# MohammadJohari/myslam

Measured on AMD Instinct MI355X. Metric: ray.samples/s (render+bwd), higher is better.
Workload: dtype f32; 1 GPU; BASELINE configs[1]: Replica room0 (synthetic), 4096 rays x 64 samples (56+8); mapping iteration: sample + render fwd + loss + bwd (planes+decoders), no optimiser; rays_of_the_job=4096, rays_this_rank=4096, samples_per_ray=64, plane_bytes=27147008, planes_layout=channels_last, parallelism=single GPU, launch=hipGraph replay of the captured iteration

## Files before the change

### include/eslam_hip.h

```cpp
#ifndef ESLAM_HIP_H
#define ESLAM_HIP_H

#include <stdint.h>

#ifdef __cplusplus
extern "C" {
#endif

#define ESLAM_ABI_VERSION 5
#define ESLAM_C_DIM 32
#define ESLAM_HIDDEN 16
#define ESLAM_FEAT (2 * ESLAM_C_DIM)
#define ESLAM_N_PLANES 12
#define ESLAM_MAX_SAMPLES 256
#define ESLAM_RAY_ORDERS 3
#define ESLAM_RAY_ORDER_WORDS(R) (ESLAM_RAY_ORDERS * (int64_t)(R) + 4)
#define ESLAM_N_DEC_PARAMS (2 * (16 * 64 + 16 + 16 * 16 + 16) + (1 * 16 + 1) + (3 * 16 + 3))

typedef void* eslam_stream_t;

typedef struct {
    const float* data;
    float* grad;
    int32_t h, w;
// ... 35 lines not shown
int eslam_importance_z(const eslam_plane_t* planes, const eslam_decoders_t* dec, const float* bound6_host,
                       const float* rays_o, const float* rays_d, const float* gt_depth, int R, int n_strat,
                       int n_imp, const float* t_free, const float* t_rand_uni, const float* u, float* z_vals,
                       eslam_stream_t stream);

int eslam_sample_z_all(const eslam_plane_t* planes, const eslam_decoders_t* dec, const float* bound6_host,
                       const float* rays_o, const float* rays_d, const float* gt_depth, int R, int n_strat, int n_imp,
                       double truncation, const float* t_free, const float* t_surf, const float* t_rand,
                       const float* t_rand_uni, const float* u, float* z_vals, eslam_stream_t stream);

int eslam_sample_z_all_rng(const eslam_plane_t* planes, const eslam_decoders_t* dec, const float* bound6_host,
                           const float* rays_o, const float* rays_d, const float* gt_depth, int R, int n_strat, int n_imp,
                           double truncation, const float* t_free, const float* t_surf, int perturb, uint64_t seed,
                           const uint32_t* rng_state, int64_t ray_offset, float* z_vals, eslam_stream_t stream);

int eslam_render_fwd(const eslam_plane_t* planes, const eslam_decoders_t* dec, const float* bound6_host,
                     const float* rays_o, const float* rays_d, const float* z_vals, int R, int S, float* depth,
                     float* rgb, float* sdf, float* raw_rgb, float* feat, const int32_t* ray_order,
                     uint32_t* rng_bump, eslam_stream_t stream);

int eslam_render_fwd_loss(const eslam_plane_t* planes, const eslam_decoders_t* dec, const float* bound6_host,
                          const float* rays_o, const float* rays_d, const float* z_vals, int R, int S, float* depth,
                          float* rgb, float* sdf, float* raw_rgb, float* feat, const int32_t* ray_order,
                          const float* gt_depth, const float* gt_color, double truncation, const float* weights5_host,
                          const uint8_t* ray_mask, float* scratch, float* acc, float* loss, uint32_t* rng_bump,
                          eslam_stream_t stream);

int eslam_planes_to_half(const eslam_plane_t* planes, eslam_stream_t stream);

int eslam_planes_relayout(const eslam_plane_t* src, const eslam_plane_t* dst, int field, eslam_stream_t stream);

int eslam_render_fwd_lowp(const eslam_plane_t* planes_f16, const eslam_decoders_t* dec, const float* bound6_host,
                          const float* rays_o, const float* rays_d, const float* z_vals, int R, int S, float* depth,
                          float* rgb, float* sdf, eslam_stream_t stream);

int eslam_ray_order(const float* rays_o, const float* rays_d, int R, int32_t* perm, eslam_stream_t stream);

int64_t eslam_bwd_workspace_bytes(int64_t n_points);

int eslam_render_bwd(const eslam_plane_t* planes, const eslam_decoders_t* dec, const float* bound6_host,
                     const float* rays_o, const float* rays_d, const float* z_vals, int R, int S,
                     const float* sdf, const float* raw_rgb, const float* feat, const float* g_depth,
                     const float* g_rgb, const float* g_sdf, float* g_dec, float* g_beta, float* g_rays_o,
                     float* g_rays_d, const int32_t* ray_order, void* workspace, eslam_stream_t stream);

int eslam_render_bwd_loss(const eslam_plane_t* planes, const eslam_decoders_t* dec, const float* bound6_host,
                          const float* rays_o, const float* rays_d, const float* z_vals, int R, int S,
                          const float* sdf, const float* raw_rgb, const float* feat, const float* depth,
                          const float* rgb, const float* gt_depth, const float* gt_color, double truncation,
                          const float* weights5_host, const uint8_t* ray_mask, const float* acc,
                          const float* upstream, float* loss_out, const float* g_depth, const float* g_rgb,
                          const float* g_sdf, float* g_dec, float* g_beta, float* g_rays_o, float* g_rays_d,
                          const int32_t* ray_order, void* workspace, eslam_stream_t stream);

#define ESLAM_DECODE_SDF_ONLY 1
#define ESLAM_DECODE_MASK_OUTSIDE 2
int eslam_decode_fwd(const eslam_plane_t* planes, const eslam_decoders_t* dec, const float* bound6_host,
                     const float* pts, int64_t N, int flags, float* raw, float* feat, eslam_stream_t stream);

int eslam_sdf_grid(const eslam_plane_t* planes, const eslam_decoders_t* dec, const float* bound6_host,
                   const float* xs, const float* ys, const float* zs, int64_t nx, int64_t ny, int64_t nz,
                   const float* halfspaces, int n_halfspaces, int flags, float* vol, eslam_stream_t stream);

int64_t eslam_mc_workspace_bytes(int64_t nx, int64_t ny, int64_t nz);
int eslam_mc_count(const float* vol, int64_t nx, int64_t ny, int64_t nz, float level, void* workspace, int64_t* counts,
                   eslam_stream_t stream);
int eslam_mc_emit(const float* vol, int64_t nx, int64_t ny, int64_t nz, float level, const double* origin3_host,
                  const double* spacing3_host, const void* workspace, int64_t n_verts, int64_t n_faces, float* verts,
                  int32_t* faces, eslam_stream_t stream);

int eslam_mc_count_masked(const float* vol, const float* weight, int64_t nx, int64_t ny, int64_t nz, float level,
                          void* workspace, int64_t* counts, eslam_stream_t stream);

int eslam_tsdf_integrate(float* tsdf, float* weight, float* color, int64_t nx, int64_t ny, int64_t nz,
                         const float* origin3_host, float voxel, float trunc, const float* depths, const float* colors,
                         const float* w2c, const float* depth_max, int n_frames, int H, int W, float fx, float fy, float cx,
                         float cy, eslam_stream_t stream);

int eslam_tsdf_sample_color(const float* color, int64_t nx, int64_t ny, int64_t nz, const float* origin3_host, float voxel,
                            const float* pts, int64_t n, float* out, eslam_stream_t stream);

int eslam_frame_out_shape(int Hc, int Wc, int Hd, int Wd, int crop_h, int crop_w, int crop_edge, int* H_out_host,
                          int* W_out_host);
int eslam_frame_prepare(const uint8_t* rgb, int Hc, int Wc, const uint16_t* depth, int Hd, int Wd, int crop_h, int crop_w,
                        int crop_edge, float png_depth_scale, float scale, float* color_out, float* depth_out,
                        eslam_stream_t stream);

int eslam_frame_undistort(const uint8_t* rgb, const float* grid, int H, int W, uint8_t* out, eslam_stream_t stream);

int eslam_cull_vertices(const float* verts, int64_t n_verts, const float* depths, int n_frames, int depth_h, int depth_w,
                        const float* w2c, float fx, float fy, float cx, float cy, int H, int W, float truncation,
                        int depth_test, uint8_t* seen, eslam_stream_t stream);

#define ESLAM_NN_MAX_CELLS (1 << 24)
#define ESLAM_NN_CELLS_PER_POINT 2
#define ESLAM_NN_INPUT_ORDER 1
typedef struct {
    float lo[3];
    float cell;
    int32_t dims[3];
    int32_t reserved;
} eslam_nn_grid_t;
int eslam_nn_grid_plan(int64_t n_ref, const float* bbox6_host, eslam_nn_grid_t* grid);
int64_t eslam_nn_workspace_bytes(const eslam_nn_grid_t* grid, int64_t n_ref);
int eslam_nn_build(const float* ref, int64_t n_ref, const eslam_nn_grid_t* grid, void* workspace, eslam_stream_t stream);
int64_t eslam_nn_query_workspace_bytes(const eslam_nn_grid_t* grid, int64_t n_query);
// ... 52 lines not shown
                    const double* stats, const uint8_t* lut, uint8_t* out, eslam_stream_t stream);

int eslam_views_see_points(const float* points, int64_t n_points, const float* w2c, int n_views, float fx, float fy,
                           float cx, float cy, int H, int W, uint8_t* seen, eslam_stream_t stream);

int eslam_decode_bwd(const eslam_plane_t* planes, const eslam_decoders_t* dec, const float* bound6_host,
                     const float* pts, int64_t N, const float* raw, const float* feat, const float* g_raw,
                     float* g_dec, float* g_pts, void* workspace, eslam_stream_t stream);

int eslam_mapping_loss(const float* depth, const float* rgb, const float* sdf, const float* z_vals,
                       const float* gt_depth, const float* gt_color, int R, int S, double truncation,
                       const float* weights5_host, const uint8_t* ray_mask, float* loss,
                       float* g_depth, float* g_rgb, float* g_sdf, void* scratch, eslam_stream_t stream);

#define ESLAM_LOSS_ACC 16
int eslam_loss_reduce(const float* depth, const float* rgb, const float* sdf, const float* z_vals,
                      const float* gt_depth, const float* gt_color, int R, int S, double truncation,
                      const uint8_t* ray_mask, float* acc, eslam_stream_t stream);
int eslam_loss_grad(const float* depth, const float* rgb, const float* sdf, const float* z_vals,
                    const float* gt_depth, const float* gt_color, int R, int S, double truncation,
                    const float* weights5_host, const uint8_t* ray_mask, const float* acc, float* loss,
                    float* g_depth, float* g_rgb, float* g_sdf, const float* upstream, eslam_stream_t stream);

#define ESLAM_ADAM_MAX_TENSORS 32
typedef struct {
    float* param;
    float* grad;
    float* exp_avg;
    float* exp_avg_sq;
    int64_t n;
    double lr;
} eslam_adam_tensor_t;
int eslam_adam_step(const eslam_adam_tensor_t* tensors_host, int n_tensors, int step, int32_t* step_dev,
                    double beta1, double beta2, double eps, int zero_grad, eslam_stream_t stream);

int eslam_keyframe_overlap(const float* rays_o, const float* rays_d, const float* gt_depth, int n_rays,
                           int num_samples, const float* c2ws, int n_keyframes, int H, int W, float fx, float fy,
                           float cx, float cy, int edge, int32_t* counts, eslam_stream_t stream);

#define ESLAM_TRACKING_MASK_MAX 8192
int eslam_prefilter(const float* rays_o, const float* rays_d, const float* gt_depth, int R, const float* bound6_host,
                    int need_depth, uint8_t* keep, eslam_stream_t stream);
int eslam_pose_to_c2w(const float* poses, int b, float* c2ws, eslam_stream_t stream);
int eslam_pose_to_c2w_bwd(const float* poses, const float* g_c2ws, int b, float* g_poses, eslam_stream_t stream);
int eslam_tracking_mask(const float* depth, const float* gt_depth, const uint8_t* keep, int R, float factor,
                        uint8_t* mask, eslam_stream_t stream);
int eslam_keep_best(const float* loss, const float* pose, int n, float* best, float* best_pose,
                    eslam_stream_t stream);

#define ESLAM_LOSS_SCRATCH (32 * 17)
int eslam_deterministic(void);
int eslam_scatter_bundle_samples(int64_t n, int S, int render);
int eslam_last_backward_rank16(void);

int eslam_stream_wait(eslam_stream_t waiter, eslam_stream_t signaler);

int eslam_zero_async(void* ptr, int64_t bytes, eslam_stream_t stream);
int64_t eslam_loss_scratch_floats(int64_t n_rays);
int eslam_loss_scratch_reset(float* scratch, int64_t floats, eslam_stream_t stream);
int eslam_loss_value(const float* depth, const float* rgb, const float* sdf, const float* z_vals,
                     const float* gt_depth, const float* gt_color, int R, int S, double truncation,
                     const float* weights5_host, const uint8_t* ray_mask, float* scratch, float* acc, float* loss,
                     eslam_stream_t stream);

#define ESLAM_PROF_KERNELS 12
int eslam_profile_enable(int on);
int eslam_profile_read(float* ms_out);
const char* eslam_profile_name(int kernel_id);

int eslam_loss_set_sizes(const float* gt_depth, const uint8_t* ray_mask, int R, int n_strat, int n_imp, double truncation,
                         const float* t_free, const float* t_surf, const float* t_rand, int perturb, uint64_t seed,
                         const uint32_t* rng_state, uint32_t* scratch, float* acc_out, eslam_stream_t stream);
int eslam_mark_rays(const eslam_plane_t* planes, const float* bound6_host, const float* rays_o, const float* rays_d,
                    const float* gt_depth, int R, double truncation, const int64_t* block_base_host, int64_t n_blocks,
                    uint8_t* touched, eslam_stream_t stream);
int64_t eslam_blocks_compact_scratch_words(int64_t n_blocks);
int eslam_blocks_compact(uint8_t* touched, int64_t n_blocks, uint32_t* scratch, int32_t* idx, int32_t* meta,
                         int32_t* host_meta_dev, int clear_touched, eslam_stream_t stream);
int eslam_host_meta_alloc(void** host_ptr, void** dev_ptr);
int eslam_host_meta_free(void* host_ptr);
int eslam_shard_prologue(float* clear_flat, const int32_t* clear_idx, const int32_t* clear_meta, int64_t clear_capacity,
                         float* clear_tail, int64_t clear_n_tail, const float* rays_o, const float* rays_d,
                         const float* gt_depth, const uint8_t* ray_mask, int R, int n_strat, int n_imp, double truncation,
                         const float* t_free, const float* t_surf, int perturb, uint64_t seed, const uint32_t* rng_state,
                         uint32_t* sizes_scratch, float* acc_out, const eslam_plane_t* mark_planes, const float* bound6_host,
                         const int64_t* block_base_host, int64_t n_blocks, uint8_t* touched, eslam_stream_t stream);
int eslam_blocks_pack_dev(const float* flat, const int32_t* idx, const int32_t* meta, int64_t capacity, const float* tail,
                          int64_t n_tail, int64_t tail_pad, float* buf, uint32_t* step_bump, eslam_stream_t stream);
int eslam_blocks_unpack_dev(float* flat, const int32_t* idx, const int32_t* meta, int64_t capacity, float* tail,
                            int64_t n_tail, int64_t tail_pad, const float* buf, eslam_stream_t stream);
int eslam_blocks_zero_dev(float* flat, const int32_t* idx, const int32_t* meta, int64_t capacity, float* tail, int64_t n_tail,
                          eslam_stream_t stream);

#ifdef __cplusplus
}
#endif
#endif
```

### myslam_amd/_hip.py

```python
import ctypes
import os
import threading

import torch

_HERE = os.path.dirname(os.path.abspath(__file__))
LIB_PATH = os.environ.get("ESLAM_HIP_LIB") or os.path.join(_HERE, "lib", "libeslam_hip.so")

ABI_VERSION = 5
RAY_ORDERS = 3


def ray_order_words(R):
    return RAY_ORDERS * int(R) + 4
N_DEC_PARAMS = 2692
N_PLANES = 12


class PlaneDesc(ctypes.Structure):
    _fields_ = [("data", ctypes.c_void_p), ("grad", ctypes.c_void_p), ("h", ctypes.c_int32), ("w", ctypes.c_int32),
                ("stride_c", ctypes.c_int64), ("stride_y", ctypes.c_int64), ("stride_x", ctypes.c_int64),
                ("data_f16", ctypes.c_void_p)]


# ... 15 lines not shown
NN_INPUT_ORDER = 1
ICP_MOMENTS = 17
MESH_MAX_COUNT = 1 << 30
RASTER_LARGE_AREA = 64
RASTER_Z_NEAR = 0.01
RASTER_Z_FAR = 20.0
STATS_BLOCK_PIXELS = 4096
SSIM_TILE_H = 16
SSIM_TILE_W = 32
Bound6 = ctypes.c_float * 6

_vp, _i, _i64, _f, _d = ctypes.c_void_p, ctypes.c_int, ctypes.c_int64, ctypes.c_float, ctypes.c_double
_PP = ctypes.POINTER(PlaneDesc)
_DP = ctypes.POINTER(DecodersDesc)
_BP = ctypes.POINTER(ctypes.c_float)
_GP = ctypes.POINTER(NnGrid)

SIGNATURES = {
    "eslam_last_error": (ctypes.c_char_p, []),
    "eslam_abi_version": (_i, []),
    "eslam_sample_rays": (_i, [_vp, _i, _i, _i, _i, _i, _i, _i, _i, _f, _f, _f, _f, _vp, _vp, _vp, _vp, _vp, _vp, _vp, _vp]),
    "eslam_sample_rays_bwd": (_i, [_vp, _i, _i, _i, _i, _i, _f, _f, _f, _f, _vp, _vp, _vp, _vp]),
    "eslam_image_rays": (_i, [_i, _i, _f, _f, _f, _f, _vp, _vp, _vp, _vp]),
    "eslam_aabb_exit": (_i, [_vp, _vp, _i, _BP, _vp, _vp]),
    "eslam_sample_z": (_i, [_vp, _i, _i, _i, _d, _vp, _vp, _vp, _vp, _vp]),
    "eslam_importance_z": (_i, [_PP, _DP, _BP, _vp, _vp, _vp, _i, _i, _i, _vp, _vp, _vp, _vp, _vp]),
    "eslam_sample_z_all": (_i, [_PP, _DP, _BP, _vp, _vp, _vp, _i, _i, _i, _d, _vp, _vp, _vp, _vp, _vp, _vp, _vp]),
    "eslam_sample_z_all_rng": (_i, [_PP, _DP, _BP, _vp, _vp, _vp, _i, _i, _i, _d, _vp, _vp, _i, ctypes.c_uint64, _vp, _i64, _vp, _vp]),
    "eslam_loss_set_sizes": (_i, [_vp, _vp, _i, _i, _i, _d, _vp, _vp, _vp, _i, ctypes.c_uint64, _vp, _vp, _vp, _vp]),
    "eslam_mark_rays": (_i, [_PP, _BP, _vp, _vp, _vp, _i, _d, _vp, _i64, _vp, _vp]),
    "eslam_blocks_compact_scratch_words": (_i64, [_i64]),
    "eslam_blocks_compact": (_i, [_vp, _i64, _vp, _vp, _vp, _vp, _i, _vp]),
    "eslam_host_meta_alloc": (_i, [ctypes.POINTER(ctypes.c_void_p), ctypes.POINTER(ctypes.c_void_p)]),
    "eslam_host_meta_free": (_i, [_vp]),
    "eslam_shard_prologue": (_i, [_vp, _vp, _vp, _i64, _vp, _i64, _vp, _vp, _vp, _vp, _i, _i, _i, _d, _vp, _vp, _i, ctypes.c_uint64,
                                  _vp, _vp, _vp, _PP, _BP, _vp, _i64, _vp, _vp]),
    "eslam_blocks_pack_dev": (_i, [_vp, _vp, _vp, _i64, _vp, _i64, _i64, _vp, _vp, _vp]),
    "eslam_blocks_unpack_dev": (_i, [_vp, _vp, _vp, _i64, _vp, _i64, _i64, _vp, _vp]),
    "eslam_blocks_zero_dev": (_i, [_vp, _vp, _vp, _i64, _vp, _i64, _vp]),
    "eslam_render_fwd": (_i, [_PP, _DP, _BP, _vp, _vp, _vp, _i, _i, _vp, _vp, _vp, _vp, _vp, _vp, _vp, _vp]),
    "eslam_render_fwd_loss": (_i, [_PP, _DP, _BP, _vp, _vp, _vp, _i, _i, _vp, _vp, _vp, _vp, _vp, _vp, _vp, _vp, _d, _BP, _vp,
                                   _vp, _vp, _vp, _vp, _vp]),
    "eslam_planes_to_half": (_i, [_PP, _vp]),
    "eslam_planes_relayout": (_i, [_PP, _PP, _i, _vp]),
    "eslam_render_fwd_lowp": (_i, [_PP, _DP, _BP, _vp, _vp, _vp, _i, _i, _vp, _vp, _vp, _vp]),
    "eslam_ray_order": (_i, [_vp, _vp, _i, _vp, _vp]),
    "eslam_stream_wait": (_i, [_vp, _vp]),
    "eslam_zero_async": (_i, [_vp, _i64, _vp]),
    "eslam_bwd_workspace_bytes": (_i64, [_i64]),
    "eslam_render_bwd": (_i, [_PP, _DP, _BP, _vp, _vp, _vp, _i, _i, _vp, _vp, _vp, _vp, _vp, _vp, _vp, _vp, _vp, _vp,
                              _vp, _vp, _vp]),
    "eslam_render_bwd_loss": (_i, [_PP, _DP, _BP, _vp, _vp, _vp, _i, _i, _vp, _vp, _vp, _vp, _vp, _vp, _vp, _d, _BP, _vp, _vp,
                                   _vp, _vp, _vp, _vp, _vp, _vp, _vp, _vp, _vp, _vp, _vp, _vp]),
    "eslam_decode_fwd": (_i, [_PP, _DP, _BP, _vp, _i64, _i, _vp, _vp, _vp]),
    "eslam_sdf_grid": (_i, [_PP, _DP, _BP, _vp, _vp, _vp, _i64, _i64, _i64, _vp, _i, _i, _vp, _vp]),
    "eslam_mc_workspace_bytes": (_i64, [_i64, _i64, _i64]),
    "eslam_mc_count": (_i, [_vp, _i64, _i64, _i64, _f, _vp, _vp, _vp]),
    "eslam_mc_emit": (_i, [_vp, _i64, _i64, _i64, _f, ctypes.POINTER(_d), ctypes.POINTER(_d), _vp, _i64, _i64, _vp, _vp, _vp]),
    "eslam_mc_count_masked": (_i, [_vp, _vp, _i64, _i64, _i64, _f, _vp, _vp, _vp]),
    "eslam_tsdf_integrate": (_i, [_vp, _vp, _vp, _i64, _i64, _i64, ctypes.POINTER(_f), _f, _f, _vp, _vp, _vp, _vp, _i, _i, _i,
                                  _f, _f, _f, _f, _vp]),
    "eslam_tsdf_sample_color": (_i, [_vp, _i64, _i64, _i64, ctypes.POINTER(_f), _f, _vp, _i64, _vp, _vp]),
    "eslam_frame_out_shape": (_i, [_i, _i, _i, _i, _i, _i, _i, ctypes.POINTER(_i), ctypes.POINTER(_i)]),
    "eslam_frame_prepare": (_i, [_vp, _i, _i, _vp, _i, _i, _i, _i, _i, _f, _f, _vp, _vp, _vp]),
    "eslam_frame_undistort": (_i, [_vp, _vp, _i, _i, _vp, _vp]),
    "eslam_cull_vertices": (_i, [_vp, _i64, _vp, _i, _i, _i, _vp, _f, _f, _f, _f, _i, _i, _f, _i, _vp, _vp]),
    "eslam_nn_grid_plan": (_i, [_i64, _BP, _GP]),
    "eslam_nn_workspace_bytes": (_i64, [_GP, _i64]),
    "eslam_nn_build": (_i, [_vp, _i64, _GP, _vp, _vp]),
    "eslam_nn_query_workspace_bytes": (_i64, [_GP, _i64]),
    "eslam_nn_query": (_i, [_GP, _vp, _i64, _vp, _i64, _f, _i, _vp, _vp, _vp, _vp]),
    "eslam_icp_moments_workspace_bytes": (_i64, []),
    "eslam_icp_moments": (_i, [_vp, _vp, _vp, _vp, _i64, _f, _vp, _vp, _vp]),
    "eslam_mesh_weld_workspace_bytes": (_i64, [_i64]),
    "eslam_mesh_weld": (_i, [_vp, _i64, _vp, _vp, _vp]),
    "eslam_mesh_components": (_i, [_vp, _i64, _i64, _vp, _vp]),
    "eslam_mesh_component_sizes": (_i, [_vp, _i64, _vp, _i64, _vp, _vp]),
    "eslam_raster_workspace_bytes": (_i64, [_i64, _i, _i, _i]),
    "eslam_raster_depth": (_i, [_vp, _i64, _vp, _i64, _vp, _i, _f, _f, _f, _f, _i, _i, _f, _f, _i, _vp, _vp, _vp]),
    "eslam_viewer_workspace_bytes": (_i64, [_i64, _i, _i, _i]),
    "eslam_viewer_begin": (_i, [_i, _i, _i, _vp, _vp]),
    "eslam_viewer_mesh": (_i, [_vp, _i64, _vp, _i64, _vp, _vp, _i, _f, _f, _f, _f, _i, _i, _f, _f, _i, _i, _vp, _vp]),
    "eslam_viewer_points": (_i, [_vp, _i64, _vp, _i, _i, _vp, _i, _f, _f, _f, _f, _i, _i, _f, _f, _vp, _vp]),
    "eslam_viewer_resolve": (_i, [_i, _i, _i, _i, _i, _i, _vp, _vp, _vp, _vp]),
    "eslam_depth_l1_workspace_bytes": (_i64, [_i]),
    "eslam_depth_l1": (_i, [_vp, _vp, _i, _i64, _vp, _vp, _vp]),
    "eslam_views_see_points": (_i, [_vp, _i64, _vp, _i, _f, _f, _f, _f, _i, _i, _vp, _vp]),
    "eslam_frame_stats_workspace_bytes": (_i64, [_i, _i]),
    "eslam_frame_stats": (_i, [_vp, _vp, _vp, _vp, _i, _i, _vp, _vp, _vp]),
    "eslam_ssim_workspace_bytes": (_i64, [_i, _i, _i]),
    "eslam_ssim": (_i, [_vp, _vp, _i, _i, _i, _vp, _vp, _vp, _vp]),
    "eslam_vis_panel": (_i, [_vp, _vp, _vp, _vp, _i, _i, _vp, _vp, _vp, _vp]),
    "eslam_decode_bwd": (_i, [_PP, _DP, _BP, _vp, _i64, _vp, _vp, _vp, _vp, _vp, _vp, _vp]),
    "eslam_mapping_loss": (_i, [_vp, _vp, _vp, _vp, _vp, _vp, _i, _i, _d, _BP, _vp, _vp, _vp, _vp, _vp, _vp, _vp]),
    "eslam_loss_reduce": (_i, [_vp, _vp, _vp, _vp, _vp, _vp, _i, _i, _d, _vp, _vp, _vp]),
    "eslam_profile_enable": (_i, [_i]),
    "eslam_profile_read": (_i, [_BP]),
    "eslam_profile_name": (ctypes.c_char_p, [_i]),
    "eslam_loss_grad": (_i, [_vp, _vp, _vp, _vp, _vp, _vp, _i, _i, _d, _BP, _vp, _vp, _vp, _vp, _vp, _vp, _vp, _vp]),
    "eslam_deterministic": (_i, []),
    "eslam_scatter_bundle_samples": (_i, [_i64, _i, _i]),
    "eslam_last_backward_rank16": (_i, []),
    "eslam_loss_scratch_floats": (_i64, [_i64]),
    "eslam_loss_scratch_reset": (_i, [_vp, _i64, _vp]),
    "eslam_loss_value": (_i, [_vp, _vp, _vp, _vp, _vp, _vp, _i, _i, _d, _BP, _vp, _vp, _vp, _vp, _vp]),
    "eslam_adam_step": (_i, [_vp, _i, _i, _vp, _d, _d, _d, _i, _vp]),
    "eslam_prefilter": (_i, [_vp, _vp, _vp, _i, _BP, _i, _vp, _vp]),
    "eslam_pose_to_c2w": (_i, [_vp, _i, _vp, _vp]),
    "eslam_pose_to_c2w_bwd": (_i, [_vp, _vp, _i, _vp, _vp]),
    "eslam_tracking_mask": (_i, [_vp, _vp, _vp, _i, _f, _vp, _vp]),
    "eslam_keep_best": (_i, [_vp, _vp, _i, _vp, _vp, _vp]),
    "eslam_keyframe_overlap": (_i, [_vp, _vp, _vp, _i, _i, _vp, _i, _i, _i, _f, _f, _f, _f, _i, _vp, _vp]),
}

PROF_KERNELS = 12


class AdamTensor(ctypes.Structure):
    _fields_ = [("param", ctypes.c_void_p), ("grad", ctypes.c_void_p), ("exp_avg", ctypes.c_void_p),
                ("exp_avg_sq", ctypes.c_void_p), ("n", ctypes.c_int64), ("lr", ctypes.c_double)]


_lib = None
_lock = threading.Lock()


def load_library(path=None):
    global _lib
    with _lock:
        if _lib is not None and path is None:
            return _lib
        p = path or LIB_PATH
        if not os.path.exists(p):
            raise RuntimeError(
                f"HIP extension not built: {p} is missing. Run `python -c 'import __graft_entry__ as g; g.build()'` "
                "(or `make -C myslam_amd/csrc`). There is no CPU fallback for the render path.")
        lib = ctypes.CDLL(p)
        for name, (res, args) in SIGNATURES.items():
            fn = getattr(lib, name)
            fn.restype = res
            fn.argtypes = args
        if lib.eslam_abi_version() != ABI_VERSION:
            raise RuntimeError(f"ABI mismatch: library reports version {lib.eslam_abi_version()}, binding expects {ABI_VERSION}")
        if path is None:
            _lib = lib
        return lib


def lib():
    return _lib if _lib is not None else load_library()


def check(rc, what):
    if rc != 0:
        msg = lib().eslam_last_error()
# ... 159 lines not shown
```

### myslam_amd/csrc/eslam_decode_tile.h

```cpp
#pragma once
#include "eslam_common.h"

__device__ __forceinline__ int piece_channel(int g, int i) { return i < 4 ? 4 * g + i : 12 + 4 * g + i; }

template <bool CL>
__device__ __forceinline__ void gather8(const eslam_plane_t& P, float u, float v, int q, float acc[8]) {
    const AxisCoord ax = axis_coord(u, P.w);
    const AxisCoord ay = axis_coord(v, P.h);
    const float w00 = (1.0f - ax.t) * (1.0f - ay.t);
    const float w01 = ax.t * (1.0f - ay.t);
    const float w10 = (1.0f - ax.t) * ay.t;
    const float w11 = ax.t * ay.t;
    const unsigned sy = (unsigned)P.stride_y, sx = (unsigned)P.stride_x;
    const unsigned r0 = ay.i0 * sy, r1 = ay.i1 * sy;
    const unsigned c0 = ax.i0 * sx, c1 = ax.i1 * sx;
    const float* __restrict__ data = P.data;
    if (CL) {
        const unsigned q4 = 4u * q;
        const unsigned o00 = r0 + c0 + q4, o01 = r0 + c1 + q4, o10 = r1 + c0 + q4, o11 = r1 + c1 + q4;
        const float4_t a00 = *(const float4_t*)(data + o00), b00 = *(const float4_t*)(data + o00 + 16u);
        const float4_t a01 = *(const float4_t*)(data + o01), b01 = *(const float4_t*)(data + o01 + 16u);
        const float4_t a10 = *(const float4_t*)(data + o10), b10 = *(const float4_t*)(data + o10 + 16u);
        const float4_t a11 = *(const float4_t*)(data + o11), b11 = *(const float4_t*)(data + o11 + 16u);
#pragma unroll
        for (int i = 0; i < 4; ++i) {
            acc[i] += a00[i] * w00 + a01[i] * w01 + a10[i] * w10 + a11[i] * w11;
            acc[4 + i] += b00[i] * w00 + b01[i] * w01 + b10[i] * w10 + b11[i] * w11;
        }
    } else {
        const unsigned sc = (unsigned)P.stride_c;
#pragma unroll
        for (int i = 0; i < 8; ++i) {
            const unsigned co = (unsigned)piece_channel(q, i) * sc;
            acc[i] += data[co + r0 + c0] * w00 + data[co + r0 + c1] * w01 + data[co + r1 + c0] * w10 +
                      data[co + r1 + c1] * w11;
        }
    }
}

struct DecFrag {
    float w1[16];
    float4_t w2;
    float4_t w3;
    float4_t b1, b2;
    float4_t b3;
};

__device__ __forceinline__ void load_dec_frag(DecFrag& f, const float* L, int r, int q) {
#pragma unroll
    for (int lvl = 0; lvl < 2; ++lvl) {
        const float4_t a = *(const float4_t*)(L + DEC_W1 + r * 64 + lvl * 32 + 4 * q);
        const float4_t b = *(const float4_t*)(L + DEC_W1 + r * 64 + lvl * 32 + 16 + 4 * q);
#pragma unroll
        for (int i = 0; i < 4; ++i) {
            f.w1[lvl * 8 + i] = a[i];
            f.w1[lvl * 8 + 4 + i] = b[i];
        }
    }
    f.w2 = *(const float4_t*)(L + DEC_W2 + r * 16 + 4 * q);
    f.w3 = *(const float4_t*)(L + DEC_W3 + (r & 3) * 16 + 4 * q);
    f.b1 = *(const float4_t*)(L + DEC_B1 + 4 * q);
    f.b2 = *(const float4_t*)(L + DEC_B2 + 4 * q);
    f.b3 = *(const float4_t*)(L + DEC_B3);
}

__device__ __forceinline__ void mlp_hidden(const DecFrag& f, const float feat[16], float4_t& h1, float4_t& h2) {
    float4_t a1 = f.b1;
#pragma unroll
    for (int ks = 0; ks < 16; ++ks) a1 = mfma16(f.w1[ks], feat[ks], a1);
#pragma unroll
    for (int i = 0; i < 4; ++i) h1[i] = fmaxf(a1[i], 0.0f);
    float4_t a2 = f.b2;
#pragma unroll
    for (int ks = 0; ks < 4; ++ks) a2 = mfma16(f.w2[ks], h1[ks], a2);
#pragma unroll
    for (int i = 0; i < 4; ++i) h2[i] = fmaxf(a2[i], 0.0f);
}

__device__ __forceinline__ void mlp_out_accum(const DecFrag& f, const float4_t& h2, int b, int r, float4_t& out) {
    const bool mine = (r >> 2) == b;
#pragma unroll
    for (int ks = 0; ks < 4; ++ks) out = mfma16(mine ? f.w3[ks] : 0.0f, h2[ks], out);
}

#define GATHER_PIPELINE 1

struct PlaneTaps {
    float4_t a00, b00, a01, b01, a10, b10, a11, b11;
    float w00, w01, w10, w11;
};

__device__ __forceinline__ void issue_taps(const eslam_plane_t& P, float u, float v, int q, PlaneTaps& t) {
    const AxisCoord ax = axis_coord(u, P.w);
    const AxisCoord ay = axis_coord(v, P.h);
    t.w00 = (1.0f - ax.t) * (1.0f - ay.t);
    t.w01 = ax.t * (1.0f - ay.t);
    t.w10 = (1.0f - ax.t) * ay.t;
    t.w11 = ax.t * ay.t;
    const unsigned sy = (unsigned)P.stride_y, sx = (unsigned)P.stride_x;
    const unsigned r0 = ay.i0 * sy, r1 = ay.i1 * sy;
    const unsigned c0 = ax.i0 * sx, c1 = ax.i1 * sx;
    const float* __restrict__ data = P.data;
    const unsigned q4 = 4u * q;
    const unsigned o00 = r0 + c0 + q4, o01 = r0 + c1 + q4, o10 = r1 + c0 + q4, o11 = r1 + c1 + q4;
    t.a00 = *(const float4_t*)(data + o00); t.b00 = *(const float4_t*)(data + o00 + 16u);
    t.a01 = *(const float4_t*)(data + o01); t.b01 = *(const float4_t*)(data + o01 + 16u);
    t.a10 = *(const float4_t*)(data + o10); t.b10 = *(const float4_t*)(data + o10 + 16u);
    t.a11 = *(const float4_t*)(data + o11); t.b11 = *(const float4_t*)(data + o11 + 16u);
}

__device__ __forceinline__ void accumulate_taps(const PlaneTaps& t, float acc[8]) {
#pragma unroll
    for (int i = 0; i < 4; ++i) {
        acc[i] += t.a00[i] * t.w00 + t.a01[i] * t.w01 + t.a10[i] * t.w10 + t.a11[i] * t.w11;
        acc[4 + i] += t.b00[i] * t.w00 + t.b01[i] * t.w01 + t.b10[i] * t.w10 + t.b11[i] * t.w11;
    }
}

template <bool CL>
__device__ __forceinline__ void gather_features(const PlaneSet& planes, int d, float x, float y, float z, int q,
                                                float feat[16], int opaque0) {
#pragma unroll
    for (int i = 0; i < 16; ++i) feat[i] = 0.0f;
    if (CL && GATHER_PIPELINE) {
        constexpr int D = GATHER_PIPELINE + 1;
        PlaneTaps taps[D];
#pragma unroll
        for (int k = 0; k < D - 1 && k < 6; ++k)
            issue_taps(planes.p[2 * (3 * d + (k % 3)) + (k / 3) + opaque0], ORIENT_U(k % 3, x, y, z),
                       ORIENT_V(k % 3, x, y, z), q, taps[k % D]);
// ... 18 lines not shown
        }
    }
}

__device__ __forceinline__ void issue_plane0(const PlaneSet& planes, int d, float x, float y, float z, int q, int opaque0,
                                             PlaneTaps& t) {
    issue_taps(planes.p[6 * d + opaque0], ORIENT_U(0, x, y, z), ORIENT_V(0, x, y, z), q, t);
}

__device__ __forceinline__ void gather_features_chain(const PlaneSet& planes, int d, float x, float y, float z, int q,
                                                      float feat[16], int opaque0, PlaneTaps& carry, int dn, float xn, float yn,
                                                      float zn) {
#pragma unroll
    for (int i = 0; i < 16; ++i) feat[i] = 0.0f;
    PlaneTaps odd;
#pragma unroll
    for (int k = 0; k < 6; ++k) {
        const int kn = k + 1;
        if (kn < 6) {
            issue_taps(planes.p[2 * (3 * d + (kn % 3)) + (kn / 3) + opaque0], ORIENT_U(kn % 3, x, y, z),
                       ORIENT_V(kn % 3, x, y, z), q, (kn & 1) ? odd : carry);
        } else {
            issue_plane0(planes, dn, xn, yn, zn, q, opaque0, carry);
        }
        accumulate_taps((k & 1) ? odd : carry, feat + 8 * (k / 3));
        __builtin_amdgcn_sched_barrier(0);
    }
}

__device__ __forceinline__ void store_features(float* feat_out, int64_t pt, int d, int q, const float feat[16]) {
    float* dst = feat_out + pt * 128 + d * 64 + 4 * q;
#pragma unroll
    for (int lvl = 0; lvl < 2; ++lvl) {
        float4_t a, b;
#pragma unroll
        for (int i = 0; i < 4; ++i) {
            a[i] = feat[lvl * 8 + i];
            b[i] = feat[lvl * 8 + 4 + i];
        }
        __builtin_nontemporal_store(a, (float4_t*)(dst + lvl * 32));
        __builtin_nontemporal_store(b, (float4_t*)(dst + lvl * 32 + 16));
    }
}

typedef unsigned uint4_bits __attribute__((ext_vector_type(4)));
#define ESLAM_OOB_OFFSET 0xFFFFFF00u
__device__ __forceinline__ void store_features_buffer(__amdgpu_buffer_rsrc_t rsrc, unsigned byte_off, const float feat[16]) {
#pragma unroll
    for (int j = 0; j < 4; ++j)
        __builtin_amdgcn_raw_buffer_store_b128(__builtin_bit_cast(uint4_bits, (float4_t){feat[4 * j], feat[4 * j + 1], feat[4 * j + 2], feat[4 * j + 3]}),
                                               rsrc, (int)byte_off + 64 * j, 0, 2);
}

__device__ __forceinline__ void load_features(const float* feat_in, int64_t pt, int d, int q, float feat[16]) {
    const float* src = feat_in + pt * 128 + d * 64 + 4 * q;
#pragma unroll
    for (int lvl = 0; lvl < 2; ++lvl) {
        const float4_t a = *(const float4_t*)(src + lvl * 32), b = *(const float4_t*)(src + lvl * 32 + 16);
#pragma unroll
        for (int i = 0; i < 4; ++i) {
            feat[lvl * 8 + i] = a[i];
            feat[lvl * 8 + 4 + i] = b[i];
        }
    }
}

template <bool CL> __device__ __forceinline__ int gather_point(int lane) { return CL ? lane >> 2 : lane & 15; }
template <bool CL> __device__ __forceinline__ int gather_piece(int lane) { return CL ? lane & 3 : lane >> 4; }

template <bool CL, int NREG>
__device__ __forceinline__ void to_mfma_role(float v[NREG], int lane) {
    if (!CL) return;
    const int src = (((lane & 15) << 2) | (lane >> 4)) << 2;
#pragma unroll
    for (int i = 0; i < NREG; ++i) v[i] = __int_as_float(__builtin_amdgcn_ds_bpermute(src, __float_as_int(v[i])));
}

template <bool CL, int NREG>
__device__ __forceinline__ void to_gather_role(float v[NREG], int lane) {
    if (!CL) return;
    const int src = (((lane & 3) << 4) | (lane >> 2)) << 2;
#pragma unroll
    for (int i = 0; i < NREG; ++i) v[i] = __int_as_float(__builtin_amdgcn_ds_bpermute(src, __float_as_int(v[i])));
}

typedef _Float16 half8_t __attribute__((ext_vector_type(8)));
typedef short short8_t __attribute__((ext_vector_type(8)));
typedef short short4_t __attribute__((ext_vector_type(4)));
#define LP_W1 0
#define LP_W2 1024
#define LP_W3 1280
#define LP_SHORTS 1344
#define LP_BIAS_FLOATS 36
#define LP_LDS_FLOATS (LP_SHORTS + 2 * LP_BIAS_FLOATS)

__device__ __forceinline__ short f2bf(float x) {
    unsigned u = __builtin_bit_cast(unsigned, x);
    u += 0x7FFFu + ((u >> 16) & 1u);
    return (short)(u >> 16);
}
__device__ __forceinline__ short4_t pack4(float a, float b, float c, float d) { return (short4_t){f2bf(a), f2bf(b), f2bf(c), f2bf(d)}; }

__device__ __forceinline__ short* lp_weights(float* lds, int d) { return (short*)lds + d * LP_SHORTS; }
__device__ __forceinline__ float* lp_biases(float* lds, int d) { return lds + LP_SHORTS + d * LP_BIAS_FLOATS; }

__device__ __forceinline__ void stage_decoder_weights_lowp(float* lds, const eslam_decoders_t& dec, int tid, int nthreads) {
// ... 118 lines not shown
```

### myslam_amd/csrc/eslam_render_bwd.hip

```cpp
#include <stdlib.h>
#include "eslam_decode_tile.h"
#include "eslam_loss_final.h"
#include "eslam_dec_reduce.h"

struct RayUp { float gd, gr, gg, gb; };

__device__ __forceinline__ float4_t composite_bwd_chunk(const RayUp up, float beta, bool valid, float sd, float z, float cr,
                                                        float cg, float cb, float g_sdf_s, float trans_in, float& carry,
                                                        float& gbeta_acc, int lane) {
    const float sg = sigmoidf_(-sd * beta);
    const float e = expf(-beta * sg);
    const float alpha = valid ? 1.0f - e : 0.0f;
    const float fac = valid ? (1.0f - alpha) + 1e-10f : 1.0f;
    const float pin = wave_incl_prod(fac, lane);
    const float pex = wave_up1(pin, 1.0f);
    const float T = trans_in * pex;
    const float w = alpha * T;
    const float gw = (up.gd != 0.0f ? up.gd * z : 0.0f) + up.gr * cr + up.gg * cg + up.gb * cb;
    const float v = valid ? gw * w : 0.0f;
    const float vn = wave_down1(v, 0.0f);
    const float after_local = wave_incl_suffix_sum(vn, lane);
    const float after = after_local + carry;
    const float g_alpha = gw * T - after / fac;
    carry += wave_lane<0>(after_local) + wave_lane<0>(v);
    float4_t o = (float4_t){0.f, 0.f, 0.f, 0.f};
    if (valid) {
        const float ds = sg * (1.0f - sg);
        const float dalpha_dsdf = -beta * beta * e * ds;
        const float dalpha_dbeta = e * (sg - beta * ds * sd);
        gbeta_acc += g_alpha * dalpha_dbeta;
        const float g_sdf_tot = g_sdf_s + g_alpha * dalpha_dsdf;
        o[0] = w * up.gr * cr * (1.0f - cr);
        o[1] = w * up.gg * cg * (1.0f - cg);
        o[2] = w * up.gb * cb * (1.0f - cb);
        o[3] = g_sdf_tot * (1.0f - sd * sd);
    }
    return o;
}

__global__ void decode_act_bwd_kernel(const float* __restrict__ raw, const float* __restrict__ g_raw, int64_t N,
                                      float* __restrict__ g_o) {
    const int64_t i = (int64_t)blockIdx.x * blockDim.x + threadIdx.x;
    if (i >= N) return;
    const float4_t v = *(const float4_t*)(raw + 4 * i);
    const float4_t g = *(const float4_t*)(g_raw + 4 * i);
    float4_t o;
    o[0] = g[0] * v[0] * (1.0f - v[0]);
    o[1] = g[1] * v[1] * (1.0f - v[1]);
    o[2] = g[2] * v[2] * (1.0f - v[2]);
    o[3] = g[3] * (1.0f - v[3] * v[3]);
    *(float4_t*)(g_o + 4 * i) = o;
}

#define TP 20
#define TPF 68
#define TPH 72

struct RayBwdIn {
    const float* z_vals;
    const float* sdf;
    const float* raw_rgb;
    const float* beta;
    const float* g_depth;
    const float* g_rgb;
    const float* g_sdf;
    float* beta_parts;
    int R, S;
};

template <int MODE, bool WGRAD, bool LOWP, bool GZ = false>
__global__ __launch_bounds__(256, 2) void mlp_bwd_kernel(const eslam_decoders_t dec, const float* __restrict__ feat,
                                                      const float* __restrict__ g_o, int64_t N,
                                                      float* __restrict__ g_feat, float* __restrict__ slabs,
                                                      const RayBwdIn rb, const LossGradIn li) {
    __shared__ __attribute__((aligned(16))) float wlds[2 * DEC_LDS];
    __shared__ __attribute__((aligned(16))) float tiles[4][4][16 * TP];
    __shared__ __attribute__((aligned(16))) float gtile[4][64 * 4];
    __shared__ __attribute__((aligned(16))) float ftile[WGRAD ? 4 : 1][WGRAD ? (LOWP ? 16 * TPH / 2 : 16 * TPF) : 4];
    if (LOWP) stage_decoder_weights_lowp(wlds, dec, threadIdx.x, blockDim.x);
    else stage_decoder_weights(wlds, dec, threadIdx.x, blockDim.x);
    __syncthreads();

    static_assert(!GZ || (!LOWP && MODE != 0), "GZ: float32 rays only");
    const int d = blockIdx.y;
    const int nout = d ? 3 : 1;
    const float* L = wlds + d * DEC_LDS;
    const int lane = threadIdx.x & 63, wave = threadIdx.x >> 6;
    const int r = lane & 15, q = lane >> 4;
    const int gp = lane >> 2, gq = lane & 3;
    float* tz1 = tiles[wave][0];
    float* tz2 = tiles[wave][1];
    float* th1 = tiles[wave][2];
    float* th2 = tiles[wave][3];
    float* gt = gtile[wave];

    DecFrag f;
    float w3col[4], w2t[4], w1t[4][4];
    DecFragLP fl;
    short4_t w3colp = {0, 0, 0, 0}, w2tp = {0, 0, 0, 0}, w1tp[4];
    if (LOWP) {
        const short* W = lp_weights(wlds, d);
        load_dec_frag_lp(fl, W, lp_biases(wlds, d), r, q);
#pragma unroll
        for (int jj = 0; jj < 4; ++jj) {
            if (q == 0) w3colp[jj] = W[LP_W3 + jj * 16 + r];
            w2tp[jj] = W[LP_W2 + (4 * q + jj) * 16 + r];
#pragma unroll
            for (int mb = 0; mb < 4; ++mb) w1tp[mb][jj] = W[LP_W1 + (4 * q + jj) * 64 + 16 * mb + r];
        }
    } else {
    load_dec_frag(f, L, r, q);
#pragma unroll
    for (int ks = 0; ks < 4; ++ks) {
        w3col[ks] = L[DEC_W3 + ks * 16 + r];
        w2t[ks] = L[DEC_W2 + (4 * q + ks) * 16 + r];
#pragma unroll
        for (int mb = 0; mb < 4; ++mb)
            if (!GZ) w1t[mb][ks] = L[DEC_W1 + (4 * q + ks) * 64 + (mb >> 1) * 32 + 16 * (mb & 1) + r];
    }
    }

    float4_t gW1[4], gW2, gW3, gb1, gb2;
#pragma unroll
    for (int i = 0; i < 4; ++i) gW1[i] = (float4_t){0.f, 0.f, 0.f, 0.f};
    gW2 = gW3 = gb1 = gb2 = (float4_t){0.f, 0.f, 0.f, 0.f};
    float gb3[3] = {0.f, 0.f, 0.f};
    float gbeta_acc = 0.0f;

    typedef unsigned uint4_t __attribute__((ext_vector_type(4)));
    const __amdgpu_buffer_rsrc_t gfrsrc = __builtin_amdgcn_make_buffer_rsrc((void*)g_feat, 0, (int)((unsigned)N * (GZ ? 128u : 512u)), 0x00020000);
    auto dropped_stores = [&]() {
#pragma unroll
        for (int j = 0; j < (GZ ? 1 : 4); ++j) __builtin_amdgcn_raw_buffer_store_b128((uint4_t){0u, 0u, 0u, 0u}, gfrsrc, (int)(0xFFFFFF00u + 16u * j), 0, 0);
    };
    const unsigned gz_base = (unsigned)d * ((unsigned)N * 64u);
    auto store_gz = [&](const int64_t p0, const int b, const int nvalid, const float gzr[4]) {
        const unsigned off = (16 * b + gp < nvalid) ? (unsigned)(p0 + 16 * b + gp) * 64u + gz_base + (unsigned)(gq * 16) : 0xFFFFFF00u;
        __builtin_amdgcn_raw_buffer_store_b128(__builtin_bit_cast(uint4_t, (float4_t){gzr[0], gzr[1], gzr[2], gzr[3]}), gfrsrc, (int)off, 0, 0);
    };
    auto store_rows = [&](const int64_t p0, const int b, const int nvalid, const float gf[16]) {
        const unsigned off = (16 * b + gp < nvalid) ? (unsigned)(p0 + 16 * b + gp) * 512u + (unsigned)(d * 256 + gq * 16) : 0xFFFFFF00u;
#pragma unroll
        for (int j = 0; j < 4; ++j)
            __builtin_amdgcn_raw_buffer_store_b128(__builtin_bit_cast(uint4_t, (float4_t){gf[4 * j], gf[4 * j + 1], gf[4 * j + 2], gf[4 * j + 3]}),
                                                   gfrsrc, (int)off + 64 * j, 0, 0);
    };
    auto load_block = [&](int b, float4_t v[4], const int64_t pbase) {
        const int64_t pt = min(pbase + 16 * b + gp, N - 1);
        if (LOWP) {
            const short* fp = (const short*)feat + pt * 128 + d * 64 + 8 * gq;
            v[0] = *(const float4_t*)(fp);
            v[1] = *(const float4_t*)(fp + 32);
            v[2] = v[3] = (float4_t){0.f, 0.f, 0.f, 0.f};
            return;
        }
        const float* fp = feat + pt * 128 + d * 64 + 4 * gq;
        v[0] = *(const float4_t*)(fp);
        v[1] = *(const float4_t*)(fp + 16);
        v[2] = *(const float4_t*)(fp + 32);
        v[3] = *(const float4_t*)(fp + 48);
    };
#define TOUCH(x) asm volatile("" :: "v"(x))
#define TOUCH_ROWS { TOUCH(fnext[0]); TOUCH(fnext[1]); TOUCH(fnext[2]); TOUCH(fnext[3]); }
    float4_t fnext[4];
    auto tile_bwd = [&](const int64_t p0, const int nvalid, const float go[4], const int64_t p0_next) {
        const int nblk = (nvalid + 15) >> 4;
        __builtin_assume(nblk >= 1);
#pragma unroll
        for (int o = 0; o < 3; ++o) gb3[o] += go[o];
        *(float4_t*)(gt + lane * 4) = (float4_t){go[0], go[1], go[2], go[3]};

#pragma unroll 1
        for (int b = 0; b < nblk; ++b) {
            float ft[16];
#pragma unroll
            for (int i = 0; i < 4; ++i) {
                ft[i] = fnext[0][i]; ft[4 + i] = fnext[1][i]; ft[8 + i] = fnext[2][i]; ft[12 + i] = fnext[3][i];
            }
            load_block(0, fnext, b + 1 < nblk ? p0 + 16 * (b + 1) : p0_next);
            float4_t fbk[4];
            short4_t fbkp[4];
            if (WGRAD && LOWP) {
                short* T = (short*)ftile[wave] + gp * TPH + 8 * gq;
                *(float4_t*)(T) = (float4_t){ft[0], ft[1], ft[2], ft[3]};
                *(float4_t*)(T + 32) = (float4_t){ft[4], ft[5], ft[6], ft[7]};
            } else if (WGRAD) {
                float* T = ftile[wave] + gp * TPF + 4 * gq;
#pragma unroll
                for (int j = 0; j < 4; ++j) *(float4_t*)(T + 16 * j) = (float4_t){ft[4 * j], ft[4 * j + 1], ft[4 * j + 2], ft[4 * j + 3]};
            }
            if (LOWP) to_mfma_role<true, 8>(ft, lane);
            else to_mfma_role<true, 16>(ft, lane);
            float4_t h1, h2, gz1, gz2;
            const float4_t zero4 = (float4_t){0.f, 0.f, 0.f, 0.f};
            float gf[16];
            if (LOWP) {
                float4_t a1, a2;
                short8_t bfeat[2];
#pragma unroll
                for (int lvl = 0; lvl < 2; ++lvl)
#pragma unroll
                    for (int i = 0; i < 4; ++i) {
                        const unsigned u = __builtin_bit_cast(unsigned, ft[lvl * 4 + i]);
                        bfeat[lvl][2 * i] = (short)(u & 0xFFFFu);
                        bfeat[lvl][2 * i + 1] = (short)(u >> 16);
                    }
                mlp_hidden_lp_bf(fl, bfeat, a1, a2);
#pragma unroll
                for (int i = 0; i < 4; ++i) { h1[i] = fmaxf(a1[i], 0.f); h2[i] = fmaxf(a2[i], 0.f); }
                const float s0 = __shfl(go[0], 16 * b + r, WAVE), s1 = __shfl(go[1], 16 * b + r, WAVE), s2 = __shfl(go[2], 16 * b + r, WAVE);
                const short4_t bgo = (q == 0) ? pack4(s0, s1, s2, 0.f) : (short4_t){0, 0, 0, 0};
                const float4_t gh2 = __builtin_amdgcn_mfma_f32_16x16x16bf16_1k(w3colp, bgo, zero4, 0, 0, 0);
#pragma unroll
                for (int i = 0; i < 4; ++i) gz2[i] = a2[i] > 0.0f ? gh2[i] : 0.0f;
                const float4_t gh1 = __builtin_amdgcn_mfma_f32_16x16x16bf16_1k(w2tp, pack4(gz2[0], gz2[1], gz2[2], gz2[3]), zero4, 0, 0, 0);
#pragma unroll
                for (int i = 0; i < 4; ++i) gz1[i] = a1[i] > 0.0f ? gh1[i] : 0.0f;
                gb1 += gz1;
                gb2 += gz2;
                const short4_t bz1 = pack4(gz1[0], gz1[1], gz1[2], gz1[3]);
#pragma unroll
                for (int mb = 0; mb < 4; ++mb) {
                    const float4_t acc = __builtin_amdgcn_mfma_f32_16x16x16bf16_1k(w1tp[mb], bz1, zero4, 0, 0, 0);
#pragma unroll
                    for (int i = 0; i < 4; ++i) gf[4 * mb + i] = acc[i];
                }
                to_gather_role<true, 16>(gf, lane);
                store_rows(p0, b, nvalid, gf);
            } else {
            mlp_hidden(f, ft, h1, h2);

            float4_t gh2 = (float4_t){0.f, 0.f, 0.f, 0.f};
            const bool mine = (q == b);
#pragma unroll
            for (int ks = 0; ks < 4; ++ks) gh2 = mfma16(mine ? w3col[ks] : 0.0f, go[ks], gh2);
#pragma unroll
            for (int i = 0; i < 4; ++i) gz2[i] = h2[i] > 0.0f ? gh2[i] : 0.0f;
            float4_t gh1 = (float4_t){0.f, 0.f, 0.f, 0.f};
#pragma unroll
            for (int ks = 0; ks < 4; ++ks) gh1 = mfma16(w2t[ks], gz2[ks], gh1);
#pragma unroll
            for (int i = 0; i < 4; ++i) gz1[i] = h1[i] > 0.0f ? gh1[i] : 0.0f;
            gb1 += gz1;
            gb2 += gz2;

            if (GZ) {
                float gzr[4] = {gz1[0], gz1[1], gz1[2], gz1[3]};
                to_gather_role<true, 4>(gzr, lane);
                store_gz(p0, b, nvalid, gzr);
            } else {
#pragma unroll
            for (int mb = 0; mb < 4; ++mb) {
                float4_t acc = (float4_t){0.f, 0.f, 0.f, 0.f};
#pragma unroll
                for (int ks = 0; ks < 4; ++ks) acc = mfma16(w1t[mb][ks], gz1[ks], acc);
#pragma unroll
                for (int i = 0; i < 4; ++i) gf[(mb >> 1) * 8 + 4 * (mb & 1) + i] = acc[i];
            }
            to_gather_role<true, 16>(gf, lane);
            store_rows(p0, b, nvalid, gf);
            }
            }
            if (!WGRAD) continue;

            *(float4_t*)(tz1 + r * TP + 4 * q) = gz1;
            *(float4_t*)(tz2 + r * TP + 4 * q) = gz2;
            *(float4_t*)(th1 + r * TP + 4 * q) = h1;
            *(float4_t*)(th2 + r * TP + 4 * q) = h2;
            WAVE_SYNC();

            float az1[4], az2[4], bh1[4], bh2[4], ago[4];
#pragma unroll
            for (int ks = 0; ks < 4; ++ks) {
                const int prow = 4 * q + ks;
                az1[ks] = tz1[prow * TP + r];
                az2[ks] = tz2[prow * TP + r];
                bh1[ks] = th1[prow * TP + r];
                bh2[ks] = th2[prow * TP + r];
                ago[ks] = (r < 4) ? gt[(16 * b + prow) * 4 + r] : 0.0f;
            }
            if (LOWP) {
                gW2 = __builtin_amdgcn_mfma_f32_16x16x16bf16_1k(pack4(az2[0], az2[1], az2[2], az2[3]),
                                                                pack4(bh1[0], bh1[1], bh1[2], bh1[3]), gW2, 0, 0, 0);
                gW3 = __builtin_amdgcn_mfma_f32_16x16x16bf16_1k(pack4(ago[0], ago[1], ago[2], ago[3]),
                                                                pack4(bh2[0], bh2[1], bh2[2], bh2[3]), gW3, 0, 0, 0);
                const short4_t a1p = pack4(az1[0], az1[1], az1[2], az1[3]);
#pragma unroll
                for (int ks = 0; ks < 4; ++ks) fbkp[ks] = *(const short4_t*)((const short*)ftile[wave] + (4 * q + ks) * TPH + 4 * r);
#pragma unroll
                for (int nb = 0; nb < 4; ++nb)
                    gW1[nb] = __builtin_amdgcn_mfma_f32_16x16x16bf16_1k(a1p, (short4_t){fbkp[0][nb], fbkp[1][nb], fbkp[2][nb], fbkp[3][nb]},
                                                                        gW1[nb], 0, 0, 0);
            } else {
#pragma unroll
            for (int ks = 0; ks < 4; ++ks) {
                gW2 = mfma16(az2[ks], bh1[ks], gW2);
                gW3 = mfma16(ago[ks], bh2[ks], gW3);
            }
#pragma unroll
            for (int ks = 0; ks < 4; ++ks) fbk[ks] = *(const float4_t*)(ftile[wave] + (4 * q + ks) * TPF + 4 * r);
#pragma unroll
            for (int ks = 0; ks < 4; ++ks) {
#pragma unroll
                for (int nb = 0; nb < 4; ++nb) gW1[nb] = mfma16(az1[ks], fbk[ks][nb], gW1[nb]);
            }
            }
            WAVE_SYNC();
        }
    };

    if (MODE == 0) {
        const int64_t ntiles = (N + 63) / 64;
        int64_t tile = (int64_t)blockIdx.x * 4 + wave;
        if (tile < ntiles) {
            load_block(0, fnext, tile * 64);
            dropped_stores();
        }
        for (; tile < ntiles; tile += (int64_t)gridDim.x * 4) {
            const int64_t p0 = tile * 64;
            const int nvalid = (int)min((int64_t)64, N - p0);
            float go[4] = {0.f, 0.f, 0.f, 0.f};
            if (lane < nvalid) {
                const float4_t g = *(const float4_t*)(g_o + (p0 + lane) * 4);
                if (d == 0) go[0] = g[3];
                else { go[0] = g[0]; go[1] = g[1]; go[2] = g[2]; }
            }
            TOUCH_ROWS
            tile_bwd(p0, nvalid, go, (tile + (int64_t)gridDim.x * 4) * 64);
        }
    } else {
        const int R = rb.R, S = rb.S;
        const int nchunk = (S + WAVE - 1) / WAVE;
        __builtin_assume(nchunk >= 1);
        const float beta = rb.beta[0];
        LossW lw = {};
        LossK lk = {};
        float nd = 1.0f, ncol = 1.0f;
        if (MODE == 2) {
            lw = loss_scaled_weights(li.w, li.upstream);
            lk = loss_sdf_factors(lw, li.tr, li.acc);
            nd = li.acc[A_N_DEPTH]; ncol = li.acc[A_N_COLOR];
            if (blockIdx.x == 0 && blockIdx.y == 0 && threadIdx.x == 0 && li.loss_out)
                li.loss_out[0] = loss_value_from_acc(li.w, li.acc);
        }
        struct RayIn { float gd, gr, gg, gb, gtd, dep, cr, cg, cb, tr, tg, tb; int mask; };
        struct ChunkIn { float sd, z, cr, cg, cb, gs; };
        auto load_ray = [&](int ray) {
            RayIn x;
            x.gd = rb.g_depth ? rb.g_depth[ray] : 0.0f;
            x.gr = rb.g_rgb ? rb.g_rgb[3 * ray + 0] : 0.0f;
            x.gg = rb.g_rgb ? rb.g_rgb[3 * ray + 1] : 0.0f;
            x.gb = rb.g_rgb ? rb.g_rgb[3 * ray + 2] : 0.0f;
            x.gtd = x.dep = x.cr = x.cg = x.cb = x.tr = x.tg = x.tb = 0.0f;
            x.mask = 1;
            if (MODE == 2) {
                x.gtd = li.gt_depth[ray];
                x.mask = li.ray_mask ? (int)li.ray_mask[ray] : 1;
                x.dep = li.depth[ray];
                x.cr = li.rgb[3 * ray + 0]; x.cg = li.rgb[3 * ray + 1]; x.cb = li.rgb[3 * ray + 2];
                x.tr = li.gt_color[3 * ray + 0]; x.tg = li.gt_color[3 * ray + 1]; x.tb = li.gt_color[3 * ray + 2];
            }
            return x;
        };
        auto load_chunk = [&](int ray, int c) {
            ChunkIn x = {0.f, 0.f, 0.f, 0.f, 0.f, 0.f};
            const int s = c * WAVE + lane;
            if (s < S) {
                const int64_t i = (int64_t)ray * S + s;
                x.sd = rb.sdf[i];
                x.z = rb.z_vals[i];
                x.cr = rb.raw_rgb[i * 3 + 0];
                x.cg = rb.raw_rgb[i * 3 + 1];
                x.cb = rb.raw_rgb[i * 3 + 2];
                if (rb.g_sdf) x.gs = rb.g_sdf[i];
            }
            return x;
        };
        static_assert(ESLAM_MAX_SAMPLES <= 4 * WAVE, "pass A prefetch holds three chunks");
        struct PassA { float sd[3]; };
        auto load_pa = [&](int ray) {
            PassA x = {{0.f, 0.f, 0.f}};
#pragma unroll
            for (int k = 0; k < 3; ++k)
                if (k < nchunk - 1) x.sd[k] = rb.sdf[(int64_t)ray * S + k * WAVE + lane];
            return x;
        };
        const int stride = gridDim.x * 4;
        int ray = blockIdx.x * 4 + wave;
        RayIn rin = {};
        ChunkIn cin = {};
        PassA pin = {{0.f, 0.f, 0.f}};
        if (ray < R) {
            rin = load_ray(ray);
            cin = load_chunk(ray, nchunk - 1);
            pin = load_pa(ray);
            load_block(0, fnext, (int64_t)ray * S + (nchunk - 1) * WAVE);
        }
        dropped_stores();
#define TOUCH_CHUNK(ci) { TOUCH(ci.sd); TOUCH(ci.z); TOUCH(ci.cr); TOUCH(ci.cg); TOUCH(ci.cb); TOUCH(ci.gs); }
        for (; ray < R; ray += stride) {
            const int64_t base = (int64_t)ray * S;
            TOUCH(rin.gd); TOUCH(rin.gr); TOUCH(rin.gg); TOUCH(rin.gb); TOUCH(rin.gtd); TOUCH(rin.dep); TOUCH(rin.cr); TOUCH(rin.cg);
            TOUCH(rin.cb); TOUCH(rin.tr); TOUCH(rin.tg); TOUCH(rin.tb); TOUCH(rin.mask);
            TOUCH_CHUNK(cin)
            TOUCH(pin.sd[0]); TOUCH(pin.sd[1]); TOUCH(pin.sd[2]);
            TOUCH_ROWS
            ChunkIn ch = cin;
            RayIn rnx = {};
            ChunkIn cnx = {};
            PassA pnx = {{0.f, 0.f, 0.f}};
            if (ray + stride < R) { rnx = load_ray(ray + stride); cnx = load_chunk(ray + stride, nchunk - 1); pnx = load_pa(ray + stride); }
            RayUp up;
            up.gd = rin.gd; up.gr = rin.gr; up.gg = rin.gg; up.gb = rin.gb;
            const float gtd = rin.gtd;
            bool m = false;
            if (MODE == 2) {
                const bool mc = rin.mask != 0;
                m = mc && gtd > 0.0f;
                up.gd += loss_g_depth(m, gtd, rin.dep, lw, nd);
                up.gr += loss_g_color(mc, rin.tr, rin.cr, lw, ncol);
                up.gg += loss_g_color(mc, rin.tg, rin.cg, lw, ncol);
                up.gb += loss_g_color(mc, rin.tb, rin.cb, lw, ncol);
            }
            float myprod = 1.0f;
#pragma unroll
            for (int c = 0; c < 3; ++c) {
                if (c < nchunk - 1) {
                    const float sd = pin.sd[c];
                    const float alpha = 1.0f - expf(-beta * sigmoidf_(-sd * beta));
                    const float cp = wave_lane<63>(wave_incl_prod((1.0f - alpha) + 1e-10f, lane));
                    if (lane == c) myprod = cp;
                }
            }
            float carry = 0.0f;
            int c = nchunk - 1;
            do {
                ChunkIn cn = {};
                if (c > 0) cn = load_chunk(ray, c - 1);
                float trans_in = 1.0f;
                for (int k = 0; k < c; ++k) trans_in *= __shfl(myprod, k, WAVE);
                const bool valid = c * WAVE + lane < S;
                float gs = ch.gs;
                if (MODE == 2 && valid) gs += loss_g_sdf(m, ch.z, ch.sd, gtd, li.tr, lk);
                const float4_t o = composite_bwd_chunk(up, beta, valid, ch.sd, ch.z, ch.cr, ch.cg, ch.cb, gs, trans_in, carry,
                                                       gbeta_acc, lane);
                float go[4] = {0.f, 0.f, 0.f, 0.f};
                if (d == 0) go[0] = o[3];
                else { go[0] = o[0]; go[1] = o[1]; go[2] = o[2]; }
                tile_bwd(base + c * WAVE, min(WAVE, S - c * WAVE), go,
                         c > 0 ? base + (c - 1) * WAVE : (int64_t)(ray + stride) * S + (nchunk - 1) * WAVE);
                if (c > 0) {
                    TOUCH_CHUNK(cn)
                    TOUCH_ROWS
                    ch = cn;
                }
            } while (--c >= 0);
            rin = rnx;
            cin = cnx;
            pin = pnx;
        }
#undef TOUCH_CHUNK
        __shared__ float beta_part[4];
        const float tot = wave_sum(gbeta_acc);
        if (lane == 0) beta_part[wave] = tot;
        __syncthreads();
        if (d == 0 && threadIdx.x == 0 && rb.beta_parts)
            rb.beta_parts[blockIdx.x] = (beta_part[0] + beta_part[1]) + (beta_part[2] + beta_part[3]);
    }

    if (!WGRAD) return;
    __shared__ __attribute__((aligned(16))) float comb[4][SLAB];
    float* sl = comb[wave];
    for (int i = lane; i < SLAB; i += WAVE) sl[i] = 0.0f;
    WAVE_SYNC();
#pragma unroll
    for (int reg = 0; reg < 4; ++reg) {
        const int j = 4 * q + reg;
        float4_t v;
#pragma unroll
        for (int nb = 0; nb < 4; ++nb) v[nb] = gW1[nb][reg];
        *(float4_t*)(sl + SL_W1 + j * 64 + 4 * r) = v;
        sl[SL_W2 + j * 16 + r] = gW2[reg];
        if (q == 0 && reg < nout) sl[SL_W3 + reg * 16 + r] = gW3[reg];
    }
#pragma unroll
    for (int reg = 0; reg < 4; ++reg) {
        float a = gb1[reg], c = gb2[reg];
#pragma unroll
        for (int m = 8; m >= 1; m >>= 1) {
            a += __shfl_xor(a, m, WAVE);
            c += __shfl_xor(c, m, WAVE);
        }
        if (r == 0) {
            sl[SL_B1 + 4 * q + reg] = a;
            sl[SL_B2 + 4 * q + reg] = c;
        }
    }
#pragma unroll
    for (int o = 0; o < 3; ++o) {
        const float t = wave_sum(gb3[o]);
        if (lane == 0 && o < nout) sl[SL_B3 + o] = t;
    }
    __syncthreads();
// ... 236 lines not shown
    }
    if (RENDER) {
        const bool any_live = __ballot(live) != 0ull;
#pragma unroll
        for (int k = 0; k < 3; ++k) {
            const float a = wave_sum(go_acc[k]);
            const float b = wave_sum(gd_acc[k]);
            if (lane == 0) {
                g_rays_o[unit * 3 + k] = a;
                g_rays_d[unit * 3 + k] = any_live ? b : 0.0f;
            }
        }
    } else if (16 * g + r < scount) {
        float* dst = g_rays_o + (base + 16 * g + r) * 3;
        dst[0] = go_acc[0]; dst[1] = go_acc[1]; dst[2] = go_acc[2];
    }
}

bool eslam_planes_channels_last(const eslam_plane_t* planes, int first, int count);
int eslam_validate_planes(const eslam_plane_t* planes, int first, int count);
int eslam_planes_lowp(const eslam_plane_t* planes);

static Bound make_bound(const float* b6) {
    Bound b;
    for (int k = 0; k < 3; ++k) {
        b.lo[k] = b6[2 * k];
        b.hi[k] = b6[2 * k + 1];
    }
    return b;
}

#define MLP_BWD_MAX_WG 256

int eslam_scatter_v2(const eslam_plane_t* planes, const Bound& bnd, const float* rays_o, const float* rays_d,
                     const float* z_or_pts, int64_t R, int S, bool render, const float* g_feat, const int* perm,
                     hipStream_t st, const DecReduceArgs* red, const eslam_decoders_t* gz_dec);
bool eslam_scatter_can_reduce(bool render);


static int64_t align256(int64_t v) { return (v + 255) & ~(int64_t)255; }

static int64_t slab_region_bytes(int64_t n_points) {
    return ((int64_t)MLP_BWD_MAX_WG * 4 * 2 * SLAB + n_points / 4 + 1) * 4;
}

extern "C" int64_t eslam_bwd_workspace_bytes(int64_t n_points) {
    if (n_points < 0) return -1;
    return align256(n_points * 4 * 4) + align256(n_points * 128 * 4) +
           align256(slab_region_bytes(n_points)) + align256(n_points * 4);
}

static int g_last_backward_rank16 = 0;
extern "C" int eslam_last_backward_rank16(void) { return g_last_backward_rank16; }

static int bwd_common(const eslam_plane_t* planes, const eslam_decoders_t* dec, const Bound& bnd, const float* rays_o,
                      const float* rays_d, const float* z_or_pts, int64_t R, int S, int mode, const float* feat,
                      float* g_o, float* g_feat, float* slabs, const int* perm, float* g_dec, float* g_out_a, float* g_out_b,
                      RayBwdIn rb, const LossGradIn* li, float* g_beta, hipStream_t st) {
    const bool render = mode != 0;
    const int64_t N = render ? R * S : R;
    PlaneSet ps;
    for (int i = 0; i < NPL; ++i) ps.p[i] = planes[i];
    const bool cl = eslam_planes_channels_last(planes, 0, NPL);

    const int64_t ntiles = render ? R : (N + 63) / 64;
    const int nwg = (int)((ntiles + 3) / 4 < MLP_BWD_MAX_WG ? (ntiles + 3) / 4 : MLP_BWD_MAX_WG);
    float* beta_parts = slabs + (int64_t)MLP_BWD_MAX_WG * 4 * 2 * SLAB;
    rb.beta_parts = render ? beta_parts : nullptr;
    const LossGradIn none = {};
    if (N * 512 >= ((int64_t)1 << 32) - 256) {
        eslam_set_error("backward: %lld points exceed the 32-bit offset range of the feature-gradient buffer (8.3 M): split the batch",
                        (long long)N);
        return 1;
    }
    eslam_prof_begin(PROF_MLP_BWD, st);
#define LAUNCH_MB(MD, WG, LP, ...) \
    hipLaunchKernelGGL((mlp_bwd_kernel<MD, WG, LP, ##__VA_ARGS__>), dim3(nwg, 2), dim3(256), 0, st, *dec, feat, g_o, N, g_feat, slabs, rb, \
                       li ? *li : none)
    const int lowp = eslam_planes_lowp(planes);
    if (lowp < 0) return 1;
    bool any_grad = false, all_grad = true;
    for (int i = 0; i < NPL; ++i) {
        any_grad |= planes[i].grad != nullptr;
        all_grad &= planes[i].grad != nullptr;
    }
    if (any_grad && !all_grad) {
        eslam_set_error("plane gradients must be requested for all 12 planes or for none");
        return 1;
    }
    const bool gz = !lowp && render && any_grad && !g_out_a && !eslam_deterministic();
    g_last_backward_rank16 = gz ? 1 : 0;
    if (gz) {
        if (mode == 1) { if (g_dec) LAUNCH_MB(1, true, false, true); else LAUNCH_MB(1, false, false, true); }
        else { if (g_dec) LAUNCH_MB(2, true, false, true); else LAUNCH_MB(2, false, false, true); }
    }
    else if (lowp) {
        if (mode == 0) { if (g_dec) LAUNCH_MB(0, true, true); else LAUNCH_MB(0, false, true); }
        else if (mode == 1) { if (g_dec) LAUNCH_MB(1, true, true); else LAUNCH_MB(1, false, true); }
        else { if (g_dec) LAUNCH_MB(2, true, true); else LAUNCH_MB(2, false, true); }
    }
    else if (mode == 0) { if (g_dec) LAUNCH_MB(0, true, false); else LAUNCH_MB(0, false, false); }
    else if (mode == 1) { if (g_dec) LAUNCH_MB(1, true, false); else LAUNCH_MB(1, false, false); }
    else { if (g_dec) LAUNCH_MB(2, true, false); else LAUNCH_MB(2, false, false); }
#undef LAUNCH_MB
    eslam_prof_end(PROF_MLP_BWD, st);
    if (int rc = eslam_check_launch("mlp_bwd_kernel")) return rc;
    const int n_beta_parts = render ? nwg : 0;
    DecReduceArgs red = {};
    red.slabs = slabs; red.nrows = nwg; red.g_dec = g_dec;
    red.beta_parts = render ? beta_parts : nullptr; red.n_beta_parts = n_beta_parts; red.g_beta = g_beta;
    const bool fold = g_dec && any_grad && eslam_scatter_can_reduce(render);
    if (g_dec && !fold) {
        eslam_prof_begin(PROF_DEC_REDUCE, st);
        hipLaunchKernelGGL(dec_grad_reduce_kernel, dim3(DEC_RED_COLBLOCKS, 2), dim3(1024), 0, st, red);
        eslam_prof_end(PROF_DEC_REDUCE, st);
        if (int rc = eslam_check_launch("dec_grad_reduce_kernel")) return rc;
    } else if (!g_dec && g_beta && render) {
        hipLaunchKernelGGL(beta_sum_kernel, dim3(1), dim3(1024), 0, st, beta_parts, n_beta_parts, g_beta);
        if (int rc = eslam_check_launch("beta_sum_kernel")) return rc;
    }

    if (any_grad) {
        eslam_prof_begin(PROF_SCATTER, st);
        if (int rc = eslam_scatter_v2(planes, bnd, rays_o, rays_d, z_or_pts, R, S, render, g_feat, perm, st, fold ? &red : nullptr,
                                      gz ? dec : nullptr))
            return rc;
        eslam_prof_end(PROF_SCATTER, st);
    }
    if (g_out_a) {
        const int64_t nunits = render ? R : (N + 63) / 64;
        dim3 grid((unsigned)((nunits + 3) / 4)), block(256);
#define LAUNCH(CLv, RD)                                                                                            \
    hipLaunchKernelGGL((coord_bwd_kernel<CLv, RD>), grid, block, 0, st, ps, bnd, rays_o, rays_d, z_or_pts, (int)R, \
                       S, g_feat, g_out_a, g_out_b)
        eslam_prof_begin(PROF_COORD_BWD, st);
        if (lowp && render)
            hipLaunchKernelGGL(coord_bwd_lowp_kernel<true>, grid, block, 0, st, ps, bnd, rays_o, rays_d, z_or_pts, (int)R, S, g_feat,
                               g_out_a, g_out_b);
        else if (lowp)
            hipLaunchKernelGGL(coord_bwd_lowp_kernel<false>, grid, block, 0, st, ps, bnd, rays_o, rays_d, z_or_pts, (int)R, S, g_feat,
                               g_out_a, g_out_b);
        else if (cl && render) LAUNCH(true, true);
        else if (cl) LAUNCH(true, false);
        else if (render) LAUNCH(false, true);
        else LAUNCH(false, false);
#undef LAUNCH
        eslam_prof_end(PROF_COORD_BWD, st);
        if (int rc = eslam_check_launch("coord_bwd_kernel")) return rc;
    }
    return 0;
}

static int render_bwd_impl(const char* who, const eslam_plane_t* planes, const eslam_decoders_t* dec,
                           const float* bound6_host, const float* rays_o, const float* rays_d, const float* z_vals, int R,
                           int S, const float* sdf, const float* raw_rgb, const float* feat, const float* g_depth,
                           const float* g_rgb, const float* g_sdf, const LossGradIn* li, float* g_dec, float* g_beta,
                           float* g_rays_o, float* g_rays_d, const int32_t* ray_order, void* workspace,
                           eslam_stream_t stream) {
    if (R <= 0) return 0;
    if (S <= 0 || S > ESLAM_MAX_SAMPLES) {
        eslam_set_error("%s: S=%d outside [1,%d]", who, S, ESLAM_MAX_SAMPLES);
        return 1;
    }
    if (!planes || !dec || !bound6_host || !rays_o || !rays_d || !z_vals || !sdf || !raw_rgb || !feat || !workspace) {
        eslam_set_error("%s: null argument", who);
        return 1;
    }
    if ((g_rays_o == nullptr) != (g_rays_d == nullptr)) {
        eslam_set_error("%s: g_rays_o and g_rays_d must both be given or both be NULL", who);
        return 1;
    }
    if ((int64_t)R * S * 128 >= ((int64_t)1 << 40)) {
        eslam_set_error("%s: batch too large", who);
        return 1;
    }
    if (eslam_validate_planes(planes, 0, NPL)) return 1;
    hipStream_t st = (hipStream_t)stream;
    const int64_t N = (int64_t)R * S;
    char* ws = (char*)workspace;
    float* g_o = (float*)ws;
    float* g_feat = (float*)(ws + align256(N * 16));
    float* slabs = (float*)(ws + align256(N * 16) + align256(N * 512));
    const int* perm = ray_order;
    bool scatter_runs = false;
    for (int i = 0; i < NPL; ++i) scatter_runs = scatter_runs || planes[i].grad != nullptr;
    if (!perm && scatter_runs && (int64_t)ESLAM_RAY_ORDER_WORDS(R) <= N) {
        int* own = (int*)(ws + align256(N * 16) + align256(N * 512) + align256(slab_region_bytes(N)));
        if (int rc = eslam_ray_order(rays_o, rays_d, R, own, st)) return rc;
        perm = own;
    }
    const Bound bnd = make_bound(bound6_host);
    RayBwdIn rb = {};
    rb.z_vals = z_vals; rb.sdf = sdf; rb.raw_rgb = raw_rgb; rb.beta = dec->beta;
    rb.g_depth = g_depth; rb.g_rgb = g_rgb; rb.g_sdf = g_sdf; rb.R = R; rb.S = S;
    return bwd_common(planes, dec, bnd, rays_o, rays_d, z_vals, R, S, li ? 2 : 1, feat, g_o, g_feat, slabs, perm, g_dec,
                      g_rays_o, g_rays_d, rb, li, g_beta, st);
}

extern "C" int eslam_render_bwd(const eslam_plane_t* planes, const eslam_decoders_t* dec, const float* bound6_host,
                                const float* rays_o, const float* rays_d, const float* z_vals, int R, int S,
                                const float* sdf, const float* raw_rgb, const float* feat, const float* g_depth,
                                const float* g_rgb, const float* g_sdf, float* g_dec, float* g_beta, float* g_rays_o,
                                float* g_rays_d, const int32_t* ray_order, void* workspace, eslam_stream_t stream) {
    return render_bwd_impl("eslam_render_bwd", planes, dec, bound6_host, rays_o, rays_d, z_vals, R, S, sdf, raw_rgb, feat,
                           g_depth, g_rgb, g_sdf, nullptr, g_dec, g_beta, g_rays_o, g_rays_d, ray_order, workspace, stream);
}

extern "C" int eslam_render_bwd_loss(const eslam_plane_t* planes, const eslam_decoders_t* dec, const float* bound6_host,
                                     const float* rays_o, const float* rays_d, const float* z_vals, int R, int S,
                                     const float* sdf, const float* raw_rgb, const float* feat, const float* depth,
                                     const float* rgb, const float* gt_depth, const float* gt_color, double truncation,
                                     const float* weights5_host, const uint8_t* ray_mask, const float* acc,
                                     const float* upstream, float* loss_out, const float* g_depth, const float* g_rgb,
                                     const float* g_sdf, float* g_dec, float* g_beta, float* g_rays_o, float* g_rays_d,
                                     const int32_t* ray_order, void* workspace, eslam_stream_t stream) {
    if (!depth || !rgb || !gt_depth || !gt_color || !weights5_host || !acc) {
        eslam_set_error("eslam_render_bwd_loss: null loss argument");
        return 1;
    }
    LossGradIn li = {};
    li.gt_depth = gt_depth; li.gt_color = gt_color; li.ray_mask = ray_mask; li.depth = depth; li.rgb = rgb;
    li.acc = acc; li.upstream = upstream; li.loss_out = loss_out;
    li.tr = make_trunc(truncation);
    li.w = LossW{weights5_host[0], weights5_host[1], weights5_host[2], weights5_host[3], weights5_host[4]};
    return render_bwd_impl("eslam_render_bwd_loss", planes, dec, bound6_host, rays_o, rays_d, z_vals, R, S, sdf, raw_rgb,
                           feat, g_depth, g_rgb, g_sdf, &li, g_dec, g_beta, g_rays_o, g_rays_d, ray_order, workspace, stream);
}

extern "C" int eslam_decode_bwd(const eslam_plane_t* planes, const eslam_decoders_t* dec, const float* bound6_host,
                                const float* pts, int64_t N, const float* raw, const float* feat, const float* g_raw,
                                float* g_dec, float* g_pts, void* workspace, eslam_stream_t stream) {
    if (N <= 0) return 0;
    if (!planes || !dec || !bound6_host || !pts || !raw || !feat || !g_raw || !workspace) {
        eslam_set_error("eslam_decode_bwd: null argument");
        return 1;
    }
    if (N >= ((int64_t)1 << 31)) {
        eslam_set_error("eslam_decode_bwd: N too large");
        return 1;
    }
    if (eslam_validate_planes(planes, 0, NPL)) return 1;
    hipStream_t st = (hipStream_t)stream;
    char* ws = (char*)workspace;
    float* g_o = (float*)ws;
    float* g_feat = (float*)(ws + align256(N * 16));
    float* slabs = (float*)(ws + align256(N * 16) + align256(N * 512));
    const Bound bnd = make_bound(bound6_host);
    hipLaunchKernelGGL(decode_act_bwd_kernel, dim3((unsigned)((N + 255) / 256)), dim3(256), 0, st, raw, g_raw, N, g_o);
    if (int rc = eslam_check_launch("decode_act_bwd_kernel")) return rc;
    return bwd_common(planes, dec, bnd, nullptr, nullptr, pts, N, 64, 0, feat, g_o, g_feat, slabs, nullptr, g_dec,
                      g_pts, nullptr, RayBwdIn{}, nullptr, nullptr, st);
}
```

### myslam_amd/csrc/eslam_render_fwd.hip

```cpp
#include "eslam_decode_tile.h"
#include "eslam_loss_final.h"

struct LossIn {
    const float* gt_depth;
    const float* gt_color;
    const uint8_t* ray_mask;
    float* scratch;
    float* acc;
    float* loss;
    Trunc tr;
    LossW w;
    int det;
};

#define FWD_WAVES 2

#define DECODE_LP_WAVES 3

template <bool CL, bool SAVE, bool LOSS, bool LOWP>
__global__ __launch_bounds__(256, FWD_WAVES) void render_fwd_kernel(const PlaneSet planes, const eslam_decoders_t dec,
                                                         const Bound bnd, const float* __restrict__ rays_o,
                                                         const float* __restrict__ rays_d,
                                                         const float* __restrict__ z_vals, int R, int S,
                                                         float* __restrict__ depth_out, float* __restrict__ rgb_out,
                                                         float* __restrict__ sdf_out, float* __restrict__ raw_rgb_out,
                                                         float* __restrict__ feat_out, const int* __restrict__ perm,
                                                         const LossIn li, uint32_t* __restrict__ rng_bump) {
    if (rng_bump && blockIdx.x == 0 && threadIdx.x == 0) rng_bump[0] += 1u;
    __shared__ __attribute__((aligned(16))) float wlds[2 * DEC_LDS];
    static_assert(LP_LDS_FLOATS <= 2 * DEC_LDS, "the bf16 weight image shares the float32 image's LDS");
    if (LOWP) stage_decoder_weights_lowp(wlds, dec, threadIdx.x, blockDim.x);
    else stage_decoder_weights(wlds, dec, threadIdx.x, blockDim.x);
    __syncthreads();

    const int lane = threadIdx.x & 63;
    const int wave = threadIdx.x >> 6;
    const int r = lane & 15, q = lane >> 4;
    const int gp = gather_point<CL>(lane), gq = gather_piece<CL>(lane);
    const __amdgpu_buffer_rsrc_t frsrc = __builtin_amdgcn_make_buffer_rsrc((void*)feat_out, 0, (int)((unsigned)R * (unsigned)S * 512u), 0x00020000);
    float lv[A_COUNT];
#pragma unroll
    for (int k = 0; k < A_COUNT; ++k) lv[k] = 0.0f;
    const int cpx = gridDim.x >> 3;
    const int lblock = (blockIdx.x & 7) * cpx + (blockIdx.x >> 3);
    if (!LOSS && lblock * 4 + wave >= R) return;
    for (int slot = lblock * 4 + wave; slot < R; slot += (int)gridDim.x * 4) {
    const int ray = perm ? perm[slot] : slot;
    const float gtd = LOSS ? li.gt_depth[ray] : 0.0f;
    const bool in_batch = LOSS ? (li.ray_mask ? li.ray_mask[ray] != 0 : true) : false;
    const bool has_depth = in_batch && gtd > 0.0f;

    const float ox = rays_o[ray * 3 + 0], oy = rays_o[ray * 3 + 1], oz = rays_o[ray * 3 + 2];
    const float dx = rays_d[ray * 3 + 0], dy = rays_d[ray * 3 + 1], dz = rays_d[ray * 3 + 2];
    const float beta = dec.beta[0];
    const float* zrow = z_vals + (int64_t)ray * S;

    float trans_in = 1.0f;
    float acc_depth = 0.0f, acc_r = 0.0f, acc_g = 0.0f, acc_b = 0.0f;

    for (int c0 = 0; c0 < S; c0 += WAVE) {
        const int nvalid = min(WAVE, S - c0);
        const int nblk = (nvalid + 15) >> 4;

        float4_t out[2];
        const float zs = zrow[min(c0 + lane, S - 1)];
        auto block_point = [&](int b, float& px, float& py, float& pz) {
            const float zb = __shfl(zs, 16 * b + gp, WAVE);
            px = norm_coord(ox + dx * zb, bnd.lo[0], bnd.hi[0]);
            py = norm_coord(oy + dy * zb, bnd.lo[1], bnd.hi[1]);
            pz = norm_coord(oz + dz * zb, bnd.lo[2], bnd.hi[2]);
        };
        constexpr bool CHAIN = CL && !LOWP;
        PlaneTaps carry;
        float cx = 0.f, cy = 0.f, cz = 0.f;
        if (CHAIN) {
            block_point(0, cx, cy, cz);
            issue_plane0(planes, 0, cx, cy, cz, gq, opaque_zero(c0), carry);
        }
#pragma unroll
        for (int d = 0; d < 2; ++d) {
            out[d] = LOWP ? *(const float4_t*)(lp_biases(wlds, d) + 32) : *(const float4_t*)(wlds + d * DEC_LDS + DEC_B3);
#pragma unroll 1
            for (int b = 0; b < nblk; ++b) {
                const int oz0 = opaque_zero(b);
                const int sb = c0 + 16 * b + gp;
                float feat[16];
                if (CHAIN) {
                    const bool last = b + 1 == nblk;
                    float nx, ny, nz;
                    block_point(last ? 0 : b + 1, nx, ny, nz);
                    gather_features_chain(planes, d, cx, cy, cz, gq, feat, oz0, carry, last ? 1 : d, nx, ny, nz);
                    cx = nx; cy = ny; cz = nz;
                    if (SAVE) {
                        __builtin_amdgcn_sched_barrier(0);
                        store_features_buffer(frsrc, sb < S ? (unsigned)(ray * S + sb) * 512u + (unsigned)(d * 256 + gq * 16)
                                                            : ESLAM_OOB_OFFSET, feat);
                        __builtin_amdgcn_sched_barrier(0);
                    }
                    to_mfma_role<CL, 16>(feat, lane);
                    DecFrag f;
                    load_dec_frag(f, wlds + d * DEC_LDS + oz0, r, q);
                    float4_t h1, h2;
                    mlp_hidden(f, feat, h1, h2);
                    mlp_out_accum(f, h2, b, r, out[d]);
                    continue;
                }
                float px, py, pz;
                block_point(b, px, py, pz);
                if (LOWP) {
                    gather_features_half(planes, d, px, py, pz, gq, feat, oz0);
                    if (SAVE) {
                        if (sb < S) store_features_lp(feat_out, (int64_t)ray * S + sb, d, gq, feat);
                    }
                    to_mfma_role<true, 16>(feat, lane);
                    DecFragLP fl;
                    load_dec_frag_lp(fl, lp_weights(wlds, d) + oz0, lp_biases(wlds, d) + oz0, r, q);
                    float4_t a1, a2;
                    mlp_hidden_lp(fl, feat, a1, a2);
                    mlp_out_accum_lp(fl, a2, b, r, out[d]);
                    continue;
                }
                gather_features<CL>(planes, d, px, py, pz, gq, feat, oz0);
                if (SAVE) {
                    if (sb < S) store_features(feat_out, (int64_t)ray * S + sb, d, gq, feat);
                }
                to_mfma_role<CL, 16>(feat, lane);
                DecFrag f;
                load_dec_frag(f, wlds + d * DEC_LDS + oz0, r, q);
                float4_t h1, h2;
                mlp_hidden(f, feat, h1, h2);
                mlp_out_accum(f, h2, b, r, out[d]);
            }
        }

        const bool valid = lane < nvalid;
        const int s = c0 + lane;
        const float z = valid ? zs : 0.0f;
        const float sdf = tanhf(out[0][0]);
        const float cr = sigmoidf_(out[1][0]), cg = sigmoidf_(out[1][1]), cb = sigmoidf_(out[1][2]);
        if (valid) {
            sdf_out[(int64_t)ray * S + s] = sdf;
            if (SAVE) {
                float* rr = raw_rgb_out + ((int64_t)ray * S + s) * 3;
                rr[0] = cr; rr[1] = cg; rr[2] = cb;
            }
        }
        const float sg = sigmoidf_(-sdf * beta);
        float alpha = 1.0f - expf(-beta * sg);
        if (!valid) alpha = 0.0f;
        const float fac = valid ? (1.0f - alpha) + 1e-10f : 1.0f;
        const float pin = wave_incl_prod(fac, lane);
        const float pex = wave_up1(pin, 1.0f);
        const float w = alpha * (trans_in * pex);
        acc_depth += wave_sum(w * z);
        acc_r += wave_sum(w * cr);
        acc_g += wave_sum(w * cg);
        acc_b += wave_sum(w * cb);
        trans_in *= wave_lane<63>(pin);
        if (LOSS && valid && has_depth) {
            const int reg = sdf_region(z, gtd, li.tr);
            if (reg == 0) { lv[A_N_FRONT] += 1.0f; const float e = sdf - 1.0f; lv[A_S_FRONT] += e * e; }
            else if (reg == 1) { lv[A_N_CENTER] += 1.0f; const float e = (z + sdf * li.tr.t) - gtd; lv[A_S_CENTER] += e * e; }
            else if (reg == 2) { lv[A_N_TAIL] += 1.0f; const float e = (z + sdf * li.tr.t) - gtd; lv[A_S_TAIL] += e * e; }
        }
    }
    if (lane == 0) {
        depth_out[ray] = acc_depth;
        rgb_out[ray * 3 + 0] = acc_r;
        rgb_out[ray * 3 + 1] = acc_g;
        rgb_out[ray * 3 + 2] = acc_b;
        if (LOSS) {
            if (has_depth) { const float e = gtd - acc_depth; lv[A_N_DEPTH] += 1.0f; lv[A_S_DEPTH] += e * e; }
            if (in_batch) {
                const float er = li.gt_color[3 * ray] - acc_r, eg = li.gt_color[3 * ray + 1] - acc_g,
                            eb = li.gt_color[3 * ray + 2] - acc_b;
                lv[A_S_COLOR] += (er * er + eg * eg) + eb * eb;
                lv[A_N_COLOR] += 3.0f;
            }
        }
    }
    }
    if (LOSS) {
        __shared__ float red[4][A_COUNT];
// ... 149 lines not shown
                }
                to_mfma_role<CL, 16>(feat, lane);
                DecFrag f;
                load_dec_frag(f, wlds + d * DEC_LDS + oz0, r, q);
                float4_t h1, h2;
                mlp_hidden(f, feat, h1, h2);
                mlp_out_accum(f, h2, b, r, out[d]);
            }
        }
        bool keep = true;
        if (cls == TILE_TEST) {
            float x, y, z;
            src.point(tile, min(lane, nvalid - 1), x, y, z);
            keep = src.inside(tile, x, y, z);
        }
        if (lane < nvalid) {
            float sdf = tanhf(out[0][0]);
            if (mask_outside) {
                float x, y, z;
                src.point(tile, lane, x, y, z);
                const bool in = x < bnd.hi[0] && x > bnd.lo[0] && y < bnd.hi[1] && y > bnd.lo[1] && z < bnd.hi[2] &&
                                z > bnd.lo[2];
                if (!in) sdf = -1.0f;
            }
            if (!keep) sdf = -1.0f;
            if (SDF_ONLY) {
                raw[p0 + lane] = sdf;
            } else {
                float4_t v;
                v[0] = sigmoidf_(out[1][0]);
                v[1] = sigmoidf_(out[1][1]);
                v[2] = sigmoidf_(out[1][2]);
                v[3] = sdf;
                *(float4_t*)(raw + (p0 + lane) * 4) = v;
            }
        }
    }
}

bool eslam_planes_channels_last(const eslam_plane_t* planes, int first, int count);
int eslam_validate_planes(const eslam_plane_t* planes, int first, int count);
int eslam_planes_lowp(const eslam_plane_t* planes);
static Bound make_bound(const float* b6) {
    Bound b;
    for (int k = 0; k < 3; ++k) {
        b.lo[k] = b6[2 * k];
        b.hi[k] = b6[2 * k + 1];
    }
    return b;
}

static int render_fwd_common(const char* who, const eslam_plane_t* planes, const eslam_decoders_t* dec,
                             const float* bound6_host, const float* rays_o, const float* rays_d, const float* z_vals,
                             int R, int S, float* depth, float* rgb, float* sdf, float* raw_rgb, float* feat,
                             const int32_t* ray_order, const LossIn* li, uint32_t* rng_bump, eslam_stream_t stream) {
    if (R <= 0) return 0;
    if (S <= 0 || S > ESLAM_MAX_SAMPLES) {
        eslam_set_error("%s: S=%d outside [1,%d]", who, S, ESLAM_MAX_SAMPLES);
        return 1;
    }
    if (!planes || !dec || !bound6_host || !rays_o || !rays_d || !z_vals || !depth || !rgb || !sdf) {
        eslam_set_error("%s: null argument", who);
        return 1;
    }
    if ((raw_rgb == nullptr) != (feat == nullptr)) {
        eslam_set_error("%s: raw_rgb and feat must both be given or both be NULL", who);
        return 1;
    }
    if (eslam_validate_planes(planes, 0, NPL)) return 1;
    PlaneSet ps;
    for (int i = 0; i < NPL; ++i) ps.p[i] = planes[i];
    const Bound bnd = make_bound(bound6_host);
    const bool cl = eslam_planes_channels_last(planes, 0, NPL);
    const bool save = feat != nullptr;
    if (save && (int64_t)R * S * 512 >= ((int64_t)1 << 32) - 256) {
        eslam_set_error("%s: %lld points exceed the 32-bit offset range of the saved-feature buffer (8.3 M): split the batch", who,
                        (long long)R * S);
        return 1;
    }
    const int nblocks = (R + 3) / 4;
    static const int resident = [] {
        int dev = 0, cus = 256;
        if (hipGetDevice(&dev) == hipSuccess) (void)hipDeviceGetAttribute(&cus, hipDeviceAttributeMultiprocessorCount, dev);
        return ((FWD_WAVES * cus) / 8) * 8;
    }();
    int nwg = ((nblocks + 7) / 8) * 8;
    if (nwg > resident && nwg % resident == 0) nwg = resident;
    dim3 grid(nwg), block(256);
    hipStream_t st = (hipStream_t)stream;
    const LossIn none = {};
#define LAUNCH(CLv, SV, LS)                                                                                             \
    hipLaunchKernelGGL((render_fwd_kernel<CLv, SV, LS, false>), grid, block, 0, st, ps, *dec, bnd, rays_o, rays_d, z_vals, R, \
                       S, depth, rgb, sdf, raw_rgb, feat, (const int*)ray_order, LS ? *li : none, rng_bump)
#define LAUNCH_LP(SV, LS)                                                                                               \
    hipLaunchKernelGGL((render_fwd_kernel<true, SV, LS, true>), grid, block, 0, st, ps, *dec, bnd, rays_o, rays_d, z_vals, R, \
                       S, depth, rgb, sdf, raw_rgb, feat, (const int*)ray_order, LS ? *li : none, rng_bump)
    eslam_prof_begin(PROF_RENDER_FWD, st);
    const int lowp = eslam_planes_lowp(planes);
    if (lowp < 0) return 1;
    if (lowp) {
        if (li) { if (save) LAUNCH_LP(true, true); else LAUNCH_LP(false, true); }
        else { if (save) LAUNCH_LP(true, false); else LAUNCH_LP(false, false); }
    } else if (li) {
        if (cl && save) LAUNCH(true, true, true);
        else if (cl) LAUNCH(true, false, true);
        else if (save) LAUNCH(false, true, true);
        else LAUNCH(false, false, true);
    } else {
        if (cl && save) LAUNCH(true, true, false);
        else if (cl) LAUNCH(true, false, false);
        else if (save) LAUNCH(false, true, false);
        else LAUNCH(false, false, false);
    }
#undef LAUNCH
#undef LAUNCH_LP
    eslam_prof_end(PROF_RENDER_FWD, st);
    return eslam_check_launch("render_fwd_kernel");
}

extern "C" int eslam_render_fwd(const eslam_plane_t* planes, const eslam_decoders_t* dec, const float* bound6_host,
                                const float* rays_o, const float* rays_d, const float* z_vals, int R, int S,
                                float* depth, float* rgb, float* sdf, float* raw_rgb, float* feat,
                                const int32_t* ray_order, uint32_t* rng_bump, eslam_stream_t stream) {
    return render_fwd_common("eslam_render_fwd", planes, dec, bound6_host, rays_o, rays_d, z_vals, R, S, depth, rgb, sdf,
                             raw_rgb, feat, ray_order, nullptr, rng_bump, stream);
}

extern "C" int eslam_render_fwd_loss(const eslam_plane_t* planes, const eslam_decoders_t* dec, const float* bound6_host,
                                     const float* rays_o, const float* rays_d, const float* z_vals, int R, int S,
                                     float* depth, float* rgb, float* sdf, float* raw_rgb, float* feat,
                                     const int32_t* ray_order, const float* gt_depth, const float* gt_color,
                                     double truncation, const float* weights5_host, const uint8_t* ray_mask,
                                     float* scratch, float* acc, float* loss, uint32_t* rng_bump, eslam_stream_t stream) {
    if (!gt_depth || !gt_color || !weights5_host || !scratch || !acc) {
        eslam_set_error("eslam_render_fwd_loss: null loss argument");
        return 1;
    }
    if (R <= 0) {
        eslam_set_error("eslam_render_fwd_loss: empty batch");
        return 1;
    }
    LossIn li;
    li.gt_depth = gt_depth; li.gt_color = gt_color; li.ray_mask = ray_mask;
    li.scratch = scratch; li.acc = acc; li.loss = loss;
    li.det = eslam_deterministic();
    li.tr = make_trunc(truncation);
    li.w = LossW{weights5_host[0], weights5_host[1], weights5_host[2], weights5_host[3], weights5_host[4]};
    return render_fwd_common("eslam_render_fwd_loss", planes, dec, bound6_host, rays_o, rays_d, z_vals, R, S, depth, rgb,
                             sdf, raw_rgb, feat, ray_order, &li, rng_bump, stream);
}

extern "C" int eslam_decode_fwd(const eslam_plane_t* planes, const eslam_decoders_t* dec, const float* bound6_host,
                                const float* pts, int64_t N, int flags, float* raw, float* feat,
                                eslam_stream_t stream) {
    if (N <= 0) return 0;
    if (flags & ~(ESLAM_DECODE_SDF_ONLY | ESLAM_DECODE_MASK_OUTSIDE)) {
        eslam_set_error("eslam_decode_fwd: unknown flags 0x%x", flags);
        return 1;
    }
    const int sdf_only = flags & ESLAM_DECODE_SDF_ONLY;
    const int mask_outside = (flags & ESLAM_DECODE_MASK_OUTSIDE) ? 1 : 0;
    if (!planes || !dec || !bound6_host || !pts || !raw) {
        eslam_set_error("eslam_decode_fwd: null argument");
        return 1;
    }
    if (sdf_only && feat) {
        eslam_set_error("eslam_decode_fwd: feat cannot be saved in sdf_only mode");
        return 1;
    }
    if (eslam_validate_planes(planes, 0, sdf_only ? 6 : NPL)) return 1;
    PlaneSet ps;
    for (int i = 0; i < NPL; ++i) ps.p[i] = planes[sdf_only && i >= 6 ? i - 6 : i];
    const Bound bnd = make_bound(bound6_host);
    const bool cl = eslam_planes_channels_last(planes, 0, sdf_only ? 6 : NPL);
    const int64_t ntiles = (N + 63) / 64;
    const int64_t nwg = (ntiles + 3) / 4;
    dim3 grid((unsigned)(nwg < 8192 ? nwg : 8192)), block(256);
    hipStream_t st = (hipStream_t)stream;
    const PointList src{pts, N};
#define LAUNCH(CLv, SO, SV) \
    hipLaunchKernelGGL((decode_fwd_kernel<CLv, SO, SV, PointList>), grid, block, 0, st, ps, *dec, bnd, src, raw, feat, \
                       mask_outside)
#define LAUNCH_LP(SO, SV) \
    hipLaunchKernelGGL((decode_fwd_kernel<true, SO, SV, PointList, true>), grid, block, 0, st, ps, *dec, bnd, src, raw, feat, \
                       mask_outside)
    const int lowp = eslam_planes_lowp(ps.p);
    if (lowp < 0) return 1;
    eslam_prof_begin(PROF_DECODE_FWD, st);
    if (lowp) {
        if (sdf_only) LAUNCH_LP(true, false);
        else if (feat) LAUNCH_LP(false, true);
        else LAUNCH_LP(false, false);
    } else if (sdf_only) {
        if (cl) LAUNCH(true, true, false);
        else LAUNCH(false, true, false);
    } else if (feat) {
        if (cl) LAUNCH(true, false, true);
        else LAUNCH(false, false, true);
    } else {
        if (cl) LAUNCH(true, false, false);
        else LAUNCH(false, false, false);
    }
// ... 52 lines not shown
```

### myslam_amd/csrc/eslam_torch_ext.cpp

```cpp
#include <torch/extension.h>
#include <c10/hip/HIPGuard.h>
#include <c10/hip/HIPStream.h>
#include <hip/hip_runtime_api.h>

#include <cstdio>
#include <cstdlib>
#include <mutex>
#include <vector>

#include "../../include/eslam_hip.h"

namespace {

using torch::Tensor;
using torch::autograd::AutogradContext;
using torch::autograd::variable_list;

void check(int rc, const char* what) {
    TORCH_CHECK(rc == 0, what, " failed (rc=", rc, "): ", eslam_last_error());
}

struct Config {
    int64_t n_strat = 0, n_imp = 0;
    bool perturb = true;
// ... 30 lines not shown
    for (int i = 0; i < 12; ++i) {
        const Tensor& t = params[i];
        TORCH_CHECK(t.is_cuda() && t.scalar_type() == at::kFloat && t.is_contiguous(), "decoder parameter ", i, ": expected a contiguous float32 tensor on the GPU");
        const bool ok = shapes[i][1] ? (t.dim() == 2 && t.size(0) == shapes[i][0] && t.size(1) == shapes[i][1]) : (t.dim() == 1 && t.size(0) == shapes[i][0]);
        TORCH_CHECK(ok, "decoder parameter ", i, ": unexpected shape (c_dim=32, hidden=16, 2 blocks)");
        ptr[i] = t.data_ptr<float>();
    }
    TORCH_CHECK(beta.is_cuda() && beta.scalar_type() == at::kFloat && beta.numel() == 1, "beta: expected a float32 device tensor [1]");
    d->w1 = ptr[0]; d->b1 = ptr[1]; d->w2 = ptr[2]; d->b2 = ptr[3]; d->w3 = ptr[4]; d->b3 = ptr[5];
    d->cw1 = ptr[6]; d->cb1 = ptr[7]; d->cw2 = ptr[8]; d->cb2 = ptr[9]; d->cw3 = ptr[10]; d->cb3 = ptr[11];
    d->beta = beta.data_ptr<float>();
}

hipStream_t side_stream(int dev) {
    static std::mutex mu;
    static hipStream_t streams[64];
    TORCH_CHECK(dev >= 0 && dev < 64, "device index out of range");
    std::lock_guard<std::mutex> lk(mu);
    if (!streams[dev]) TORCH_CHECK(hipStreamCreateWithFlags(&streams[dev], hipStreamNonBlocking) == hipSuccess, "hipStreamCreate failed");
    return streams[dev];
}

struct LossArgs {
    Tensor gt_color, ray_mask, scratch, acc_out;
    std::vector<float> weights5;
};

enum class Layout { same, channels_last, nchw };
std::pair<Tensor, std::vector<Tensor>> alloc_plane_grads(const std::vector<Tensor>& planes, Layout layout = Layout::same) {
    int64_t total = 0;
    for (auto& p : planes) total += p.numel();
    Tensor flat = at::empty({total}, planes[0].options());
    std::vector<Tensor> views;
    views.reserve(12);
    int64_t off = 0;
    for (auto& p : planes) {
        TORCH_CHECK(p.is_contiguous() || p.is_contiguous(at::MemoryFormat::ChannelsLast), "planes must be dense (contiguous or channels_last)");
        const int64_t c = p.size(1), h = p.size(2), w = p.size(3);
        if (layout == Layout::same) views.push_back(at::as_strided(flat, p.sizes(), p.strides(), off));
        else if (layout == Layout::channels_last) views.push_back(at::as_strided(flat, p.sizes(), {c * h * w, 1, c * w, c}, off));
        else views.push_back(at::as_strided(flat, p.sizes(), {c * h * w, h * w, w, 1}, off));
        off += p.numel();
    }
    return {flat, views};
}

void relayout(const std::vector<Tensor>& src, const std::vector<Tensor>& dst, int field, hipStream_t st) {
    eslam_plane_t a[ESLAM_N_PLANES], b[ESLAM_N_PLANES];
    fill_planes(src, field ? &src : nullptr, a);
    fill_planes(dst, field ? &dst : nullptr, b);
    check(eslam_planes_relayout(a, b, field, st), "eslam_planes_relayout");
}

class RenderNode : public torch::autograd::Function<RenderNode> {
public:
    struct IO {
        Config cfg;
        Tensor gt_depth, t_free, t_surf, rng_state;
        uint64_t seed = 0;
        int64_t ray_offset = 0;
        LossArgs loss;
        bool needs = false, planes_grad = false;
        bool relayout = false;
    };

    static variable_list forward(AutogradContext* ctx, at::TensorList in, const IO& io) {
        const Tensor& rays_o_in = in[0];
        const Tensor& rays_d_in = in[1];
        const Tensor& beta = in[2];
        std::vector<Tensor> planes(in.begin() + 3, in.begin() + 15), params(in.begin() + 15, in.begin() + 27);
        TORCH_CHECK(rays_o_in.is_cuda() && rays_o_in.scalar_type() == at::kFloat, "rays_o: expected a float32 tensor on the GPU; the HIP render path has no CPU fallback");
        TORCH_CHECK(rays_d_in.is_cuda() && rays_d_in.scalar_type() == at::kFloat, "rays_d: expected a float32 tensor on the GPU");
        TORCH_CHECK(io.gt_depth.is_cuda() && io.gt_depth.scalar_type() == at::kFloat, "gt_depth: expected a float32 tensor on the GPU");
        const Tensor rays_o = rays_o_in.detach().contiguous(), rays_d = rays_d_in.detach().contiguous();
        const Tensor gd = io.gt_depth.detach().reshape({-1}).contiguous();
        const int64_t R = gd.size(0), S = io.cfg.n_strat + io.cfg.n_imp;
        TORCH_CHECK(rays_o.size(0) == R && rays_d.size(0) == R, "rays and gt_depth disagree on the number of rays");
        const int dev = rays_o.get_device();
        c10::hip::HIPGuard guard(dev);
        hipStream_t st = c10::hip::getCurrentHIPStream(dev).stream();
        const bool with_loss = io.loss.gt_color.defined();

        const bool needs = io.needs, planes_grad = io.planes_grad;
        auto opt = rays_o.options();
        Tensor z = at::empty({R, S}, opt), depth = at::empty({R}, opt), rgb = at::empty({R, 3}, opt), sdf = at::empty({R, S}, opt);
        Tensor raw_rgb, feat, perm, acc, value;
        if (needs) {
            raw_rgb = at::empty({R, S, 3}, opt);
            feat = at::empty({R * S, 128}, opt);
            perm = at::empty({planes_grad ? ESLAM_RAY_ORDER_WORDS(R) : 0}, opt.dtype(at::kInt));
        }
        if (io.relayout && R > 0) {
            auto cl = alloc_plane_grads(planes, Layout::channels_last);
            relayout(planes, cl.second, 0, st);
            planes = std::move(cl.second);
        }
        eslam_plane_t pd[ESLAM_N_PLANES];
        fill_planes(planes, nullptr, pd);
        eslam_decoders_t dd;
        fill_decoders(params, beta, &dd);

        std::vector<Tensor> grad_views;
        Tensor grad_flat;
        hipStream_t side = nullptr;
        if (planes_grad && R > 0) {
            side = side_stream(dev);
            auto gv = alloc_plane_grads(planes);
            grad_flat = gv.first;
            grad_views = std::move(gv.second);
            check(eslam_stream_wait(side, st), "eslam_stream_wait");
            check(eslam_zero_async(grad_flat.data_ptr<float>(), grad_flat.numel() * 4, side), "eslam_zero_async");
            check(eslam_ray_order(rays_o.data_ptr<float>(), rays_d.data_ptr<float>(), (int)R, perm.data_ptr<int32_t>(), side), "eslam_ray_order");
        }
        if (R > 0) {
            check(eslam_sample_z_all_rng(pd, &dd, io.cfg.bound_sample.data(), rays_o.data_ptr<float>(), rays_d.data_ptr<float>(),
                                         gd.data_ptr<float>(), (int)R, (int)io.cfg.n_strat, (int)io.cfg.n_imp, io.cfg.truncation,
                                         io.t_free.data_ptr<float>(), io.t_surf.data_ptr<float>(), io.cfg.perturb ? 1 : 0, io.seed,
                                         (const uint32_t*)io.rng_state.data_ptr<int32_t>(), io.ray_offset, z.data_ptr<float>(), st),
                  "eslam_sample_z_all_rng");
        }
        uint32_t* bump = (uint32_t*)io.rng_state.data_ptr<int32_t>();
        if (with_loss) {
            TORCH_CHECK(R > 0, "eslam_render_fwd_loss: empty batch");
            TORCH_CHECK(io.loss.gt_color.is_cuda() && io.loss.gt_color.scalar_type() == at::kFloat, "gt_color: expected a float32 tensor on the GPU");
            acc = io.loss.acc_out.defined() ? io.loss.acc_out : at::empty({16}, opt);
            value = at::empty({}, opt);
            const Tensor gc = io.loss.gt_color.contiguous();
            const uint8_t* mask = io.loss.ray_mask.defined() ? (const uint8_t*)io.loss.ray_mask.data_ptr() : nullptr;
            check(eslam_render_fwd_loss(pd, &dd, io.cfg.bound_decode.data(), rays_o.data_ptr<float>(), rays_d.data_ptr<float>(),
                                        z.data_ptr<float>(), (int)R, (int)S, depth.data_ptr<float>(), rgb.data_ptr<float>(),
                                        sdf.data_ptr<float>(), needs ? raw_rgb.data_ptr<float>() : nullptr,
                                        needs ? feat.data_ptr<float>() : nullptr, nullptr, gd.data_ptr<float>(), gc.data_ptr<float>(),
                                        io.cfg.truncation, io.loss.weights5.data(), mask, io.loss.scratch.data_ptr<float>(),
                                        acc.data_ptr<float>(), value.data_ptr<float>(), bump, st), "eslam_render_fwd_loss");
            ctx->saved_data["gt_color"] = gc;
            if (io.loss.ray_mask.defined()) ctx->saved_data["ray_mask"] = io.loss.ray_mask;
            ctx->saved_data["acc"] = acc;
            ctx->saved_data["w5"] = std::vector<double>(io.loss.weights5.begin(), io.loss.weights5.end());
        } else if (R > 0) {
            check(eslam_render_fwd(pd, &dd, io.cfg.bound_decode.data(), rays_o.data_ptr<float>(), rays_d.data_ptr<float>(), z.data_ptr<float>(),
                                   (int)R, (int)S, depth.data_ptr<float>(), rgb.data_ptr<float>(), sdf.data_ptr<float>(),
                                   needs ? raw_rgb.data_ptr<float>() : nullptr, needs ? feat.data_ptr<float>() : nullptr, nullptr, bump, st),
                  "eslam_render_fwd");
        }
        if (side) check(eslam_stream_wait(st, side), "eslam_stream_wait");
        if (needs) {
            variable_list saved = {rays_o, rays_d, z, sdf, raw_rgb, feat, perm, beta, depth, rgb, gd};
            saved.insert(saved.end(), planes.begin(), planes.end());
            saved.insert(saved.end(), params.begin(), params.end());
            ctx->save_for_backward(saved);
            ctx->saved_data["with_loss"] = with_loss;
            ctx->saved_data["relayout"] = io.relayout && R > 0;
            ctx->saved_data["truncation"] = io.cfg.truncation;
            ctx->saved_data["bound"] = std::vector<double>(io.cfg.bound_decode.begin(), io.cfg.bound_decode.end());
            if (planes_grad) ctx->saved_data["grad_views"] = grad_views;
        }
        ctx->set_materialize_grads(false);
        ctx->mark_non_differentiable({z});
        variable_list out = {depth, rgb, sdf, z};
        if (with_loss) {
            out.push_back(value);
            out.push_back(acc);
            ctx->mark_non_differentiable({acc});
        }
        return out;
    }

    static variable_list backward(AutogradContext* ctx, variable_list g) {
        auto saved = ctx->get_saved_variables();
        TORCH_CHECK(saved.size() == 35, "eslam_torch_ext: expected 35 saved tensors, got ", saved.size());
        const Tensor &rays_o = saved[0], &rays_d = saved[1], &z = saved[2], &sdf = saved[3], &raw_rgb = saved[4], &feat = saved[5],
                     &perm = saved[6], &beta = saved[7], &depth = saved[8], &rgb = saved[9], &gd = saved[10];
        std::vector<Tensor> planes(saved.begin() + 11, saved.begin() + 23), params(saved.begin() + 23, saved.begin() + 35);
        const int64_t R = z.size(0), S = z.size(1);
        const int dev = rays_o.get_device();
        c10::hip::HIPGuard guard(dev);
        hipStream_t st = c10::hip::getCurrentHIPStream(dev).stream();
        const bool with_loss = ctx->saved_data["with_loss"].toBool();
        const bool need_ro = ctx->needs_input_grad(0), need_rd = ctx->needs_input_grad(1), need_beta = ctx->needs_input_grad(2);
        bool need_planes = false, need_dec = false;
        for (int i = 0; i < 12; ++i) need_planes = need_planes || ctx->needs_input_grad(3 + i);
        for (int i = 0; i < 12; ++i) need_dec = need_dec || ctx->needs_input_grad(15 + i);
        const bool need_rays = need_ro || need_rd;
        auto opt = rays_o.options();
        std::vector<Tensor> grad_views;
        if (need_planes) {
            if (ctx->saved_data.count("grad_views")) {
                grad_views = ctx->saved_data["grad_views"].toTensorVector();
                ctx->saved_data.erase("grad_views");
            } else {
                auto gv = alloc_plane_grads(planes);
                gv.first.zero_();
                grad_views = std::move(gv.second);
            }
        }
        eslam_plane_t pd[ESLAM_N_PLANES];
        fill_planes(planes, need_planes ? &grad_views : nullptr, pd);
        eslam_decoders_t dd;
        fill_decoders(params, beta, &dd);
        Tensor g_dec = need_dec ? at::empty({ESLAM_N_DEC_PARAMS}, opt) : Tensor();
        Tensor g_beta = need_beta ? at::empty({1}, opt) : Tensor();
        Tensor g_ro = need_rays ? at::empty({R, 3}, opt) : Tensor(), g_rd = need_rays ? at::empty({R, 3}, opt) : Tensor();
        if (R == 0) {
            if (need_dec) g_dec.zero_();
            if (need_beta) g_beta.zero_();
        }
        Tensor ws = at::empty({eslam_bwd_workspace_bytes(R * S)}, opt.dtype(at::kByte));
        Tensor gdep = g[0].defined() ? g[0].contiguous() : Tensor(), grgb = g[1].defined() ? g[1].contiguous() : Tensor(),
               gsdf = g[2].defined() ? g[2].contiguous() : Tensor();
        auto bound_d = ctx->saved_data["bound"].toDoubleVector();
        float bound[6];
        for (int i = 0; i < 6; ++i) bound[i] = (float)bound_d[i];
        const double truncation = ctx->saved_data["truncation"].toDouble();
        const bool loss_grad = with_loss && g.size() > 4 && g[4].defined();
        if (loss_grad) {
            const Tensor up = g[4].detach().reshape({1}).to(at::kFloat).contiguous();
            const Tensor gc = ctx->saved_data["gt_color"].toTensor();
            const Tensor acc = ctx->saved_data["acc"].toTensor();
            const uint8_t* mask = ctx->saved_data.count("ray_mask") ? (const uint8_t*)ctx->saved_data["ray_mask"].toTensor().data_ptr() : nullptr;
            auto w5d = ctx->saved_data["w5"].toDoubleVector();
            float w5[5];
            for (int i = 0; i < 5; ++i) w5[i] = (float)w5d[i];
            check(eslam_render_bwd_loss(pd, &dd, bound, rays_o.data_ptr<float>(), rays_d.data_ptr<float>(), z.data_ptr<float>(), (int)R, (int)S,
                                        sdf.data_ptr<float>(), raw_rgb.data_ptr<float>(), feat.data_ptr<float>(), depth.data_ptr<float>(),
                                        rgb.data_ptr<float>(), gd.data_ptr<float>(), gc.data_ptr<float>(), truncation, w5, mask,
                                        acc.data_ptr<float>(), up.data_ptr<float>(), nullptr, gdep.defined() ? gdep.data_ptr<float>() : nullptr,
                                        grgb.defined() ? grgb.data_ptr<float>() : nullptr, gsdf.defined() ? gsdf.data_ptr<float>() : nullptr,
                                        need_dec ? g_dec.data_ptr<float>() : nullptr, need_beta ? g_beta.data_ptr<float>() : nullptr,
                                        need_rays ? g_ro.data_ptr<float>() : nullptr, need_rays ? g_rd.data_ptr<float>() : nullptr,
                                        perm.numel() ? perm.data_ptr<int32_t>() : nullptr, ws.data_ptr(), st), "eslam_render_bwd_loss");
        } else {
            check(eslam_render_bwd(pd, &dd, bound, rays_o.data_ptr<float>(), rays_d.data_ptr<float>(), z.data_ptr<float>(), (int)R, (int)S,
                                   sdf.data_ptr<float>(), raw_rgb.data_ptr<float>(), feat.data_ptr<float>(), gdep.defined() ? gdep.data_ptr<float>() : nullptr,
                                   grgb.defined() ? grgb.data_ptr<float>() : nullptr, gsdf.defined() ? gsdf.data_ptr<float>() : nullptr,
                                   need_dec ? g_dec.data_ptr<float>() : nullptr, need_beta ? g_beta.data_ptr<float>() : nullptr,
                                   need_rays ? g_ro.data_ptr<float>() : nullptr, need_rays ? g_rd.data_ptr<float>() : nullptr,
                                   perm.numel() ? perm.data_ptr<int32_t>() : nullptr, ws.data_ptr(), st), "eslam_render_bwd");
        }
        variable_list out(28);
        if (need_ro) out[0] = g_ro;
        if (need_rd) out[1] = g_rd;
        if (need_beta) out[2] = g_beta;
        if (need_planes && ctx->saved_data["relayout"].toBool()) {
            auto nchw = alloc_plane_grads(grad_views, Layout::nchw);
            relayout(grad_views, nchw.second, 1, st);
            grad_views = std::move(nchw.second);
        }
        for (int i = 0; i < 12; ++i)
            if (need_planes && ctx->needs_input_grad(3 + i)) out[3 + i] = grad_views[i];
        if (need_dec) {
            static const int64_t sizes[12] = {1024, 16, 256, 16, 16, 1, 1024, 16, 256, 16, 48, 3};
            int64_t off = 0;
            for (int i = 0; i < 12; ++i) {
                if (ctx->needs_input_grad(15 + i)) out[15 + i] = g_dec.narrow(0, off, sizes[i]).view(params[i].sizes());
                off += sizes[i];
            }
        }
        return out;
    }
};

class LossNode : public torch::autograd::Function<LossNode> {
public:
    struct IO {
        Tensor z, gt_depth, gt_color, ray_mask, scratch;
        double truncation = 0.0;
        std::vector<float> w5;
    };
    static Tensor forward(AutogradContext* ctx, const Tensor& depth_in, const Tensor& rgb_in, const Tensor& sdf_in, const IO& io) {
        for (const Tensor* t : {&depth_in, &rgb_in, &sdf_in, &io.z, &io.gt_depth, &io.gt_color})
            TORCH_CHECK(t->is_cuda() && t->scalar_type() == at::kFloat, "loss: expected float32 tensors on the GPU; the HIP render path has no CPU fallback");
        const Tensor depth = depth_in.detach().contiguous(), rgb = rgb_in.detach().contiguous(), sdf = sdf_in.detach().contiguous();
        const Tensor z = io.z.detach().contiguous(), gd = io.gt_depth.detach().contiguous(), gc = io.gt_color.detach().contiguous();
        const int64_t R = sdf.size(0), S = sdf.size(1);
        const int dev = sdf.get_device();
        c10::hip::HIPGuard guard(dev);
        hipStream_t st = c10::hip::getCurrentHIPStream(dev).stream();
        Tensor acc = at::empty({16}, sdf.options()), loss = at::empty({}, sdf.options());
        const uint8_t* mask = io.ray_mask.defined() ? (const uint8_t*)io.ray_mask.data_ptr() : nullptr;
        check(eslam_loss_value(depth.data_ptr<float>(), rgb.data_ptr<float>(), sdf.data_ptr<float>(), z.data_ptr<float>(), gd.data_ptr<float>(),
                               gc.data_ptr<float>(), (int)R, (int)S, io.truncation, io.w5.data(), mask, io.scratch.data_ptr<float>(),
                               acc.data_ptr<float>(), loss.data_ptr<float>(), st), "eslam_loss_value");
        ctx->save_for_backward({depth, rgb, sdf, z, gd, gc, acc});
        if (io.ray_mask.defined()) ctx->saved_data["ray_mask"] = io.ray_mask;
        ctx->saved_data["truncation"] = io.truncation;
        ctx->saved_data["w5"] = std::vector<double>(io.w5.begin(), io.w5.end());
        return loss;
    }
    static variable_list backward(AutogradContext* ctx, variable_list g) {
        auto sv = ctx->get_saved_variables();
        TORCH_CHECK(sv.size() == 7, "eslam_torch_ext: loss node lost its saved tensors");
        const Tensor &depth = sv[0], &rgb = sv[1], &sdf = sv[2], &z = sv[3], &gd = sv[4], &gc = sv[5], &acc = sv[6];
        const int64_t R = sdf.size(0), S = sdf.size(1);
        const int dev = sdf.get_device();
        c10::hip::HIPGuard guard(dev);
        hipStream_t st = c10::hip::getCurrentHIPStream(dev).stream();
        auto opt = sdf.options();
        Tensor g_depth = at::empty({R}, opt), g_rgb = at::empty({R, 3}, opt), g_sdf = at::empty({R, S}, opt);
        const Tensor up = g[0].detach().reshape({1}).to(at::kFloat).contiguous();
        auto w5d = ctx->saved_data["w5"].toDoubleVector();
        float w5[5];
        for (int i = 0; i < 5; ++i) w5[i] = (float)w5d[i];
        const uint8_t* mask = ctx->saved_data.count("ray_mask") ? (const uint8_t*)ctx->saved_data["ray_mask"].toTensor().data_ptr() : nullptr;
        check(eslam_loss_grad(depth.data_ptr<float>(), rgb.data_ptr<float>(), sdf.data_ptr<float>(), z.data_ptr<float>(), gd.data_ptr<float>(),
                              gc.data_ptr<float>(), (int)R, (int)S, ctx->saved_data["truncation"].toDouble(), w5, mask, acc.data_ptr<float>(),
                              nullptr, g_depth.data_ptr<float>(), g_rgb.data_ptr<float>(), g_sdf.data_ptr<float>(), up.data_ptr<float>(), st),
              "eslam_loss_grad");
        return {g_depth, g_rgb, g_sdf, Tensor()};
    }
};

Tensor mapping_loss(const Tensor& depth, const Tensor& rgb, const Tensor& sdf, const Tensor& z, const Tensor& gt_depth, const Tensor& gt_color,
                    double truncation, const std::vector<double>& weights5, const c10::optional<Tensor>& ray_mask, const Tensor& scratch) {
    TORCH_CHECK(weights5.size() == 5 && sdf.dim() == 2, "mapping_loss: 5 weights and sdf [R,S] expected");
    LossNode::IO io;
    io.z = z; io.gt_depth = gt_depth; io.gt_color = gt_color; io.scratch = scratch; io.truncation = truncation;
    io.w5.assign(weights5.begin(), weights5.end());
    if (ray_mask.has_value()) io.ray_mask = ray_mask->contiguous();
    return LossNode::apply(depth, rgb, sdf, io);
}

std::vector<Tensor> render(const Config& cfg, const Tensor& rays_o, const Tensor& rays_d, const Tensor& gt_depth, const Tensor& beta,
                           const std::vector<Tensor>& planes, const std::vector<Tensor>& params, const Tensor& t_free, const Tensor& t_surf,
                           const Tensor& rng_state, uint64_t seed, int64_t ray_offset, const c10::optional<Tensor>& gt_color,
                           const c10::optional<Tensor>& ray_mask, const c10::optional<Tensor>& scratch, const c10::optional<Tensor>& acc_out,
                           const std::vector<double>& weights5, bool relayout) {
    TORCH_CHECK(cfg.n_strat >= 3 && cfg.bound_sample.size() == 6 && cfg.bound_decode.size() == 6, "Config not initialised");
    TORCH_CHECK(planes.size() == 12 && params.size() == 12, "expected 12 planes and 12 decoder tensors");
    RenderNode::IO io;
    io.cfg = cfg;
    io.gt_depth = gt_depth; io.t_free = t_free; io.t_surf = t_surf; io.rng_state = rng_state;
    io.seed = seed; io.ray_offset = ray_offset; io.relayout = relayout;
    TORCH_CHECK(t_free.numel() == cfg.n_strat && t_surf.numel() == cfg.n_imp && rng_state.scalar_type() == at::kInt, "bad sampler tensors");
    if (gt_color.has_value()) {
        TORCH_CHECK(scratch.has_value() && weights5.size() == 5, "the fused loss needs its scratch and 5 weights");
        io.loss.gt_color = *gt_color;
        if (ray_mask.has_value()) io.loss.ray_mask = ray_mask->contiguous();
        io.loss.scratch = *scratch;
        if (acc_out.has_value()) io.loss.acc_out = *acc_out;
        io.loss.weights5.assign(weights5.begin(), weights5.end());
    }
    if (torch::GradMode::is_enabled()) {
        bool dec_grad = false;
        for (auto& p : planes) io.planes_grad = io.planes_grad || p.requires_grad();
        for (auto& p : params) dec_grad = dec_grad || p.requires_grad();
        io.needs = io.planes_grad || dec_grad || beta.requires_grad() || rays_o.requires_grad() || rays_d.requires_grad();
    }
    variable_list in;
    in.reserve(27);
    in.push_back(rays_o); in.push_back(rays_d); in.push_back(beta);
    in.insert(in.end(), planes.begin(), planes.end());
    in.insert(in.end(), params.begin(), params.end());
    return RenderNode::apply(at::TensorList(in), io);
}

}

PYBIND11_MODULE(TORCH_EXTENSION_NAME, m) {
    m.doc() = "compiled host glue of Renderer.render_batch_ray (see the header comment of eslam_torch_ext.cpp)";
    py::class_<Config>(m, "Config")
        .def(py::init([](int64_t n_strat, int64_t n_imp, bool perturb, double truncation, std::vector<float> bound_sample,
                         std::vector<float> bound_decode) {
            Config c;
            c.n_strat = n_strat; c.n_imp = n_imp; c.perturb = perturb; c.truncation = truncation;
            c.bound_sample = std::move(bound_sample); c.bound_decode = std::move(bound_decode);
            return c;
        }));
    m.def("render", &render, py::arg("cfg"), py::arg("rays_o"), py::arg("rays_d"), py::arg("gt_depth"), py::arg("beta"), py::arg("planes"),
          py::arg("params"), py::arg("t_free"), py::arg("t_surf"), py::arg("rng_state"), py::arg("seed"), py::arg("ray_offset"),
          py::arg("gt_color") = py::none(), py::arg("ray_mask") = py::none(), py::arg("scratch") = py::none(), py::arg("acc_out") = py::none(),
          py::arg("weights5") = std::vector<double>(), py::arg("relayout") = false);
    m.def("mapping_loss", &mapping_loss, py::arg("depth"), py::arg("rgb"), py::arg("sdf"), py::arg("z_vals"), py::arg("gt_depth"),
          py::arg("gt_color"), py::arg("truncation"), py::arg("weights5"), py::arg("ray_mask"), py::arg("scratch"));
    m.def("abi_version", []() { return eslam_abi_version(); });
}
```

### myslam_amd/ops.py

```python
import ctypes
import math
import os
import sys

import torch

from . import _hip

_const_cache = {}


def _cached(key, make):
    t = _const_cache.get(key)
    if t is None:
        t = make()
        _const_cache[key] = t
    return t


def beta_tensor(beta, device):
    if torch.is_tensor(beta):
        return beta
    dev = torch.device(device)
    return _cached(("beta", float(beta), dev.index), lambda: torch.full((1,), float(beta), device=dev))
# ... 168 lines not shown
        return False
    return all(p.is_cuda and p.dtype == torch.float32 and p.dim() == 4 and p.is_contiguous() for p in flat)


def planes_for_kernels(all_planes, n_points):
    if not wants_relayout(all_planes, n_points):
        return all_planes
    return _split_planes(ChannelsLastFn.apply(*[p for grp in all_planes for p in grp]))


_DEC_SIZES = [16 * 64, 16, 16 * 16, 16, 16, 1, 16 * 64, 16, 16 * 16, 16, 48, 3]


def _split_dec_grads(g_dec):
    parts = g_dec.split(_DEC_SIZES)
    return [t.view(shape) if len(shape) > 1 else t for t, (_, _, shape) in zip(parts, _hip.DEC_FIELDS)]


_dec_param_cache = {}


_side_streams = {}


def ray_order_async(rays_o, rays_d, grad_planes=None):
    _hip.require_gpu_f32("rays_o", rays_o)
    _hip.require_gpu_f32("rays_d", rays_d)
    dev = rays_o.device
    ro, rd = _c(rays_o.detach()), _c(rays_d.detach())
    R = ro.shape[0]
    side = _side_streams.get(dev.index)
    if side is None:
        side = _side_streams[dev.index] = torch.cuda.Stream(device=dev)
    perm = torch.empty(_hip.ray_order_words(R), dtype=torch.int32, device=dev)
    pre = None
    if grad_planes is not None and _grad_sink is None and not _keep_layout:
        pre = _alloc_plane_grads(grad_planes, zero=False)
    _hip.stream_wait(dev, side, None)
    with _hip.on_device(dev):
        if pre is not None:
            _hip.check(_hip.lib().eslam_zero_async(_hip.ptr(pre[0]), pre[0].numel() * 4, ctypes.c_void_p(side.cuda_stream)),
                       "eslam_zero_async")
        _hip.check(_hip.lib().eslam_ray_order(_hip.ptr(ro), _hip.ptr(rd), R, _hip.ptr(perm),
                                              ctypes.c_void_p(side.cuda_stream)), "eslam_ray_order")
    perm.record_stream(side)
    for t, src in ((ro, rays_o), (rd, rays_d)):
        if t.data_ptr() != src.data_ptr():
            t.record_stream(side)
    return (perm, side) if pre is None else (perm, side, pre[1])


_fused_loss = None

_EXT_WANTED = os.environ.get("ESLAM_TORCH_EXT", "1") != "0"
_ext_mod = False


def torch_ext():
    global _ext_mod
    if _ext_mod is False:
        _ext_mod = None
        path = os.path.join(os.path.dirname(_hip.LIB_PATH), "eslam_torch_ext.so")
        if _EXT_WANTED and os.path.exists(path) and not os.environ.get("ESLAM_HIP_LIB"):
            import importlib.util
            _hip.load_library()
            spec = importlib.util.spec_from_file_location("eslam_torch_ext", path)
            mod = importlib.util.module_from_spec(spec)
            spec.loader.exec_module(mod)
            if mod.abi_version() != _hip.ABI_VERSION:
                raise RuntimeError(f"eslam_torch_ext was built against ABI {mod.abi_version()}, the binding expects {_hip.ABI_VERSION}: "
                                   "run `make -C myslam_amd/csrc torch_ext`")
            _ext_mod = mod
    return _ext_mod


def ext_render_ok(rays_o, n_strat, rand):
    return (rand is None and _USE_KERNEL_RNG and n_strat >= 3 and _half_planes is None and _grad_sink is None and not _keep_layout and
            _rng_override is None and rays_o.is_cuda and torch_ext() is not None)


def ext_render(cfg, rays_o, rays_d, gt_depth, beta, flat_planes, dec_params, n_strat, n_imp, fl, relayout=False):
    dev = rays_o.device
    seed_v = _rng_seed(dev)
    state = _rng_state(dev)
    if _rng_pending.get(dev.index, False):
        state[0] += 1
        _rng_pending[dev.index] = False
    ext = torch_ext()
    with _hip.on_device(dev):
        if fl is None:
            outs = ext.render(cfg, rays_o, rays_d, gt_depth, beta, flat_planes, dec_params, linspace01(n_strat, dev), linspace01(n_imp, dev),
                              state, seed_v, _ray_offset, relayout=relayout)
        else:
            mask = fl.ray_mask
            if mask is not None:
                mask = _c(mask.view(torch.uint8) if mask.dtype == torch.bool else mask.to(torch.uint8))
            outs = ext.render(cfg, rays_o, rays_d, gt_depth, beta, flat_planes, dec_params, linspace01(n_strat, dev), linspace01(n_imp, dev),
                              state, seed_v, _ray_offset, fl.gt_color, mask, _loss_scratch(dev, rays_o.shape[0]), fl.acc_out,
                              list(fl.state.weights5), relayout)
            fl.loss, fl.acc = outs[4], outs[5]
            fl.value = outs[4].detach()
    return outs[0], outs[1], outs[2], outs[3]


class _LossState:
    __slots__ = ("truncation", "weights5", "rewrite_value", "gt_depth", "gt_color", "ray_mask", "acc", "value", "acc_global")

    def __init__(self, truncation, weights5, rewrite_value):
        self.truncation, self.weights5, self.rewrite_value = float(truncation), tuple(float(v) for v in weights5), rewrite_value
        self.gt_depth = self.gt_color = self.ray_mask = self.acc = self.value = self.acc_global = None


class fused_loss:

    def __init__(self, gt_depth, gt_color, truncation, weights5, ray_mask=None, rewrite_value=False, acc_out=None):
        self.gt_depth, self.gt_color, self.truncation, self.weights5, self.ray_mask = gt_depth, gt_color, truncation, weights5, ray_mask
        self.acc = self.value = self.loss = None
        self.acc_out = acc_out
        self.state = _LossState(truncation, weights5, rewrite_value)

    @property
    def acc_global(self):
        return self.state.acc_global

    @acc_global.setter
    def acc_global(self, t):
        self.state.acc_global = t

    def __enter__(self):
        global _fused_loss
        self._prev, _fused_loss = _fused_loss, self
        return self

    def __exit__(self, *a):
        global _fused_loss
        _fused_loss = self._prev


def current_fused_loss():
    return _fused_loss


_half_planes = None
_half_ray_grads = False
_half_points = False


class mixed_precision:

    def __init__(self, half, ray_grads=False, points=False):
        self.half = half
        self.ray_grads = bool(ray_grads)
# ... 105 lines not shown
    gd = _c(gt_depth.detach().reshape(-1))
    R = gd.shape[0]
    if ray_mask is not None:
        ray_mask = _c(ray_mask.view(torch.uint8) if ray_mask.dtype == torch.bool else ray_mask.to(torch.uint8))
    scratch = _pooled_scratch(dev, 7 * 32, "set_sizes")
    acc = torch.empty(16, device=dev) if out is None else out
    seed_v = 0 if t_rand is not None else _rng_seed(dev)
    if state is None:
        state = _rng_state(dev)
        if t_rand is None and _rng_pending.get(dev.index, False):
            state[0] += 1
            _rng_pending[dev.index] = False
    with _hip.on_device(dev):
        _hip.check(_hip.lib().eslam_loss_set_sizes(_hip.ptr(gd), _hip.ptr(ray_mask), R, n_strat, n_imp, float(truncation),
                                                  _hip.ptr(linspace01(n_strat, dev)), _hip.ptr(linspace01(n_imp, dev)),
                                                  _hip.ptr(None if t_rand is None else _c(t_rand)), 1 if perturb else 0, seed_v,
                                                  _hip.ptr(state), _hip.ptr(scratch), _hip.ptr(acc), _hip.stream_handle(dev)),
                   "eslam_loss_set_sizes")
    return acc


def _take_rng_bump(dev):
    if _rng_pending.pop(dev.index, False):
        return _hip.ptr(_rng_state(dev))
    return None


class RenderFn(torch.autograd.Function):

    N_LEAD = 7

    @staticmethod
    def forward(ctx, rays_o, rays_d, z_vals, bound6, beta, order_in, lossctx, *tensors):
        planes, params = tensors[:12], tensors[12:24]
        for n, t in (("rays_o", rays_o), ("rays_d", rays_d), ("z_vals", z_vals)):
            _hip.require_gpu_f32(n, t)
        rays_o, rays_d, z_vals = _c(rays_o.detach()), _c(rays_d.detach()), _c(z_vals.detach())
        R, S = z_vals.shape
        dev = rays_o.device
        lib = _hip.lib()
        half = None if _half_planes is None else list(_half_planes.flat)
        ctx.half = half
        arr, _ = _hip.make_planes(planes, half=half)
        dec, keep = _hip.make_decoders(params, beta)
        needs = any(ctx.needs_input_grad)
        if half is not None and not _half_ray_grads and (ctx.needs_input_grad[0] or ctx.needs_input_grad[1]):
            raise RuntimeError("mixed precision: gradients with respect to the rays (pose) are off; ask for them with "
                               "ops.mixed_precision(half, ray_grads=True) or detach the rays")
        depth = torch.empty(R, device=dev)
        rgb = torch.empty(R, 3, device=dev)
        sdf = torch.empty(R, S, device=dev)
        raw_rgb = torch.empty(R, S, 3, device=dev) if needs else None
        feat = torch.empty(R * S, 128, device=dev, dtype=torch.float32 if half is None else torch.bfloat16) if needs else None
        order = None
        ctx.pregrads = None
        if order_in is not None:
            order, side = order_in[0], order_in[1]
            if len(order_in) > 2 and needs:
                ctx.pregrads = order_in[2]
        fl = lossctx
        ctx.set_materialize_grads(False)
        ctx.lossctx = None
        with _hip.on_device(dev):
            if fl is None:
                _hip.check(lib.eslam_render_fwd(arr, ctypes.byref(dec), _hip.make_bound(bound6), _hip.ptr(rays_o),
                                                _hip.ptr(rays_d), _hip.ptr(z_vals), R, S, _hip.ptr(depth), _hip.ptr(rgb),
                                                _hip.ptr(sdf), _hip.ptr(raw_rgb), _hip.ptr(feat),
                                                None, _take_rng_bump(dev),
                                                _hip.stream_handle(dev)), "eslam_render_fwd")
            else:
                _hip.require_gpu_f32("gt_depth", fl.gt_depth)
                _hip.require_gpu_f32("gt_color", fl.gt_color)
                mask = fl.ray_mask
                if mask is not None:
                    mask = _c(mask.view(torch.uint8) if mask.dtype == torch.bool else mask.to(torch.uint8))
                fl.acc = torch.empty(16, device=dev) if getattr(fl, "acc_out", None) is None else fl.acc_out
                fl.value = torch.empty((), device=dev)
                st = fl.state
                st.gt_depth, st.gt_color, st.ray_mask, st.acc, st.value = _c(fl.gt_depth), _c(fl.gt_color), mask, fl.acc, fl.value
                w5 = (ctypes.c_float * 5)(*st.weights5)
                _hip.check(lib.eslam_render_fwd_loss(arr, ctypes.byref(dec), _hip.make_bound(bound6), _hip.ptr(rays_o),
                                                     _hip.ptr(rays_d), _hip.ptr(z_vals), R, S, _hip.ptr(depth),
                                                     _hip.ptr(rgb), _hip.ptr(sdf), _hip.ptr(raw_rgb), _hip.ptr(feat),
                                                     None,
                                                     _hip.ptr(st.gt_depth), _hip.ptr(st.gt_color),
                                                     st.truncation, w5, _hip.ptr(mask),
                                                     _hip.ptr(_loss_scratch(dev, R)), _hip.ptr(fl.acc), _hip.ptr(fl.value),
                                                     _take_rng_bump(dev), _hip.stream_handle(dev)), "eslam_render_fwd_loss")
                ctx.lossctx = st
        if order_in is not None and side is not None:
            _hip.stream_wait(dev, None, side)
        if needs:
            ctx.bound6 = bound6
            ctx.order_stream = None
            ctx.save_for_backward(rays_o, rays_d, z_vals, sdf, raw_rgb, feat, order, beta, depth, rgb, *planes, *params)
        if fl is not None:
            return depth, rgb, sdf, fl.value.detach()
        return depth, rgb, sdf

    @staticmethod
    def backward(ctx, g_depth, g_rgb, g_sdf, g_loss=None):
        saved = ctx.saved_tensors
        rays_o, rays_d, z_vals, sdf, raw_rgb, feat, order, beta, depth, rgb = saved[:10]
        planes, params = saved[10:22], saved[22:34]
        R, S = z_vals.shape
        dev = rays_o.device
        lib = _hip.lib()
        if getattr(ctx, "order_stream", None) is not None:
            _hip.stream_wait(dev, None, ctx.order_stream)
            ctx.order_stream = None
        need = ctx.needs_input_grad
        L = RenderFn.N_LEAD
        need_planes = any(need[L:L + 12])
        need_rays = need[0] or need[1]
        grads = None
        sink = _grad_sink
        if sink is not None:
            sink.zero_()
            grads = sink.views[:12]
        elif need_planes:
            grads = getattr(ctx, "pregrads", None)
            ctx.pregrads = None
            if grads is None:
                _, grads = _alloc_plane_grads(planes)
        arr, _ = _hip.make_planes(planes, grads, half=ctx.half)
        dec, keep = _hip.make_decoders(params, beta)
        if sink is not None:
            o = sink.offsets[12]
            g_dec = sink.flat[o:o + _hip.N_DEC_PARAMS]
            g_beta = sink.flat[sink.offsets[24]:sink.offsets[24] + 1] if len(sink.views) > 24 else \
                torch.empty(1, device=dev)
        else:
            need_dec = any(need[L + 12:L + 24])
            g_dec = torch.empty(_hip.N_DEC_PARAMS, device=dev) if need_dec else None
            g_beta = torch.empty(1, device=dev) if need[4] else None
        g_ro = torch.empty(R, 3, device=dev) if need_rays else None
        g_rd = torch.empty(R, 3, device=dev) if need_rays else None
        if R == 0:
            for t in (g_dec, g_beta):
                if t is not None:
                    t.zero_()
        ws = torch.empty(lib.eslam_bwd_workspace_bytes(R * S), dtype=torch.uint8, device=dev)
        g_depth, g_rgb, g_sdf = _c(g_depth), _c(g_rgb), _c(g_sdf)
        fl = ctx.lossctx
        with _hip.on_device(dev):
            if fl is not None and g_loss is not None:
                up = _c(g_loss.detach().reshape(1).to(torch.float32))
                w5 = (ctypes.c_float * 5)(*fl.weights5)
                _hip.check(lib.eslam_render_bwd_loss(
                    arr, ctypes.byref(dec), _hip.make_bound(ctx.bound6), _hip.ptr(rays_o), _hip.ptr(rays_d),
                    _hip.ptr(z_vals), R, S, _hip.ptr(sdf), _hip.ptr(raw_rgb), _hip.ptr(feat), _hip.ptr(depth), _hip.ptr(rgb),
                    _hip.ptr(fl.gt_depth), _hip.ptr(fl.gt_color), fl.truncation, w5, _hip.ptr(fl.ray_mask),
                    _hip.ptr(fl.acc if fl.acc_global is None else fl.acc_global), _hip.ptr(up), _hip.ptr(fl.value) if fl.rewrite_value else None, _hip.ptr(g_depth),
                    _hip.ptr(g_rgb), _hip.ptr(g_sdf), _hip.ptr(g_dec), _hip.ptr(g_beta), _hip.ptr(g_ro), _hip.ptr(g_rd),
                    _hip.ptr(order), _hip.ptr(ws), _hip.stream_handle(dev)), "eslam_render_bwd_loss")
            else:
                _hip.check(lib.eslam_render_bwd(arr, ctypes.byref(dec), _hip.make_bound(ctx.bound6), _hip.ptr(rays_o),
                                                _hip.ptr(rays_d), _hip.ptr(z_vals), R, S, _hip.ptr(sdf), _hip.ptr(raw_rgb),
                                                _hip.ptr(feat), _hip.ptr(g_depth), _hip.ptr(g_rgb), _hip.ptr(g_sdf),
                                                _hip.ptr(g_dec), _hip.ptr(g_beta), _hip.ptr(g_ro), _hip.ptr(g_rd),
                                                _hip.ptr(order), _hip.ptr(ws), _hip.stream_handle(dev)),
                           "eslam_render_bwd")
        if sink is not None:
            return (g_ro if need[0] else None, g_rd if need[1] else None) + (None,) * (L - 2 + 24)
        dec_grads = _split_dec_grads(g_dec) if g_dec is not None else [None] * 12
        out = [g_ro if need[0] else None, g_rd if need[1] else None, None, None, g_beta if need[4] else None, None, None]
        out += [grads[i] if (need_planes and need[L + i]) else None for i in range(12)]
        out += [dec_grads[i] if need[L + 12 + i] else None for i in range(12)]
        return tuple(out)


class DecodeFn(torch.autograd.Function):

    @staticmethod
    def forward(ctx, pts, bound6, dummy_beta, *tensors):
        planes, params = tensors[:12], tensors[12:24]
        _hip.require_gpu_f32("p", pts)
        pts = _c(pts.detach())
        N = pts.shape[0]
        dev = pts.device
        lib = _hip.lib()
        half = points_half()
        ctx.half = half
        arr, _ = _hip.make_planes(planes, half=half)
        dec, keep = _hip.make_decoders(params, dummy_beta)
        needs = any(ctx.needs_input_grad)
        raw = torch.empty(N, 4, device=dev)
        feat = torch.empty(N, 128, device=dev, dtype=torch.float32 if half is None else torch.bfloat16) if needs else None
        with _hip.on_device(dev):
            _hip.check(lib.eslam_decode_fwd(arr, ctypes.byref(dec), _hip.make_bound(bound6), _hip.ptr(pts), N, 0,
                                            _hip.ptr(raw), _hip.ptr(feat), _hip.stream_handle(dev)), "eslam_decode_fwd")
        if needs:
            ctx.bound6 = bound6
            ctx.save_for_backward(pts, raw, feat, dummy_beta, *planes, *params)
        return raw

    @staticmethod
    def backward(ctx, g_raw):
        saved = ctx.saved_tensors
        pts, raw, feat, dummy_beta = saved[:4]
        planes, params = saved[4:16], saved[16:28]
        N = pts.shape[0]
        dev = pts.device
        lib = _hip.lib()
        need = ctx.needs_input_grad
        need_planes = any(need[3:15])
        grads = None
        if need_planes:
            _, grads = _alloc_plane_grads(planes)
        arr, _ = _hip.make_planes(planes, grads, half=ctx.half)
        dec, keep = _hip.make_decoders(params, dummy_beta)
        g_dec = torch.empty(_hip.N_DEC_PARAMS, device=dev) if any(need[15:27]) else None
        g_pts = torch.empty(N, 3, device=dev) if need[0] else None
        ws = torch.empty(lib.eslam_bwd_workspace_bytes(N), dtype=torch.uint8, device=dev)
        g_raw = _c(g_raw)
        with _hip.on_device(dev):
            _hip.check(lib.eslam_decode_bwd(arr, ctypes.byref(dec), _hip.make_bound(ctx.bound6), _hip.ptr(pts), N,
                                            _hip.ptr(raw), _hip.ptr(feat), _hip.ptr(g_raw), _hip.ptr(g_dec),
                                            _hip.ptr(g_pts), _hip.ptr(ws), _hip.stream_handle(dev)), "eslam_decode_bwd")
        dec_grads = _split_dec_grads(g_dec) if g_dec is not None else [None] * 12
        out = [g_pts, None, None]
# ... 1004 lines not shown
```

### myslam_amd/src/utils/Renderer.py

```python
import torch

from ... import ops
from ..common import get_rays


class Renderer(object):
    def __init__(self, cfg, eslam, ray_batch_size=10000):
        self.ray_batch_size = ray_batch_size
        self.perturb = cfg['rendering']['perturb']
        self.n_stratified = cfg['rendering']['n_stratified']
        self.n_importance = cfg['rendering']['n_importance']
        self.scale = cfg['scale']
        self._bound6 = ops.bound_to_host(eslam.bound)
        self.bound = eslam.bound.to(eslam.device, non_blocking=True)
        self.H, self.W, self.fx, self.fy, self.cx, self.cy = eslam.H, eslam.W, eslam.fx, eslam.fy, eslam.cx, eslam.cy

    def render_batch_ray(self, all_planes, decoders, rays_d, rays_o, device, truncation, gt_depth=None, _rand=None):
        n_rays = rays_o.shape[0]
        S = self.n_stratified + self.n_importance
        if gt_depth is None:
            raise AttributeError("'NoneType' object has no attribute 'reshape'")
        if n_rays == 0:
            e = rays_o.new_empty
            return e(0), e(0, 3), e(0, S), e(0, S)
        beta = ops.beta_tensor(decoders.beta, rays_o.device)
        if ops.ext_render_ok(rays_o, self.n_stratified, _rand):
            return ops.ext_render(self._ext_cfg(truncation, decoders), rays_o, rays_d, gt_depth, beta,
                                  [p for grp in all_planes for p in grp], ops.decoder_params(decoders), self.n_stratified,
                                  self.n_importance, ops.current_fused_loss(), ops.wants_relayout(all_planes, n_rays * S))
        all_planes = ops.planes_for_kernels(all_planes, n_rays * S)
        flat_planes = [p for grp in all_planes for p in grp]
        grad_on = torch.is_grad_enabled()
        planes_grad = grad_on and any(p.requires_grad for p in flat_planes)
        wants_grad = planes_grad or (grad_on and (rays_o.requires_grad or rays_d.requires_grad or
                                                  any(p.requires_grad for p in ops.decoder_params(decoders)) or
                                                  (torch.is_tensor(decoders.beta) and decoders.beta.requires_grad)))
        order = ops.ray_order_async(rays_o, rays_d, flat_planes) if planes_grad else None
        z_vals = ops.sample_z(rays_o, rays_d, gt_depth, all_planes, decoders, self._bound6, truncation,
                              self.n_stratified, self.n_importance, self.perturb, _rand)
        bound6 = ops.bound_to_host(decoders.bound)
        fl = ops.current_fused_loss()
        outs = ops.RenderFn.apply(rays_o, rays_d, z_vals, bound6, beta, order, fl, *flat_planes,
                                  *ops.decoder_params(decoders))
        if fl is not None:
            fl.loss = outs[3]
        return outs[0], outs[1], outs[2], z_vals

    def _ext_cfg(self, truncation, decoders):
        b = decoders.bound
        key = (float(truncation), self.n_stratified, self.n_importance, bool(self.perturb), self._bound6, id(b),
               b._version if torch.is_tensor(b) else None)
        hit = self.__dict__.get("_ext_cfg_cache")
        if hit is None or hit[0] != key:
            cfg = ops.torch_ext().Config(self.n_stratified, self.n_importance, bool(self.perturb), float(truncation),
                                         list(self._bound6), list(ops.bound_to_host(b)))
            hit = self.__dict__["_ext_cfg_cache"] = (key, cfg)
        return hit[1]

    def __getstate__(self):
        d = dict(self.__dict__)
        d.pop("_ext_cfg_cache", None)
        return d

    def render_batch_ray_with_loss(self, all_planes, decoders, rays_d, rays_o, device, truncation, gt_depth, gt_color,
                                   weights, ray_mask=None, _rand=None, acc_out=None):
        with ops.fused_loss(gt_depth, gt_color, truncation, weights, ray_mask, acc_out=acc_out) as pre:
            depth, rgb, sdf, z_vals = self.render_batch_ray(all_planes, decoders, rays_d, rays_o, device, truncation,
                                                            gt_depth=gt_depth, _rand=_rand)
        return depth, rgb, sdf, z_vals, pre

    def sdf2alpha(self, sdf, beta=10):
        return 1. - torch.exp(-beta * torch.sigmoid(-sdf * beta))

    def render_img(self, all_planes, decoders, c2w, truncation, device, gt_depth=None, _rand_chunks=None):
        with torch.no_grad():
            H, W = self.H, self.W
            rays_o, rays_d = get_rays(H, W, self.fx, self.fy, self.cx, self.cy, c2w, device)
            rays_o = rays_o.reshape(-1, 3)
            rays_d = rays_d.reshape(-1, 3)
            gt_depth = gt_depth.reshape(-1)
            depth_list, color_list = [], []
            for k, i in enumerate(range(0, rays_d.shape[0], self.ray_batch_size)):
                ret = self.render_batch_ray(all_planes, decoders, rays_d[i:i + self.ray_batch_size],
                                            rays_o[i:i + self.ray_batch_size], device, truncation,
                                            gt_depth=gt_depth[i:i + self.ray_batch_size],
                                            _rand=None if _rand_chunks is None else _rand_chunks[k])
                depth_list.append(ret[0].double())
                color_list.append(ret[1])
            return torch.cat(depth_list, 0).reshape(H, W), torch.cat(color_list, 0).reshape(H, W, 3)
```

Before: 1.048 billion ray.samples/s.

## Save first-layer MLP hidden activations in forward and reuse them in backward

The forward render kernel now writes the first hidden layer (h1) of each decoder MLP into a saved buffer, and the backward MLP kernel loads it instead of reloading 64-float feature rows and recomputing the 16x64 first-layer matmul. When weight gradients are not needed, the feature-row loads are skipped entirely. This trades extra forward stores and backward loads of a per-sample hidden buffer (16 floats per decoder) for less feature traffic and compute, at the cost of more memory and new kernel template variants.

Measured after the change: 1.071 billion ray.samples/s (median of 6 runs). +2.2%, better.

```diff
diff --git a/include/eslam_hip.h b/include/eslam_hip.h
--- a/include/eslam_hip.h
+++ b/include/eslam_hip.h
@@ -111,6 +111,32 @@
                           const float* upstream, float* loss_out, const float* g_depth, const float* g_rgb,
                           const float* g_sdf, float* g_dec, float* g_beta, float* g_rays_o, float* g_rays_d,
                           const int32_t* ray_order, void* workspace, eslam_stream_t stream);
+
+int64_t eslam_saved_hidden_floats(int64_t R, int S);
+int eslam_render_fwd_h(const eslam_plane_t* planes, const eslam_decoders_t* dec, const float* bound6_host,
+                       const float* rays_o, const float* rays_d, const float* z_vals, int R, int S, float* depth,
+                       float* rgb, float* sdf, float* raw_rgb, float* feat, const int32_t* ray_order,
+                       uint32_t* rng_bump, float* hidden, eslam_stream_t stream);
+int eslam_render_fwd_loss_h(const eslam_plane_t* planes, const eslam_decoders_t* dec, const float* bound6_host,
+                            const float* rays_o, const float* rays_d, const float* z_vals, int R, int S, float* depth,
+                            float* rgb, float* sdf, float* raw_rgb, float* feat, const int32_t* ray_order,
+                            const float* gt_depth, const float* gt_color, double truncation, const float* weights5_host,
+                            const uint8_t* ray_mask, float* scratch, float* acc, float* loss, uint32_t* rng_bump,
+                            float* hidden, eslam_stream_t stream);
+int eslam_render_bwd_h(const eslam_plane_t* planes, const eslam_decoders_t* dec, const float* bound6_host,
+                       const float* rays_o, const float* rays_d, const float* z_vals, int R, int S,
+                       const float* sdf, const float* raw_rgb, const float* feat, const float* g_depth,
+                       const float* g_rgb, const float* g_sdf, float* g_dec, float* g_beta, float* g_rays_o,
+                       float* g_rays_d, const int32_t* ray_order, void* workspace, const float* hidden,
+                       eslam_stream_t stream);
+int eslam_render_bwd_loss_h(const eslam_plane_t* planes, const eslam_decoders_t* dec, const float* bound6_host,
+                            const float* rays_o, const float* rays_d, const float* z_vals, int R, int S,
+                            const float* sdf, const float* raw_rgb, const float* feat, const float* depth,
+                            const float* rgb, const float* gt_depth, const float* gt_color, double truncation,
+                            const float* weights5_host, const uint8_t* ray_mask, const float* acc,
+                            const float* upstream, float* loss_out, const float* g_depth, const float* g_rgb,
+                            const float* g_sdf, float* g_dec, float* g_beta, float* g_rays_o, float* g_rays_d,
+                            const int32_t* ray_order, void* workspace, const float* hidden, eslam_stream_t stream);
 
 #define ESLAM_DECODE_SDF_ONLY 1
 #define ESLAM_DECODE_MASK_OUTSIDE 2
@@ -269,6 +295,7 @@
 int eslam_deterministic(void);
 int eslam_scatter_bundle_samples(int64_t n, int S, int render);
 int eslam_last_backward_rank16(void);
+int eslam_last_backward_saved_hidden(void);
 
 int eslam_stream_wait(eslam_stream_t waiter, eslam_stream_t signaler);
 
diff --git a/myslam_amd/_hip.py b/myslam_amd/_hip.py
--- a/myslam_amd/_hip.py
+++ b/myslam_amd/_hip.py
@@ -91,6 +91,14 @@
                               _vp, _vp, _vp]),
     "eslam_render_bwd_loss": (_i, [_PP, _DP, _BP, _vp, _vp, _vp, _i, _i, _vp, _vp, _vp, _vp, _vp, _vp, _vp, _d, _BP, _vp, _vp,
                                    _vp, _vp, _vp, _vp, _vp, _vp, _vp, _vp, _vp, _vp, _vp, _vp]),
+    "eslam_saved_hidden_floats": (_i64, [_i64, _i]),
+    "eslam_render_fwd_h": (_i, [_PP, _DP, _BP, _vp, _vp, _vp, _i, _i, _vp, _vp, _vp, _vp, _vp, _vp, _vp, _vp, _vp]),
+    "eslam_render_fwd_loss_h": (_i, [_PP, _DP, _BP, _vp, _vp, _vp, _i, _i, _vp, _vp, _vp, _vp, _vp, _vp, _vp, _vp, _d, _BP, _vp,
+                                     _vp, _vp, _vp, _vp, _vp, _vp]),
+    "eslam_render_bwd_h": (_i, [_PP, _DP, _BP, _vp, _vp, _vp, _i, _i, _vp, _vp, _vp, _vp, _vp, _vp, _vp, _vp, _vp, _vp,
+                                _vp, _vp, _vp, _vp]),
+    "eslam_render_bwd_loss_h": (_i, [_PP, _DP, _BP, _vp, _vp, _vp, _i, _i, _vp, _vp, _vp, _vp, _vp, _vp, _vp, _d, _BP, _vp, _vp,
+                                     _vp, _vp, _vp, _vp, _vp, _vp, _vp, _vp, _vp, _vp, _vp, _vp, _vp]),
     "eslam_decode_fwd": (_i, [_PP, _DP, _BP, _vp, _i64, _i, _vp, _vp, _vp]),
     "eslam_sdf_grid": (_i, [_PP, _DP, _BP, _vp, _vp, _vp, _i64, _i64, _i64, _vp, _i, _i, _vp, _vp]),
     "eslam_mc_workspace_bytes": (_i64, [_i64, _i64, _i64]),
@@ -140,6 +148,7 @@
     "eslam_deterministic": (_i, []),
     "eslam_scatter_bundle_samples": (_i, [_i64, _i, _i]),
     "eslam_last_backward_rank16": (_i, []),
+    "eslam_last_backward_saved_hidden": (_i, []),
     "eslam_loss_scratch_floats": (_i64, [_i64]),
     "eslam_loss_scratch_reset": (_i, [_vp, _i64, _vp]),
     "eslam_loss_value": (_i, [_vp, _vp, _vp, _vp, _vp, _vp, _i, _i, _d, _BP, _vp, _vp, _vp, _vp, _vp]),
diff --git a/myslam_amd/csrc/eslam_decode_tile.h b/myslam_amd/csrc/eslam_decode_tile.h
--- a/myslam_amd/csrc/eslam_decode_tile.h
+++ b/myslam_amd/csrc/eslam_decode_tile.h
@@ -64,18 +64,24 @@
     f.b3 = *(const float4_t*)(L + DEC_B3);
 }
 
+__device__ __forceinline__ void mlp_hidden2(const DecFrag& f, const float4_t& h1, float4_t& h2) {
+    float4_t a2 = f.b2;
+#pragma unroll
+    for (int ks = 0; ks < 4; ++ks) a2 = mfma16(f.w2[ks], h1[ks], a2);
+#pragma unroll
+    for (int i = 0; i < 4; ++i) h2[i] = fmaxf(a2[i], 0.0f);
+}
+
 __device__ __forceinline__ void mlp_hidden(const DecFrag& f, const float feat[16], float4_t& h1, float4_t& h2) {
     float4_t a1 = f.b1;
 #pragma unroll
     for (int ks = 0; ks < 16; ++ks) a1 = mfma16(f.w1[ks], feat[ks], a1);
 #pragma unroll
     for (int i = 0; i < 4; ++i) h1[i] = fmaxf(a1[i], 0.0f);
-    float4_t a2 = f.b2;
-#pragma unroll
-    for (int ks = 0; ks < 4; ++ks) a2 = mfma16(f.w2[ks], h1[ks], a2);
-#pragma unroll
-    for (int i = 0; i < 4; ++i) h2[i] = fmaxf(a2[i], 0.0f);
-}
+    mlp_hidden2(f, h1, h2);
+}
+
+__device__ __forceinline__ int64_t hidden_blocks(int S) { return (S + 15) >> 4; }
 
 __device__ __forceinline__ void mlp_out_accum(const DecFrag& f, const float4_t& h2, int b, int r, float4_t& out) {
     const bool mine = (r >> 2) == b;
@@ -200,6 +206,10 @@
                                                rsrc, (int)byte_off + 64 * j, 0, 2);
 }
 
+__device__ __forceinline__ void store_hidden_buffer(__amdgpu_buffer_rsrc_t rsrc, unsigned byte_off, const float4_t& h1) {
+    __builtin_amdgcn_raw_buffer_store_b128(__builtin_bit_cast(uint4_bits, h1), rsrc, (int)byte_off, 0, 2);
+}
+
 __device__ __forceinline__ void load_features(const float* feat_in, int64_t pt, int d, int q, float feat[16]) {
     const float* src = feat_in + pt * 128 + d * 64 + 4 * q;
 #pragma unroll
diff --git a/myslam_amd/csrc/eslam_render_bwd.hip b/myslam_amd/csrc/eslam_render_bwd.hip
--- a/myslam_amd/csrc/eslam_render_bwd.hip
+++ b/myslam_amd/csrc/eslam_render_bwd.hip
@@ -68,11 +68,12 @@
     int R, S;
 };
 
-template <int MODE, bool WGRAD, bool LOWP, bool GZ = false>
+template <int MODE, bool WGRAD, bool LOWP, bool GZ = false, bool SAVEDH = false>
 __global__ __launch_bounds__(256, 2) void mlp_bwd_kernel(const eslam_decoders_t dec, const float* __restrict__ feat,
                                                       const float* __restrict__ g_o, int64_t N,
                                                       float* __restrict__ g_feat, float* __restrict__ slabs,
-                                                      const RayBwdIn rb, const LossGradIn li) {
+                                                      const RayBwdIn rb, const LossGradIn li,
+                                                      const float* __restrict__ hid) {
     __shared__ __attribute__((aligned(16))) float wlds[2 * DEC_LDS];
     __shared__ __attribute__((aligned(16))) float tiles[4][4][16 * TP];
     __shared__ __attribute__((aligned(16))) float gtile[4][64 * 4];
@@ -82,6 +83,8 @@
     __syncthreads();
 
     static_assert(!GZ || (!LOWP && MODE != 0), "GZ: float32 rays only");
+    static_assert(!SAVEDH || (!LOWP && MODE != 0), "SAVEDH: float32 rays only");
+    constexpr bool ROWS = !SAVEDH || WGRAD;
     const int d = blockIdx.y;
     const int nout = d ? 3 : 1;
     const float* L = wlds + d * DEC_LDS;
@@ -161,9 +164,13 @@
         v[3] = *(const float4_t*)(fp + 48);
     };
 #define TOUCH(x) asm volatile("" :: "v"(x))
-#define TOUCH_ROWS { TOUCH(fnext[0]); TOUCH(fnext[1]); TOUCH(fnext[2]); TOUCH(fnext[3]); }
+#define TOUCH_ROWS { if (ROWS) { TOUCH(fnext[0]); TOUCH(fnext[1]); TOUCH(fnext[2]); TOUCH(fnext[3]); } if (SAVEDH) TOUCH(hnext); }
     float4_t fnext[4];
-    auto tile_bwd = [&](const int64_t p0, const int nvalid, const float go[4], const int64_t p0_next) {
+    float4_t hnext = (float4_t){0.f, 0.f, 0.f, 0.f};
+    const int64_t hb_last = SAVEDH ? 2 * (int64_t)rb.R * hidden_blocks(rb.S) - 1 : 0;
+    auto load_hidden = [&](const int64_t hblk) { return *(const float4_t*)(hid + min(hblk, hb_last) * 256 + lane * 4); };
+    auto tile_bwd = [&](const int64_t p0, const int nvalid, const float go[4], const int64_t p0_next, const int64_t hb,
+                        const int64_t hb_next) {
         const int nblk = (nvalid + 15) >> 4;
         __builtin_assume(nblk >= 1);
 #pragma unroll
@@ -173,11 +180,15 @@
 #pragma unroll 1
         for (int b = 0; b < nblk; ++b) {
             float ft[16];
-#pragma unroll
-            for (int i = 0; i < 4; ++i) {
-                ft[i] = fnext[0][i]; ft[4 + i] = fnext[1][i]; ft[8 + i] = fnext[2][i]; ft[12 + i] = fnext[3][i];
-            }
-            load_block(0, fnext, b + 1 < nblk ? p0 + 16 * (b + 1) : p0_next);
+            if (ROWS) {
+#pragma unroll
+                for (int i = 0; i < 4; ++i) {
+                    ft[i] = fnext[0][i]; ft[4 + i] = fnext[1][i]; ft[8 + i] = fnext[2][i]; ft[12 + i] = fnext[3][i];
+                }
+            }
+            const float4_t hsaved = hnext;
+            if (ROWS) load_block(0, fnext, b + 1 < nblk ? p0 + 16 * (b + 1) : p0_next);
+            if (SAVEDH) hnext = load_hidden(b + 1 < nblk ? hb + b + 1 : hb_next);
             float4_t fbk[4];
             short4_t fbkp[4];
             if (WGRAD && LOWP) {
@@ -190,7 +201,7 @@
                 for (int j = 0; j < 4; ++j) *(float4_t*)(T + 16 * j) = (float4_t){ft[4 * j], ft[4 * j + 1], ft[4 * j + 2], ft[4 * j + 3]};
             }
             if (LOWP) to_mfma_role<true, 8>(ft, lane);
-            else to_mfma_role<true, 16>(ft, lane);
+            else if (!SAVEDH) to_mfma_role<true, 16>(ft, lane);
             float4_t h1, h2, gz1, gz2;
             const float4_t zero4 = (float4_t){0.f, 0.f, 0.f, 0.f};
             float gf[16];
@@ -228,7 +239,8 @@
                 to_gather_role<true, 16>(gf, lane);
                 store_rows(p0, b, nvalid, gf);
             } else {
-            mlp_hidden(f, ft, h1, h2);
+            if (SAVEDH) { h1 = hsaved; mlp_hidden2(f, h1, h2); }
+            else mlp_hidden(f, ft, h1, h2);
 
             float4_t gh2 = (float4_t){0.f, 0.f, 0.f, 0.f};
             const bool mine = (q == b);
@@ -326,11 +338,13 @@
                 else { go[0] = g[0]; go[1] = g[1]; go[2] = g[2]; }
             }
             TOUCH_ROWS
-            tile_bwd(p0, nvalid, go, (tile + (int64_t)gridDim.x * 4) * 64);
+            tile_bwd(p0, nvalid, go, (tile + (int64_t)gridDim.x * 4) * 64, 0, 0);
         }
     } else {
         const int R = rb.R, S = rb.S;
         const int nchunk = (S + WAVE - 1) / WAVE;
+        const int64_t SB = hidden_blocks(S);
+        auto hidden_block = [&](int ray_, int c_) { return ((int64_t)d * R + ray_) * SB + 4 * c_; };
         __builtin_assume(nchunk >= 1);
         const float beta = rb.beta[0];
         LossW lw = {};
@@ -394,7 +408,8 @@
             rin = load_ray(ray);
             cin = load_chunk(ray, nchunk - 1);
             pin = load_pa(ray);
-            load_block(0, fnext, (int64_t)ray * S + (nchunk - 1) * WAVE);
+            if (ROWS) load_block(0, fnext, (int64_t)ray * S + (nchunk - 1) * WAVE);
+            if (SAVEDH) hnext = load_hidden(hidden_block(ray, nchunk - 1));
         }
         dropped_stores();
 #define TOUCH_CHUNK(ci) { TOUCH(ci.sd); TOUCH(ci.z); TOUCH(ci.cr); TOUCH(ci.cg); TOUCH(ci.cb); TOUCH(ci.gs); }
@@ -448,7 +463,8 @@
                 if (d == 0) go[0] = o[3];
                 else { go[0] = o[0]; go[1] = o[1]; go[2] = o[2]; }
                 tile_bwd(base + c * WAVE, min(WAVE, S - c * WAVE), go,
-                         c > 0 ? base + (c - 1) * WAVE : (int64_t)(ray + stride) * S + (nchunk - 1) * WAVE);
+                         c > 0 ? base + (c - 1) * WAVE : (int64_t)(ray + stride) * S + (nchunk - 1) * WAVE, hidden_block(ray, c),
+                         c > 0 ? hidden_block(ray, c - 1) : hidden_block(ray + stride, nchunk - 1));
                 if (c > 0) {
                     TOUCH_CHUNK(cn)
                     TOUCH_ROWS
@@ -791,11 +807,13 @@
 
 static int g_last_backward_rank16 = 0;
 extern "C" int eslam_last_backward_rank16(void) { return g_last_backward_rank16; }
+static int g_last_backward_saved_hidden = 0;
+extern "C" int eslam_last_backward_saved_hidden(void) { return g_last_backward_saved_hidden; }
 
 static int bwd_common(const eslam_plane_t* planes, const eslam_decoders_t* dec, const Bound& bnd, const float* rays_o,
                       const float* rays_d, const float* z_or_pts, int64_t R, int S, int mode, const float* feat,
                       float* g_o, float* g_feat, float* slabs, const int* perm, float* g_dec, float* g_out_a, float* g_out_b,
-                      RayBwdIn rb, const LossGradIn* li, float* g_beta, hipStream_t st) {
+                      RayBwdIn rb, const LossGradIn* li, float* g_beta, const float* hid, hipStream_t st) {
     const bool render = mode != 0;
     const int64_t N = render ? R * S : R;
     PlaneSet ps;
@@ -815,7 +833,7 @@
     eslam_prof_begin(PROF_MLP_BWD, st);
 #define LAUNCH_MB(MD, WG, LP, ...) \
     hipLaunchKernelGGL((mlp_bwd_kernel<MD, WG, LP, ##__VA_ARGS__>), dim3(nwg, 2), dim3(256), 0, st, *dec, feat, g_o, N, g_feat, slabs, rb, \
-                       li ? *li : none)
+                       li ? *li : none, hid)
     const int lowp = eslam_planes_lowp(planes);
     if (lowp < 0) return 1;
     bool any_grad = false, all_grad = true;
@@ -829,7 +847,17 @@
     }
     const bool gz = !lowp && render && any_grad && !g_out_a && !eslam_deterministic();
     g_last_backward_rank16 = gz ? 1 : 0;
-    if (gz) {
+    if (lowp || !render) hid = nullptr;
+    g_last_backward_saved_hidden = hid ? 1 : 0;
+    if (hid) {
+        if (gz) {
+            if (mode == 1) { if (g_dec) LAUNCH_MB(1, true, false, true, true); else LAUNCH_MB(1, false, false, true, true); }
+            else { if (g_dec) LAUNCH_MB(2, true, false, true, true); else LAUNCH_MB(2, false, false, true, true); }
+        }
+        else if (mode == 1) { if (g_dec) LAUNCH_MB(1, true, false, false, true); else LAUNCH_MB(1, false, false, false, true); }
+        else { if (g_dec) LAUNCH_MB(2, true, false, false, true); else LAUNCH_MB(2, false, false, false, true); }
+    }
+    else if (gz) {
         if (mode == 1) { if (g_dec) LAUNCH_MB(1, true, false, true); else LAUNCH_MB(1, false, false, true); }
         else { if (g_dec) LAUNCH_MB(2, true, false, true); else LAUNCH_MB(2, false, false, true); }
     }
@@ -894,7 +922,7 @@
                            const float* bound6_host, const float* rays_o, const float* rays_d, const float* z_vals, int R,
                            int S, const float* sdf, const float* raw_rgb, const float* feat, const float* g_depth,
                            const float* g_rgb, const float* g_sdf, const LossGradIn* li, float* g_dec, float* g_beta,
-                           float* g_rays_o, float* g_rays_d, const int32_t* ray_order, void* workspace,
+                           float* g_rays_o, float* g_rays_d, const int32_t* ray_order, void* workspace, const float* hid,
                            eslam_stream_t stream) {
     if (R <= 0) return 0;
     if (S <= 0 || S > ESLAM_MAX_SAMPLES) {
@@ -933,7 +961,17 @@
     rb.z_vals = z_vals; rb.sdf = sdf; rb.raw_rgb = raw_rgb; rb.beta = dec->beta;
     rb.g_depth = g_depth; rb.g_rgb = g_rgb; rb.g_sdf = g_sdf; rb.R = R; rb.S = S;
     return bwd_common(planes, dec, bnd, rays_o, rays_d, z_vals, R, S, li ? 2 : 1, feat, g_o, g_feat, slabs, perm, g_dec,
-                      g_rays_o, g_rays_d, rb, li, g_beta, st);
+                      g_rays_o, g_rays_d, rb, li, g_beta, hid, st);
+}
+
+extern "C" int eslam_render_bwd_h(const eslam_plane_t* planes, const eslam_decoders_t* dec, const float* bound6_host,
+                                  const float* rays_o, const float* rays_d, const float* z_vals, int R, int S,
+                                  const float* sdf, const float* raw_rgb, const float* feat, const float* g_depth,
+                                  const float* g_rgb, const float* g_sdf, float* g_dec, float* g_beta, float* g_rays_o,
+                                  float* g_rays_d, const int32_t* ray_order, void* workspace, const float* hidden,
+                                  eslam_stream_t stream) {
+    return render_bwd_impl("eslam_render_bwd", planes, dec, bound6_host, rays_o, rays_d, z_vals, R, S, sdf, raw_rgb, feat,
+                           g_depth, g_rgb, g_sdf, nullptr, g_dec, g_beta, g_rays_o, g_rays_d, ray_order, workspace, hidden, stream);
 }
 
 extern "C" int eslam_render_bwd(const eslam_plane_t* planes, const eslam_decoders_t* dec, const float* bound6_host,
@@ -941,8 +979,30 @@
                                 const float* sdf, const float* raw_rgb, const float* feat, const float* g_depth,
                                 const float* g_rgb, const float* g_sdf, float* g_dec, float* g_beta, float* g_rays_o,
                                 float* g_rays_d, const int32_t* ray_order, void* workspace, eslam_stream_t stream) {
-    return render_bwd_impl("eslam_render_bwd", planes, dec, bound6_host, rays_o, rays_d, z_vals, R, S, sdf, raw_rgb, feat,
-                           g_depth, g_rgb, g_sdf, nullptr, g_dec, g_beta, g_rays_o, g_rays_d, ray_order, workspace, stream);
+    return eslam_render_bwd_h(planes, dec, bound6_host, rays_o, rays_d, z_vals, R, S, sdf, raw_rgb, feat, g_depth, g_rgb, g_sdf,
+                              g_dec, g_beta, g_rays_o, g_rays_d, ray_order, workspace, nullptr, stream);
+}
+
+extern "C" int eslam_render_bwd_loss_h(const eslam_plane_t* planes, const eslam_decoders_t* dec, const float* bound6_host,
+                                       const float* rays_o, const float* rays_d, const float* z_vals, int R, int S,
+                                       const float* sdf, const float* raw_rgb, const float* feat, const float* depth,
+                                       const float* rgb, const float* gt_depth, const float* gt_color, double truncation,
+                                       const float* weights5_host, const uint8_t* ray_mask, const float* acc,
+                                       const float* upstream, float* loss_out, const float* g_depth, const float* g_rgb,
+                                       const float* g_sdf, float* g_dec, float* g_beta, float* g_rays_o, float* g_rays_d,
+                                       const int32_t* ray_order, void* workspace, const float* hidden,
+                                       eslam_stream_t stream) {
+    if (!depth || !rgb || !gt_depth || !gt_color || !weights5_host || !acc) {
+        eslam_set_error("eslam_render_bwd_loss: null loss argument");
+        return 1;
+    }
+    LossGradIn li = {};
+    li.gt_depth = gt_depth; li.gt_color = gt_color; li.ray_mask = ray_mask; li.depth = depth; li.rgb = rgb;
+    li.acc = acc; li.upstream = upstream; li.loss_out = loss_out;
+    li.tr = make_trunc(truncation);
+    li.w = LossW{weights5_host[0], weights5_host[1], weights5_host[2], weights5_host[3], weights5_host[4]};
+    return render_bwd_impl("eslam_render_bwd_loss", planes, dec, bound6_host, rays_o, rays_d, z_vals, R, S, sdf, raw_rgb,
+                           feat, g_depth, g_rgb, g_sdf, &li, g_dec, g_beta, g_rays_o, g_rays_d, ray_order, workspace, hidden, stream);
 }
 
 extern "C" int eslam_render_bwd_loss(const eslam_plane_t* planes, const eslam_decoders_t* dec, const float* bound6_host,
@@ -953,17 +1013,9 @@
                                      const float* upstream, float* loss_out, const float* g_depth, const float* g_rgb,
                                      const float* g_sdf, float* g_dec, float* g_beta, float* g_rays_o, float* g_rays_d,
                                      const int32_t* ray_order, void* workspace, eslam_stream_t stream) {
-    if (!depth || !rgb || !gt_depth || !gt_color || !weights5_host || !acc) {
-        eslam_set_error("eslam_render_bwd_loss: null loss argument");
-        return 1;
-    }
-    LossGradIn li = {};
-    li.gt_depth = gt_depth; li.gt_color = gt_color; li.ray_mask = ray_mask; li.depth = depth; li.rgb = rgb;
-    li.acc = acc; li.upstream = upstream; li.loss_out = loss_out;
-    li.tr = make_trunc(truncation);
-    li.w = LossW{weights5_host[0], weights5_host[1], weights5_host[2], weights5_host[3], weights5_host[4]};
-    return render_bwd_impl("eslam_render_bwd_loss", planes, dec, bound6_host, rays_o, rays_d, z_vals, R, S, sdf, raw_rgb,
-                           feat, g_depth, g_rgb, g_sdf, &li, g_dec, g_beta, g_rays_o, g_rays_d, ray_order, workspace, stream);
+    return eslam_render_bwd_loss_h(planes, dec, bound6_host, rays_o, rays_d, z_vals, R, S, sdf, raw_rgb, feat, depth, rgb, gt_depth,
+                                   gt_color, truncation, weights5_host, ray_mask, acc, upstream, loss_out, g_depth, g_rgb, g_sdf,
+                                   g_dec, g_beta, g_rays_o, g_rays_d, ray_order, workspace, nullptr, stream);
 }
 
 extern "C" int eslam_decode_bwd(const eslam_plane_t* planes, const eslam_decoders_t* dec, const float* bound6_host,
@@ -988,5 +1040,5 @@
     hipLaunchKernelGGL(decode_act_bwd_kernel, dim3((unsigned)((N + 255) / 256)), dim3(256), 0, st, raw, g_raw, N, g_o);
     if (int rc = eslam_check_launch("decode_act_bwd_kernel")) return rc;
     return bwd_common(planes, dec, bnd, nullptr, nullptr, pts, N, 64, 0, feat, g_o, g_feat, slabs, nullptr, g_dec,
-                      g_pts, nullptr, RayBwdIn{}, nullptr, nullptr, st);
-}
+                      g_pts, nullptr, RayBwdIn{}, nullptr, nullptr, nullptr, st);
+}
diff --git a/myslam_amd/csrc/eslam_render_fwd.hip b/myslam_amd/csrc/eslam_render_fwd.hip
--- a/myslam_amd/csrc/eslam_render_fwd.hip
+++ b/myslam_amd/csrc/eslam_render_fwd.hip
@@ -24,8 +24,9 @@
                                                          const float* __restrict__ z_vals, int R, int S,
                                                          float* __restrict__ depth_out, float* __restrict__ rgb_out,
                                                          float* __restrict__ sdf_out, float* __restrict__ raw_rgb_out,
-                                                         float* __restrict__ feat_out, const int* __restrict__ perm,
-                                                         const LossIn li, uint32_t* __restrict__ rng_bump) {
+                                                         float* __restrict__ feat_out, float* __restrict__ hid_out,
+                                                         const int* __restrict__ perm, const LossIn li,
+                                                         uint32_t* __restrict__ rng_bump) {
     if (rng_bump && blockIdx.x == 0 && threadIdx.x == 0) rng_bump[0] += 1u;
     __shared__ __attribute__((aligned(16))) float wlds[2 * DEC_LDS];
     static_assert(LP_LDS_FLOATS <= 2 * DEC_LDS, "the bf16 weight image shares the float32 image's LDS");
@@ -38,6 +39,8 @@
     const int r = lane & 15, q = lane >> 4;
     const int gp = gather_point<CL>(lane), gq = gather_piece<CL>(lane);
     const __amdgpu_buffer_rsrc_t frsrc = __builtin_amdgcn_make_buffer_rsrc((void*)feat_out, 0, (int)((unsigned)R * (unsigned)S * 512u), 0x00020000);
+    const int SB = (int)hidden_blocks(S);
+    const __amdgpu_buffer_rsrc_t hrsrc = __builtin_amdgcn_make_buffer_rsrc((void*)hid_out, 0, hid_out ? (int)(2u * (unsigned)R * (unsigned)SB * 1024u) : 0, 0x00020000);
     float lv[A_COUNT];
 #pragma unroll
     for (int k = 0; k < A_COUNT; ++k) lv[k] = 0.0f;
@@ -102,6 +105,7 @@
                     load_dec_frag(f, wlds + d * DEC_LDS + oz0, r, q);
                     float4_t h1, h2;
                     mlp_hidden(f, feat, h1, h2);
+                    if (SAVE) store_hidden_buffer(hrsrc, (unsigned)((d * R + ray) * SB + (c0 >> 4) + b) * 1024u + (unsigned)lane * 16u, h1);
                     mlp_out_accum(f, h2, b, r, out[d]);
                     continue;
                 }
@@ -129,6 +133,7 @@
                 load_dec_frag(f, wlds + d * DEC_LDS + oz0, r, q);
                 float4_t h1, h2;
                 mlp_hidden(f, feat, h1, h2);
+                if (SAVE) store_hidden_buffer(hrsrc, (unsigned)((d * R + ray) * SB + (c0 >> 4) + b) * 1024u + (unsigned)lane * 16u, h1);
                 mlp_out_accum(f, h2, b, r, out[d]);
             }
         }
@@ -384,7 +389,7 @@
 
 static int render_fwd_common(const char* who, const eslam_plane_t* planes, const eslam_decoders_t* dec,
                              const float* bound6_host, const float* rays_o, const float* rays_d, const float* z_vals,
-                             int R, int S, float* depth, float* rgb, float* sdf, float* raw_rgb, float* feat,
+                             int R, int S, float* depth, float* rgb, float* sdf, float* raw_rgb, float* feat, float* hid,
                              const int32_t* ray_order, const LossIn* li, uint32_t* rng_bump, eslam_stream_t stream) {
     if (R <= 0) return 0;
     if (S <= 0 || S > ESLAM_MAX_SAMPLES) {
@@ -397,6 +402,15 @@
     }
     if ((raw_rgb == nullptr) != (feat == nullptr)) {
         eslam_set_error("%s: raw_rgb and feat must both be given or both be NULL", who);
+        return 1;
+    }
+    if (hid && !feat) {
+        eslam_set_error("%s: the hidden layer is saved beside the features: feat is NULL", who);
+        return 1;
+    }
+    if (hid && eslam_saved_hidden_floats(R, S) * 4 >= ((int64_t)1 << 32) - 256) {
+        eslam_set_error("%s: %lld rays of %d samples exceed the 32-bit offset range of the saved hidden layer: split the batch", who,
+                        (long long)R, S);
         return 1;
     }
     if (eslam_validate_planes(planes, 0, NPL)) return 1;
@@ -421,15 +435,16 @@
     dim3 grid(nwg), block(256);
     hipStream_t st = (hipStream_t)stream;
     const LossIn none = {};
+    const int lowp = eslam_planes_lowp(planes);
+    if (lowp < 0) return 1;
+    float* hidp = lowp ? nullptr : hid;
 #define LAUNCH(CLv, SV, LS)                                                                                             \
     hipLaunchKernelGGL((render_fwd_kernel<CLv, SV, LS, false>), grid, block, 0, st, ps, *dec, bnd, rays_o, rays_d, z_vals, R, \
-                       S, depth, rgb, sdf, raw_rgb, feat, (const int*)ray_order, LS ? *li : none, rng_bump)
+                       S, depth, rgb, sdf, raw_rgb, feat, hidp, (const int*)ray_order, LS ? *li : none, rng_bump)
 #define LAUNCH_LP(SV, LS)                                                                                               \
     hipLaunchKernelGGL((render_fwd_kernel<true, SV, LS, true>), grid, block, 0, st, ps, *dec, bnd, rays_o, rays_d, z_vals, R, \
-                       S, depth, rgb, sdf, raw_rgb, feat, (const int*)ray_order, LS ? *li : none, rng_bump)
+                       S, depth, rgb, sdf, raw_rgb, feat, hidp, (const int*)ray_order, LS ? *li : none, rng_bump)
     eslam_prof_begin(PROF_RENDER_FWD, st);
-    const int lowp = eslam_planes_lowp(planes);
-    if (lowp < 0) return 1;
     if (lowp) {
         if (li) { if (save) LAUNCH_LP(true, true); else LAUNCH_LP(false, true); }
         else { if (save) LAUNCH_LP(true, false); else LAUNCH_LP(false, false); }
@@ -450,20 +465,34 @@
     return eslam_check_launch("render_fwd_kernel");
 }
 
+extern "C" int64_t eslam_saved_hidden_floats(int64_t R, int S) {
+    if (R < 0 || S < 0) return -1;
+    return 2 * R * (((int64_t)S + 15) >> 4) * 256;
+}
+
+extern "C" int eslam_render_fwd_h(const eslam_plane_t* planes, const eslam_decoders_t* dec, const float* bound6_host,
+                                  const float* rays_o, const float* rays_d, const float* z_vals, int R, int S,
+                                  float* depth, float* rgb, float* sdf, float* raw_rgb, float* feat,
+                                  const int32_t* ray_order, uint32_t* rng_bump, float* hidden, eslam_stream_t stream) {
+    return render_fwd_common("eslam_render_fwd", planes, dec, bound6_host, rays_o, rays_d, z_vals, R, S, depth, rgb, sdf,
+                             raw_rgb, feat, hidden, ray_order, nullptr, rng_bump, stream);
+}
+
 extern "C" int eslam_render_fwd(const eslam_plane_t* planes, const eslam_decoders_t* dec, const float* bound6_host,
                                 const float* rays_o, const float* rays_d, const float* z_vals, int R, int S,
                                 float* depth, float* rgb, float* sdf, float* raw_rgb, float* feat,
                                 const int32_t* ray_order, uint32_t* rng_bump, eslam_stream_t stream) {
-    return render_fwd_common("eslam_render_fwd", planes, dec, bound6_host, rays_o, rays_d, z_vals, R, S, depth, rgb, sdf,
-                             raw_rgb, feat, ray_order, nullptr, rng_bump, stream);
-}
-
-extern "C" int eslam_render_fwd_loss(const eslam_plane_t* planes, const eslam_decoders_t* dec, const float* bound6_host,
-                                     const float* rays_o, const float* rays_d, const float* z_vals, int R, int S,
-                                     float* depth, float* rgb, float* sdf, float* raw_rgb, float* feat,
-                                     const int32_t* ray_order, const float* gt_depth, const float* gt_color,
-                                     double truncation, const float* weights5_host, const uint8_t* ray_mask,
-                                     float* scratch, float* acc, float* loss, uint32_t* rng_bump, eslam_stream_t stream) {
+    return eslam_render_fwd_h(planes, dec, bound6_host, rays_o, rays_d, z_vals, R, S, depth, rgb, sdf, raw_rgb, feat, ray_order,
+                              rng_bump, nullptr, stream);
+}
+
+extern "C" int eslam_render_fwd_loss_h(const eslam_plane_t* planes, const eslam_decoders_t* dec, const float* bound6_host,
+                                       const float* rays_o, const float* rays_d, const float* z_vals, int R, int S,
+                                       float* depth, float* rgb, float* sdf, float* raw_rgb, float* feat,
+                                       const int32_t* ray_order, const float* gt_depth, const float* gt_color,
+                                       double truncation, const float* weights5_host, const uint8_t* ray_mask,
+                                       float* scratch, float* acc, float* loss, uint32_t* rng_bump, float* hidden,
+                                       eslam_stream_t stream) {
     if (!gt_depth || !gt_color || !weights5_host || !scratch || !acc) {
         eslam_set_error("eslam_render_fwd_loss: null loss argument");
         return 1;
@@ -479,7 +508,18 @@
     li.tr = make_trunc(truncation);
     li.w = LossW{weights5_host[0], weights5_host[1], weights5_host[2], weights5_host[3], weights5_host[4]};
     return render_fwd_common("eslam_render_fwd_loss", planes, dec, bound6_host, rays_o, rays_d, z_vals, R, S, depth, rgb,
-                             sdf, raw_rgb, feat, ray_order, &li, rng_bump, stream);
+                             sdf, raw_rgb, feat, hidden, ray_order, &li, rng_bump, stream);
+}
+
+extern "C" int eslam_render_fwd_loss(const eslam_plane_t* planes, const eslam_decoders_t* dec, const float* bound6_host,
+                                     const float* rays_o, const float* rays_d, const float* z_vals, int R, int S,
+                                     float* depth, float* rgb, float* sdf, float* raw_rgb, float* feat,
+                                     const int32_t* ray_order, const float* gt_depth, const float* gt_color,
+                                     double truncation, const float* weights5_host, const uint8_t* ray_mask,
+                                     float* scratch, float* acc, float* loss, uint32_t* rng_bump, eslam_stream_t stream) {
+    return eslam_render_fwd_loss_h(planes, dec, bound6_host, rays_o, rays_d, z_vals, R, S, depth, rgb, sdf, raw_rgb, feat, ray_order,
+                                   gt_depth, gt_color, truncation, weights5_host, ray_mask, scratch, acc, loss, rng_bump, nullptr,
+                                   stream);
 }
 
 extern "C" int eslam_decode_fwd(const eslam_plane_t* planes, const eslam_decoders_t* dec, const float* bound6_host,
diff --git a/myslam_amd/csrc/eslam_torch_ext.cpp b/myslam_amd/csrc/eslam_torch_ext.cpp
--- a/myslam_amd/csrc/eslam_torch_ext.cpp
+++ b/myslam_amd/csrc/eslam_torch_ext.cpp
@@ -106,6 +106,13 @@
     check(eslam_planes_relayout(a, b, field, st), "eslam_planes_relayout");
 }
 
+const float* require_saved_hidden(const Tensor& h, int64_t R, int64_t S) {
+    const int64_t want = eslam_saved_hidden_floats(R, (int)S);
+    TORCH_CHECK(h.defined() && h.scalar_type() == at::kFloat && h.is_contiguous() && h.numel() >= want,
+                "saved hidden layer: ", h.defined() ? h.numel() : 0, " elements, ", want, " contiguous float32 needed for ", R, " x ", S, " samples");
+    return h.data_ptr<float>();
+}
+
 class RenderNode : public torch::autograd::Function<RenderNode> {
 public:
     struct IO {
@@ -116,6 +123,7 @@
         LossArgs loss;
         bool needs = false, planes_grad = false;
         bool relayout = false;
+        bool saved_hidden = true;
     };
 
     static variable_list forward(AutogradContext* ctx, at::TensorList in, const IO& io) {
@@ -138,10 +146,11 @@
         const bool needs = io.needs, planes_grad = io.planes_grad;
         auto opt = rays_o.options();
         Tensor z = at::empty({R, S}, opt), depth = at::empty({R}, opt), rgb = at::empty({R, 3}, opt), sdf = at::empty({R, S}, opt);
-        Tensor raw_rgb, feat, perm, acc, value;
+        Tensor raw_rgb, feat, hid, perm, acc, value;
         if (needs) {
             raw_rgb = at::empty({R, S, 3}, opt);
             feat = at::empty({R * S, 128}, opt);
+            if (io.saved_hidden && R > 0) hid = at::empty({eslam_saved_hidden_floats(R, (int)S)}, opt);
             perm = at::empty({planes_grad ? ESLAM_RAY_ORDER_WORDS(R) : 0}, opt.dtype(at::kInt));
         }
         if (io.relayout && R > 0) {
@@ -181,20 +190,22 @@
             value = at::empty({}, opt);
             const Tensor gc = io.loss.gt_color.contiguous();
             const uint8_t* mask = io.loss.ray_mask.defined() ? (const uint8_t*)io.loss.ray_mask.data_ptr() : nullptr;
-            check(eslam_render_fwd_loss(pd, &dd, io.cfg.bound_decode.data(), rays_o.data_ptr<float>(), rays_d.data_ptr<float>(),
+            check(eslam_render_fwd_loss_h(pd, &dd, io.cfg.bound_decode.data(), rays_o.data_ptr<float>(), rays_d.data_ptr<float>(),
                                         z.data_ptr<float>(), (int)R, (int)S, depth.data_ptr<float>(), rgb.data_ptr<float>(),
                                         sdf.data_ptr<float>(), needs ? raw_rgb.data_ptr<float>() : nullptr,
                                         needs ? feat.data_ptr<float>() : nullptr, nullptr, gd.data_ptr<float>(), gc.data_ptr<float>(),
                                         io.cfg.truncation, io.loss.weights5.data(), mask, io.loss.scratch.data_ptr<float>(),
-                                        acc.data_ptr<float>(), value.data_ptr<float>(), bump, st), "eslam_render_fwd_loss");
+                                        acc.data_ptr<float>(), value.data_ptr<float>(), bump, hid.defined() ? hid.data_ptr<float>() : nullptr, st),
+                  "eslam_render_fwd_loss");
             ctx->saved_data["gt_color"] = gc;
             if (io.loss.ray_mask.defined()) ctx->saved_data["ray_mask"] = io.loss.ray_mask;
             ctx->saved_data["acc"] = acc;
             ctx->saved_data["w5"] = std::vector<double>(io.loss.weights5.begin(), io.loss.weights5.end());
         } else if (R > 0) {
-            check(eslam_render_fwd(pd, &dd, io.cfg.bound_decode.data(), rays_o.data_ptr<float>(), rays_d.data_ptr<float>(), z.data_ptr<float>(),
+            check(eslam_render_fwd_h(pd, &dd, io.cfg.bound_decode.data(), rays_o.data_ptr<float>(), rays_d.data_ptr<float>(), z.data_ptr<float>(),
                                    (int)R, (int)S, depth.data_ptr<float>(), rgb.data_ptr<float>(), sdf.data_ptr<float>(),
-                                   needs ? raw_rgb.data_ptr<float>() : nullptr, needs ? feat.data_ptr<float>() : nullptr, nullptr, bump, st),
+                                   needs ? raw_rgb.data_ptr<float>() : nullptr, needs ? feat.data_ptr<float>() : nullptr, nullptr, bump,
+                                   hid.defined() ? hid.data_ptr<float>() : nullptr, st),
                   "eslam_render_fwd");
         }
         if (side) check(eslam_stream_wait(st, side), "eslam_stream_wait");
@@ -202,7 +213,9 @@
             variable_list saved = {rays_o, rays_d, z, sdf, raw_rgb, feat, perm, beta, depth, rgb, gd};
             saved.insert(saved.end(), planes.begin(), planes.end());
             saved.insert(saved.end(), params.begin(), params.end());
+            if (hid.defined()) saved.push_back(hid);
             ctx->save_for_backward(saved);
+            ctx->saved_data["saved_hidden"] = hid.defined();
             ctx->saved_data["with_loss"] = with_loss;
             ctx->saved_data["relayout"] = io.relayout && R > 0;
             ctx->saved_data["truncation"] = io.cfg.truncation;
@@ -222,11 +235,13 @@
 
     static variable_list backward(AutogradContext* ctx, variable_list g) {
         auto saved = ctx->get_saved_variables();
-        TORCH_CHECK(saved.size() == 35, "eslam_torch_ext: expected 35 saved tensors, got ", saved.size());
+        const bool saved_hidden = ctx->saved_data["saved_hidden"].toBool();
+        TORCH_CHECK(saved.size() == (saved_hidden ? 36u : 35u), "eslam_torch_ext: expected ", saved_hidden ? 36 : 35, " saved tensors, got ", saved.size());
         const Tensor &rays_o = saved[0], &rays_d = saved[1], &z = saved[2], &sdf = saved[3], &raw_rgb = saved[4], &feat = saved[5],
                      &perm = saved[6], &beta = saved[7], &depth = saved[8], &rgb = saved[9], &gd = saved[10];
         std::vector<Tensor> planes(saved.begin() + 11, saved.begin() + 23), params(saved.begin() + 23, saved.begin() + 35);
         const int64_t R = z.size(0), S = z.size(1);
+        const float* hid = saved_hidden ? require_saved_hidden(saved[35], R, S) : nullptr;
         const int dev = rays_o.get_device();
         c10::hip::HIPGuard guard(dev);
         hipStream_t st = c10::hip::getCurrentHIPStream(dev).stream();
@@ -275,21 +290,21 @@
             auto w5d = ctx->saved_data["w5"].toDoubleVector();
             float w5[5];
             for (int i = 0; i < 5; ++i) w5[i] = (float)w5d[i];
-            check(eslam_render_bwd_loss(pd, &dd, bound, rays_o.data_ptr<float>(), rays_d.data_ptr<float>(), z.data_ptr<float>(), (int)R, (int)S,
+            check(eslam_render_bwd_loss_h(pd, &dd, bound, rays_o.data_ptr<float>(), rays_d.data_ptr<float>(), z.data_ptr<float>(), (int)R, (int)S,
                                         sdf.data_ptr<float>(), raw_rgb.data_ptr<float>(), feat.data_ptr<float>(), depth.data_ptr<float>(),
                                         rgb.data_ptr<float>(), gd.data_ptr<float>(), gc.data_ptr<float>(), truncation, w5, mask,
                                         acc.data_ptr<float>(), up.data_ptr<float>(), nullptr, gdep.defined() ? gdep.data_ptr<float>() : nullptr,
                                         grgb.defined() ? grgb.data_ptr<float>() : nullptr, gsdf.defined() ? gsdf.data_ptr<float>() : nullptr,
                                         need_dec ? g_dec.data_ptr<float>() : nullptr, need_beta ? g_beta.data_ptr<float>() : nullptr,
                                         need_rays ? g_ro.data_ptr<float>() : nullptr, need_rays ? g_rd.data_ptr<float>() : nullptr,
-                                        perm.numel() ? perm.data_ptr<int32_t>() : nullptr, ws.data_ptr(), st), "eslam_render_bwd_loss");
+                                        perm.numel() ? perm.data_ptr<int32_t>() : nullptr, ws.data_ptr(), hid, st), "eslam_render_bwd_loss");
         } else {
-            check(eslam_render_bwd(pd, &dd, bound, rays_o.data_ptr<float>(), rays_d.data_ptr<float>(), z.data_ptr<float>(), (int)R, (int)S,
+            check(eslam_render_bwd_h(pd, &dd, bound, rays_o.data_ptr<float>(), rays_d.data_ptr<float>(), z.data_ptr<float>(), (int)R, (int)S,
                                    sdf.data_ptr<float>(), raw_rgb.data_ptr<float>(), feat.data_ptr<float>(), gdep.defined() ? gdep.data_ptr<float>() : nullptr,
                                    grgb.defined() ? grgb.data_ptr<float>() : nullptr, gsdf.defined() ? gsdf.data_ptr<float>() : nullptr,
                                    need_dec ? g_dec.data_ptr<float>() : nullptr, need_beta ? g_beta.data_ptr<float>() : nullptr,
                                    need_rays ? g_ro.data_ptr<float>() : nullptr, need_rays ? g_rd.data_ptr<float>() : nullptr,
-                                   perm.numel() ? perm.data_ptr<int32_t>() : nullptr, ws.data_ptr(), st), "eslam_render_bwd");
+                                   perm.numel() ? perm.data_ptr<int32_t>() : nullptr, ws.data_ptr(), hid, st), "eslam_render_bwd");
         }
         variable_list out(28);
         if (need_ro) out[0] = g_ro;
@@ -378,13 +393,13 @@
                            const std::vector<Tensor>& planes, const std::vector<Tensor>& params, const Tensor& t_free, const Tensor& t_surf,
                            const Tensor& rng_state, uint64_t seed, int64_t ray_offset, const c10::optional<Tensor>& gt_color,
                            const c10::optional<Tensor>& ray_mask, const c10::optional<Tensor>& scratch, const c10::optional<Tensor>& acc_out,
-                           const std::vector<double>& weights5, bool relayout) {
+                           const std::vector<double>& weights5, bool relayout, bool saved_hidden) {
     TORCH_CHECK(cfg.n_strat >= 3 && cfg.bound_sample.size() == 6 && cfg.bound_decode.size() == 6, "Config not initialised");
     TORCH_CHECK(planes.size() == 12 && params.size() == 12, "expected 12 planes and 12 decoder tensors");
     RenderNode::IO io;
     io.cfg = cfg;
     io.gt_depth = gt_depth; io.t_free = t_free; io.t_surf = t_surf; io.rng_state = rng_state;
-    io.seed = seed; io.ray_offset = ray_offset; io.relayout = relayout;
+    io.seed = seed; io.ray_offset = ray_offset; io.relayout = relayout; io.saved_hidden = saved_hidden;
     TORCH_CHECK(t_free.numel() == cfg.n_strat && t_surf.numel() == cfg.n_imp && rng_state.scalar_type() == at::kInt, "bad sampler tensors");
     if (gt_color.has_value()) {
         TORCH_CHECK(scratch.has_value() && weights5.size() == 5, "the fused loss needs its scratch and 5 weights");
@@ -423,8 +438,11 @@
     m.def("render", &render, py::arg("cfg"), py::arg("rays_o"), py::arg("rays_d"), py::arg("gt_depth"), py::arg("beta"), py::arg("planes"),
           py::arg("params"), py::arg("t_free"), py::arg("t_surf"), py::arg("rng_state"), py::arg("seed"), py::arg("ray_offset"),
           py::arg("gt_color") = py::none(), py::arg("ray_mask") = py::none(), py::arg("scratch") = py::none(), py::arg("acc_out") = py::none(),
-          py::arg("weights5") = std::vector<double>(), py::arg("relayout") = false);
+          py::arg("weights5") = std::vector<double>(), py::arg("relayout") = false, py::arg("saved_hidden") = true);
     m.def("mapping_loss", &mapping_loss, py::arg("depth"), py::arg("rgb"), py::arg("sdf"), py::arg("z_vals"), py::arg("gt_depth"),
           py::arg("gt_color"), py::arg("truncation"), py::arg("weights5"), py::arg("ray_mask"), py::arg("scratch"));
     m.def("abi_version", []() { return eslam_abi_version(); });
-}
+    m.def("require_saved_hidden", [](const c10::optional<Tensor>& h, int64_t R, int64_t S) {
+        require_saved_hidden(h.has_value() ? *h : Tensor(), R, S);
+    }, py::arg("hidden"), py::arg("R"), py::arg("S"), "the check RenderNode's backward makes on its saved hidden layer before its first launch");
+}
diff --git a/myslam_amd/ops.py b/myslam_amd/ops.py
--- a/myslam_amd/ops.py
+++ b/myslam_amd/ops.py
@@ -244,6 +244,44 @@
 
 _fused_loss = None
 
+SAVED_HIDDEN_DEFAULT = True
+_saved_hidden = None
+
+
+class saved_hidden:
+
+    def __init__(self, on):
+        self.on = None if on is None else bool(on)
+
+    def __enter__(self):
+        global _saved_hidden
+        self.prev, _saved_hidden = _saved_hidden, self.on
+        return self
+
+    def __exit__(self, *exc):
+        global _saved_hidden
+        _saved_hidden = self.prev
+        return False
+
+
+def saved_hidden_on():
+    return SAVED_HIDDEN_DEFAULT if _saved_hidden is None else _saved_hidden
+
+
+def saved_hidden_floats(R, S):
+    return int(_hip.lib().eslam_saved_hidden_floats(int(R), int(S)))
+
+
+def require_saved_hidden(hid, R, S):
+    want = saved_hidden_floats(R, S)
+    if hid is None:
+        raise RuntimeError(f"saved hidden layer: the forward pass left no buffer ({want} floats for {R} x {S} samples expected)")
+    if hid.dtype != torch.float32 or not hid.is_contiguous() or hid.numel() < want:
+        raise RuntimeError(f"saved hidden layer: {hid.numel()} {hid.dtype} elements, {want} contiguous float32 needed for "
+                           f"{R} x {S} samples")
+    return hid
+
+
 _EXT_WANTED = os.environ.get("ESLAM_TORCH_EXT", "1") != "0"
 _ext_mod = False
 
@@ -271,7 +309,7 @@
             _rng_override is None and rays_o.is_cuda and torch_ext() is not None)
 
 
-def ext_render(cfg, rays_o, rays_d, gt_depth, beta, flat_planes, dec_params, n_strat, n_imp, fl, relayout=False):
+def ext_render(cfg, rays_o, rays_d, gt_depth, beta, flat_planes, dec_params, n_strat, n_imp, fl, relayout=False, saved_hidden=None):
     dev = rays_o.device
     seed_v = _rng_seed(dev)
     state = _rng_state(dev)
@@ -279,17 +317,18 @@
         state[0] += 1
         _rng_pending[dev.index] = False
     ext = torch_ext()
+    keep_h = saved_hidden_on() if saved_hidden is None else bool(saved_hidden)
     with _hip.on_device(dev):
         if fl is None:
             outs = ext.render(cfg, rays_o, rays_d, gt_depth, beta, flat_planes, dec_params, linspace01(n_strat, dev), linspace01(n_imp, dev),
-                              state, seed_v, _ray_offset, relayout=relayout)
+                              state, seed_v, _ray_offset, relayout=relayout, saved_hidden=keep_h)
         else:
             mask = fl.ray_mask
             if mask is not None:
                 mask = _c(mask.view(torch.uint8) if mask.dtype == torch.bool else mask.to(torch.uint8))
             outs = ext.render(cfg, rays_o, rays_d, gt_depth, beta, flat_planes, dec_params, linspace01(n_strat, dev), linspace01(n_imp, dev),
                               state, seed_v, _ray_offset, fl.gt_color, mask, _loss_scratch(dev, rays_o.shape[0]), fl.acc_out,
-                              list(fl.state.weights5), relayout)
+                              list(fl.state.weights5), relayout, keep_h)
             fl.loss, fl.acc = outs[4], outs[5]
             fl.value = outs[4].detach()
     return outs[0], outs[1], outs[2], outs[3]
@@ -501,6 +540,10 @@
         sdf = torch.empty(R, S, device=dev)
         raw_rgb = torch.empty(R, S, 3, device=dev) if needs else None
         feat = torch.empty(R * S, 128, device=dev, dtype=torch.float32 if half is None else torch.bfloat16) if needs else None
+        ctx.extra_inputs = len(tensors) - 24
+        keep_h = bool(tensors[24]) if ctx.extra_inputs else saved_hidden_on()
+        ctx.saved_hidden = bool(needs and half is None and R > 0 and keep_h)
+        hid = torch.empty(saved_hidden_floats(R, S), device=dev) if ctx.saved_hidden else None
         order = None
         ctx.pregrads = None
         if order_in is not None:
@@ -512,11 +555,11 @@
         ctx.lossctx = None
         with _hip.on_device(dev):
             if fl is None:
-                _hip.check(lib.eslam_render_fwd(arr, ctypes.byref(dec), _hip.make_bound(bound6), _hip.ptr(rays_o),
-                                                _hip.ptr(rays_d), _hip.ptr(z_vals), R, S, _hip.ptr(depth), _hip.ptr(rgb),
-                                                _hip.ptr(sdf), _hip.ptr(raw_rgb), _hip.ptr(feat),
-                                                None, _take_rng_bump(dev),
-                                                _hip.stream_handle(dev)), "eslam_render_fwd")
+                _hip.check(lib.eslam_render_fwd_h(arr, ctypes.byref(dec), _hip.make_bound(bound6), _hip.ptr(rays_o),
+                                                  _hip.ptr(rays_d), _hip.ptr(z_vals), R, S, _hip.ptr(depth), _hip.ptr(rgb),
+                                                  _hip.ptr(sdf), _hip.ptr(raw_rgb), _hip.ptr(feat),
+                                                  None, _take_rng_bump(dev), _hip.ptr(hid),
+                                                  _hip.stream_handle(dev)), "eslam_render_fwd")
             else:
                 _hip.require_gpu_f32("gt_depth", fl.gt_depth)
                 _hip.require_gpu_f32("gt_color", fl.gt_color)
@@ -528,21 +571,23 @@
                 st = fl.state
                 st.gt_depth, st.gt_color, st.ray_mask, st.acc, st.value = _c(fl.gt_depth), _c(fl.gt_color), mask, fl.acc, fl.value
                 w5 = (ctypes.c_float * 5)(*st.weights5)
-                _hip.check(lib.eslam_render_fwd_loss(arr, ctypes.byref(dec), _hip.make_bound(bound6), _hip.ptr(rays_o),
-                                                     _hip.ptr(rays_d), _hip.ptr(z_vals), R, S, _hip.ptr(depth),
-                                                     _hip.ptr(rgb), _hip.ptr(sdf), _hip.ptr(raw_rgb), _hip.ptr(feat),
-                                                     None,
-                                                     _hip.ptr(st.gt_depth), _hip.ptr(st.gt_color),
-                                                     st.truncation, w5, _hip.ptr(mask),
-                                                     _hip.ptr(_loss_scratch(dev, R)), _hip.ptr(fl.acc), _hip.ptr(fl.value),
-                                                     _take_rng_bump(dev), _hip.stream_handle(dev)), "eslam_render_fwd_loss")
+                _hip.check(lib.eslam_render_fwd_loss_h(arr, ctypes.byref(dec), _hip.make_bound(bound6), _hip.ptr(rays_o),
+                                                       _hip.ptr(rays_d), _hip.ptr(z_vals), R, S, _hip.ptr(depth),
+                                                       _hip.ptr(rgb), _hip.ptr(sdf), _hip.ptr(raw_rgb), _hip.ptr(feat),
+                                                       None,
+                                                       _hip.ptr(st.gt_depth), _hip.ptr(st.gt_color),
+                                                       st.truncation, w5, _hip.ptr(mask),
+                                                       _hip.ptr(_loss_scratch(dev, R)), _hip.ptr(fl.acc), _hip.ptr(fl.value),
+                                                       _take_rng_bump(dev), _hip.ptr(hid), _hip.stream_handle(dev)),
+                           "eslam_render_fwd_loss")
                 ctx.lossctx = st
         if order_in is not None and side is not None:
             _hip.stream_wait(dev, None, side)
         if needs:
             ctx.bound6 = bound6
             ctx.order_stream = None
-            ctx.save_for_backward(rays_o, rays_d, z_vals, sdf, raw_rgb, feat, order, beta, depth, rgb, *planes, *params)
+            ctx.save_for_backward(rays_o, rays_d, z_vals, sdf, raw_rgb, feat, order, beta, depth, rgb, *planes, *params,
+                                  *(() if hid is None else (hid,)))
         if fl is not None:
             return depth, rgb, sdf, fl.value.detach()
         return depth, rgb, sdf
@@ -553,6 +598,9 @@
         rays_o, rays_d, z_vals, sdf, raw_rgb, feat, order, beta, depth, rgb = saved[:10]
         planes, params = saved[10:22], saved[22:34]
         R, S = z_vals.shape
+        hid = None
+        if ctx.saved_hidden:
+            hid = require_saved_hidden(saved[34] if len(saved) > 34 else None, R, S)
         dev = rays_o.device
         lib = _hip.lib()
         if getattr(ctx, "order_stream", None) is not None:
@@ -596,26 +644,27 @@
             if fl is not None and g_loss is not None:
                 up = _c(g_loss.detach().reshape(1).to(torch.float32))
                 w5 = (ctypes.c_float * 5)(*fl.weights5)
-                _hip.check(lib.eslam_render_bwd_loss(
+                _hip.check(lib.eslam_render_bwd_loss_h(
                     arr, ctypes.byref(dec), _hip.make_bound(ctx.bound6), _hip.ptr(rays_o), _hip.ptr(rays_d),
                     _hip.ptr(z_vals), R, S, _hip.ptr(sdf), _hip.ptr(raw_rgb), _hip.ptr(feat), _hip.ptr(depth), _hip.ptr(rgb),
                     _hip.ptr(fl.gt_depth), _hip.ptr(fl.gt_color), fl.truncation, w5, _hip.ptr(fl.ray_mask),
                     _hip.ptr(fl.acc if fl.acc_global is None else fl.acc_global), _hip.ptr(up), _hip.ptr(fl.value) if fl.rewrite_value else None, _hip.ptr(g_depth),
                     _hip.ptr(g_rgb), _hip.ptr(g_sdf), _hip.ptr(g_dec), _hip.ptr(g_beta), _hip.ptr(g_ro), _hip.ptr(g_rd),
-                    _hip.ptr(order), _hip.ptr(ws), _hip.stream_handle(dev)), "eslam_render_bwd_loss")
+                    _hip.ptr(order), _hip.ptr(ws), _hip.ptr(hid), _hip.stream_handle(dev)), "eslam_render_bwd_loss")
             else:
-                _hip.check(lib.eslam_render_bwd(arr, ctypes.byref(dec), _hip.make_bound(ctx.bound6), _hip.ptr(rays_o),
-                                                _hip.ptr(rays_d), _hip.ptr(z_vals), R, S, _hip.ptr(sdf), _hip.ptr(raw_rgb),
-                                                _hip.ptr(feat), _hip.ptr(g_depth), _hip.ptr(g_rgb), _hip.ptr(g_sdf),
-                                                _hip.ptr(g_dec), _hip.ptr(g_beta), _hip.ptr(g_ro), _hip.ptr(g_rd),
-                                                _hip.ptr(order), _hip.ptr(ws), _hip.stream_handle(dev)),
+                _hip.check(lib.eslam_render_bwd_h(arr, ctypes.byref(dec), _hip.make_bound(ctx.bound6), _hip.ptr(rays_o),
+                                                  _hip.ptr(rays_d), _hip.ptr(z_vals), R, S, _hip.ptr(sdf), _hip.ptr(raw_rgb),
+                                                  _hip.ptr(feat), _hip.ptr(g_depth), _hip.ptr(g_rgb), _hip.ptr(g_sdf),
+                                                  _hip.ptr(g_dec), _hip.ptr(g_beta), _hip.ptr(g_ro), _hip.ptr(g_rd),
+                                                  _hip.ptr(order), _hip.ptr(ws), _hip.ptr(hid), _hip.stream_handle(dev)),
                            "eslam_render_bwd")
         if sink is not None:
-            return (g_ro if need[0] else None, g_rd if need[1] else None) + (None,) * (L - 2 + 24)
+            return (g_ro if need[0] else None, g_rd if need[1] else None) + (None,) * (L - 2 + 24 + ctx.extra_inputs)
         dec_grads = _split_dec_grads(g_dec) if g_dec is not None else [None] * 12
         out = [g_ro if need[0] else None, g_rd if need[1] else None, None, None, g_beta if need[4] else None, None, None]
         out += [grads[i] if (need_planes and need[L + i]) else None for i in range(12)]
         out += [dec_grads[i] if need[L + 12 + i] else None for i in range(12)]
+        out += [None] * ctx.extra_inputs
         return tuple(out)
 
 
diff --git a/myslam_amd/src/utils/Renderer.py b/myslam_amd/src/utils/Renderer.py
--- a/myslam_amd/src/utils/Renderer.py
+++ b/myslam_amd/src/utils/Renderer.py
@@ -15,7 +15,9 @@
         self.bound = eslam.bound.to(eslam.device, non_blocking=True)
         self.H, self.W, self.fx, self.fy, self.cx, self.cy = eslam.H, eslam.W, eslam.fx, eslam.fy, eslam.cx, eslam.cy
 
-    def render_batch_ray(self, all_planes, decoders, rays_d, rays_o, device, truncation, gt_depth=None, _rand=None):
+    def render_batch_ray(self, all_planes, decoders, rays_d, rays_o, device, truncation, gt_depth=None, _rand=None,
+                         saved_hidden=None):
+        keep_h = ops.saved_hidden_on() if saved_hidden is None else bool(saved_hidden)
         n_rays = rays_o.shape[0]
         S = self.n_stratified + self.n_importance
         if gt_depth is None:
@@ -27,7 +29,7 @@
         if ops.ext_render_ok(rays_o, self.n_stratified, _rand):
             return ops.ext_render(self._ext_cfg(truncation, decoders), rays_o, rays_d, gt_depth, beta,
                                   [p for grp in all_planes for p in grp], ops.decoder_params(decoders), self.n_stratified,
-                                  self.n_importance, ops.current_fused_loss(), ops.wants_relayout(all_planes, n_rays * S))
+                                  self.n_importance, ops.current_fused_loss(), ops.wants_relayout(all_planes, n_rays * S), keep_h)
         all_planes = ops.planes_for_kernels(all_planes, n_rays * S)
         flat_planes = [p for grp in all_planes for p in grp]
         grad_on = torch.is_grad_enabled()
@@ -41,7 +43,7 @@
         bound6 = ops.bound_to_host(decoders.bound)
         fl = ops.current_fused_loss()
         outs = ops.RenderFn.apply(rays_o, rays_d, z_vals, bound6, beta, order, fl, *flat_planes,
-                                  *ops.decoder_params(decoders))
+                                  *ops.decoder_params(decoders), keep_h)
         if fl is not None:
             fl.loss = outs[3]
         return outs[0], outs[1], outs[2], z_vals
@@ -63,10 +65,10 @@
         return d
 
     def render_batch_ray_with_loss(self, all_planes, decoders, rays_d, rays_o, device, truncation, gt_depth, gt_color,
-                                   weights, ray_mask=None, _rand=None, acc_out=None):
+                                   weights, ray_mask=None, _rand=None, acc_out=None, saved_hidden=None):
         with ops.fused_loss(gt_depth, gt_color, truncation, weights, ray_mask, acc_out=acc_out) as pre:
             depth, rgb, sdf, z_vals = self.render_batch_ray(all_planes, decoders, rays_d, rays_o, device, truncation,
-                                                            gt_depth=gt_depth, _rand=_rand)
+                                                            gt_depth=gt_depth, _rand=_rand, saved_hidden=saved_hidden)
         return depth, rgb, sdf, z_vals, pre
 
     def sdf2alpha(self, sdf, beta=10):
```
